# wei-zeng98/piano-a2s

Hardware: AMD Instinct MI355X
Metric: training clips/sec (12 s, 5-bar) (higher is better)
Workload: dtype f32

## Files before the change

### piano_a2s_amd/csrc/a2s_bwd.hip

```cpp
#include "a2s_internal.h"

__global__ __launch_bounds__(256) void log_softmax_bwd_rows(const float* __restrict__ g, const float* __restrict__ y,
                                                            long outer_stride, int inner, float* __restrict__ dx,
                                                            int R, int V, int n_outer, int time_major) {
    const int row = blockIdx.x * 4 + (threadIdx.x >> 6), lane = threadIdx.x & 63;
    if (row >= R) return;
    const int ob = row / inner, in = row % inner;
    const float* gr = g + (long)ob * outer_stride + (long)in * V;
    const float* yr = y + (long)ob * outer_stride + (long)in * V;
    float s = 0.f;
    for (int j = lane; j < V; j += 64) s += gr[j];
    s = wave_sum(s);
    const long orow = time_major ? ((long)in * n_outer + ob) : row;
    for (int j = lane; j < V; j += 64) dx[orow * V + j] = gr[j] - expf(yr[j]) * s;
}

int a2s_log_softmax_bwd_rows_impl(hipStream_t st, const float* g, const float* y, long outer_stride, int inner, float* dx,
                                  int R, int V, int n_outer, int time_major) {
    hipLaunchKernelGGL(log_softmax_bwd_rows, dim3(a2s_cdiv(R, 4)), dim3(256), 0, st, g, y, outer_stride, inner, dx, R, V, n_outer, time_major);
    A2S_CHECK_LAUNCH("log_softmax_bwd_rows");
    return A2S_OK;
}

__global__ void gru_gates_bwd(const float* __restrict__ dh_a, long lda, const float* __restrict__ dh_b, long ldb,
                              const float* __restrict__ save, const float* __restrict__ hprev, long ldhp,
                              float* __restrict__ dgi, long ldgi, float* __restrict__ dgh, long ldgh,
                              float* __restrict__ dgh2, long ldgh2, float* __restrict__ dhprev, long lddp, int R, int H) {
    const long idx = (long)blockIdx.x * blockDim.x + threadIdx.x;
    if (idx >= (long)R * H) return;
    const int r_ = (int)(idx / H), j = (int)(idx % H);
    const float* s = save + (long)r_ * 4 * H;
    const float rg = s[j], zg = s[H + j], ng = s[2 * H + j], ghn = s[3 * H + j];
    float dh = dh_a[(long)r_ * lda + j];
    if (dh_b) dh += dh_b[(long)r_ * ldb + j];
    const float hp = hprev ? hprev[(long)r_ * ldhp + j] : 0.f;
    const GruCellGrad cg = gru_cell_bwd(dh, rg, zg, ng, ghn, hp);
    const float dn = cg.dn, dz = cg.dz, dr = cg.dr;
    float* a = dgi + (long)r_ * ldgi;
    a[j] = dr; a[H + j] = dz; a[2 * H + j] = dn;
    float* b = dgh + (long)r_ * ldgh;
    b[j] = dr; b[H + j] = dz; b[2 * H + j] = cg.dnr;
    if (dgh2) { float* c = dgh2 + (long)r_ * ldgh2; c[j] = dr; c[H + j] = dz; c[2 * H + j] = cg.dnr; }
    dhprev[(long)r_ * lddp + j] = cg.dhz;
}

int a2s_gru_gates_bwd_impl(hipStream_t st, const float* dh_a, long lda, const float* dh_b, long ldb, const float* save,
                           const float* hprev, long ldhp, float* dgi, long ldgi, float* dgh, long ldgh, float* dgh2, long ldgh2,
                           float* dhprev, long lddp, int R, int H) {
    hipLaunchKernelGGL(gru_gates_bwd, dim3(a2s_cdiv((long)R * H, 256)), dim3(256), 0, st, dh_a, lda, dh_b, ldb, save, hprev, ldhp,
                       dgi, ldgi, dgh, ldgh, dgh2, ldgh2, dhprev, lddp, R, H);
    A2S_CHECK_LAUNCH("gru_gates_bwd");
    return A2S_OK;
}

__global__ __launch_bounds__(256) void attn_step_bwd(const float* __restrict__ Kmat, const float* __restrict__ enc,
                                                     const float* __restrict__ q, long ldq, const float* __restrict__ v,
                                                     const float* __restrict__ attw, const float* __restrict__ ctx, long ldctx,
                                                     const float* __restrict__ dctx_a, long ldda, const float* __restrict__ dctx_b, long lddb,
                                                     float* __restrict__ dctx_out, long lddo, float* __restrict__ dq, long lddq,
                                                     float* __restrict__ ds_out, int T, int n_clips, int H) {
    extern __shared__ __attribute__((aligned(16))) float sm[];
    float* dsv = sm;
    float* dc = sm + ((T + 3) & ~3);
    float* red = dc + 2 * H;
    const int b = blockIdx.x, tid = threadIdx.x, lane = tid & 63, wave = tid >> 6;
    const int clip = b % n_clips;
    const float* Kb = Kmat + (long)clip * T * H;
    const float* Eb = enc + (long)clip * T * 2 * H;
    float part = 0.f;
    for (int d = tid; d < 2 * H; d += 256) {
        float g = dctx_a[(long)b * ldda + d];
        if (dctx_b) g += dctx_b[(long)b * lddb + d];
        dc[d] = g;
        if (dctx_out) dctx_out[(long)b * lddo + d] = g;
        part += g * ctx[(long)b * ldctx + d];
    }
    const float dot_ctx = block_sum(part, red);
    for (int t = wave; t < T; t += 4) {
        float s = 0.f;
        for (int d = lane; d < 2 * H; d += 64) s = fmaf(dc[d], Eb[(long)t * 2 * H + d], s);
        s = wave_sum(s);
        if (lane == 0) {
            const float d_s = attw[(long)b * T + t] * (s - dot_ctx);
            dsv[t] = d_s;
            if (ds_out) ds_out[(long)b * T + t] = d_s;
        }
    }
    __syncthreads();
    for (int j = tid; j < H; j += 256) {
        const float eq = exp2x_clamped(q[(long)b * ldq + j]), vj = v[j];
        float acc = 0.f;
        for (int t = 0; t < T; ++t) acc = fmaf(dsv[t], sech2_ek(Kb[(long)t * H + j], eq), acc);
        dq[(long)b * lddq + j] = acc * vj;
    }
}

static int attn_step_bwd_split_impl(hipStream_t st, const float* Kmat, const float* enc, const float* q, long ldq, const float* v,
                                 const float* attw, const float* ctx, long ldctx, const float* dctx_a, long ldda, const float* dctx_b,
                                 long lddb, float* dctx_out, long lddo, float* dq, long lddq, float* ds_out, float* ws, int B, int T, int H,
                                 const a2s_attn_rows* rows);

int a2s_attn_step_bwd_impl(hipStream_t st, const float* Kmat, const float* enc, const float* q, long ldq, const float* v,
                           const float* attw, const float* ctx, long ldctx, const float* dctx_a, long ldda, const float* dctx_b,
                           long lddb, float* dctx_out, long lddo, float* dq, long lddq, float* ds_out, int B, int T, int H, float* ws,
                           const a2s_attn_rows* rows) {
    if (H == 256 && ws)
        return attn_step_bwd_split_impl(st, Kmat, enc, q, ldq, v, attw, ctx, ldctx, dctx_a, ldda, dctx_b, lddb, dctx_out, lddo, dq, lddq, ds_out, ws, B, T, H, rows);
    const int n_clips = rows ? rows->n_clips : B;
    const size_t shm = (((T + 3) & ~3) + 2 * H + 16) * sizeof(float);
    A2S_REQUIRE(H >= 1 && H <= 512, "attn_step_bwd: hidden_size must be in 1 .. 512 (got %d)", H);
    hipLaunchKernelGGL(attn_step_bwd, dim3(B), dim3(256), shm, st, Kmat, enc, q, ldq, v, attw, ctx, ldctx, dctx_a, ldda, dctx_b, lddb, dctx_out, lddo, dq, lddq, ds_out, T, n_clips, H);
    A2S_CHECK_LAUNCH("attn_step_bwd");
    return A2S_OK;
}

__global__ __launch_bounds__(256) void attn_dk_accum(const float* __restrict__ Kmat, const float* __restrict__ q_all,
                                                     const float* __restrict__ ds_all, const float* __restrict__ v,
                                                     float* __restrict__ dK, float* __restrict__ dv_partial, int B, int T, int S,
                                                     const int* __restrict__ row_until, int groups, int H) {
    constexpr int TT = 16;
    const int tiles = (T + TT - 1) / TT;
    const int b = blockIdx.x / tiles, t0 = (blockIdx.x % tiles) * TT;
    __shared__ float dss[TT];
    for (int j0 = 0; j0 < H; j0 += blockDim.x) {
        const int j = j0 + threadIdx.x;
        float kreg[TT], acc[TT];
        float dvj = 0.f;
        if (j < H) {
#pragma unroll
            for (int i = 0; i < TT; ++i) { kreg[i] = (t0 + i < T) ? Kmat[((long)b * T + t0 + i) * H + j] : 0.f; acc[i] = 0.f; }
        }
        for (int sg = 0; sg < S * groups; ++sg) {
            const int s = sg / groups, grp = sg % groups;
            if (row_until && s >= row_until[grp * B + b]) continue;
            const long row = (long)sg * B + b;
// ... 205 lines not shown
}

__global__ __launch_bounds__(256) void col_sum(const float* __restrict__ x, long ld, float* __restrict__ out, long rows, int C,
                                               float alpha, float beta) {
    const int c = blockIdx.x * 64 + (threadIdx.x & 63);
    const int part = threadIdx.x >> 6;
    __shared__ float red[4][64];
    float s = 0.f;
    if (c < C) for (long r = part; r < rows; r += 4) s += x[r * ld + c];
    red[part][threadIdx.x & 63] = s;
    __syncthreads();
    if (part == 0 && c < C) {
        const float t = red[0][threadIdx.x] + red[1][threadIdx.x] + red[2][threadIdx.x] + red[3][threadIdx.x];
        out[c] = alpha * t + (beta != 0.f ? beta * out[c] : 0.f);
    }
}

__global__ __launch_bounds__(256) void col_sum_partial(const float* __restrict__ x, long ld, float* __restrict__ partial, long rows, int C, long rpb) {
    const int c = blockIdx.x * 64 + (threadIdx.x & 63);
    const int part = threadIdx.x >> 6;
    const long r0 = (long)blockIdx.y * rpb, r1 = min(rows, r0 + rpb);
    __shared__ float red[4][64];
    float s = 0.f;
    if (c < C) for (long r = r0 + part; r < r1; r += 4) s += x[r * ld + c];
    red[part][threadIdx.x & 63] = s;
    __syncthreads();
    if (part == 0 && c < C)
        partial[(long)blockIdx.y * C + c] = red[0][threadIdx.x] + red[1][threadIdx.x] + red[2][threadIdx.x] + red[3][threadIdx.x];
}

int a2s_col_sum_impl(hipStream_t st, const float* x, long ld, float* out, long rows, int C, float alpha, float beta, float* ws, size_t ws_floats) {
    if (ws && rows >= 2048 && ws_floats >= (size_t)2 * C) {
        long nb = (rows + 511) / 512;
        if (nb > 1024) nb = 1024;
        if ((size_t)nb * C > ws_floats) nb = (long)(ws_floats / C);
        const long rpb = (rows + nb - 1) / nb;
        nb = (rows + rpb - 1) / rpb;
        hipLaunchKernelGGL(col_sum_partial, dim3(a2s_cdiv(C, 64), (unsigned)nb), dim3(256), 0, st, x, ld, ws, rows, C, rpb);
        A2S_CHECK_LAUNCH("col_sum_partial");
        hipLaunchKernelGGL(col_sum, dim3(a2s_cdiv(C, 64)), dim3(256), 0, st, ws, (long)C, out, nb, C, alpha, beta);
        A2S_CHECK_LAUNCH("col_sum");
        return A2S_OK;
    }
    hipLaunchKernelGGL(col_sum, dim3(a2s_cdiv(C, 64)), dim3(256), 0, st, x, ld, out, rows, C, alpha, beta);
    A2S_CHECK_LAUNCH("col_sum");
    return A2S_OK;
}

__global__ void embed_scatter_add(float* __restrict__ table_grad, const long long* __restrict__ ids64, const int* __restrict__ ids32,
                                  long id_stride, int const_id, const float* __restrict__ g, long ldg, int col0, int R, int E,
                                  const uint8_t* __restrict__ drop, float inv_keep) {
    const long idx = (long)blockIdx.x * blockDim.x + threadIdx.x;
    if (idx >= (long)R * E) return;
    const int r = (int)(idx / E), j = (int)(idx % E);
    const long id = ids64 ? ids64[(long)r * id_stride] : (ids32 ? ids32[(long)r * id_stride] : const_id);
    float v = g[(long)r * ldg + col0 + j];
    if (drop) v = drop[idx] ? v * inv_keep : 0.f;
    atomicAdd(table_grad + id * E + j, v);
}

int a2s_embed_scatter_add_impl(hipStream_t st, float* table_grad, const long long* ids64, const int* ids32, long id_stride,
                               int const_id, const float* g, long ldg, int col0, int R, int E, const uint8_t* drop, float inv_keep) {
    hipLaunchKernelGGL(embed_scatter_add, dim3(a2s_cdiv((long)R * E, 256)), dim3(256), 0, st, table_grad, ids64, ids32, id_stride,
                       const_id, g, ldg, col0, R, E, drop, inv_keep);
    A2S_CHECK_LAUNCH("embed_scatter_add");
    return A2S_OK;
}

__global__ void ew_act_bwd(const float* __restrict__ g, const float* __restrict__ y, float* __restrict__ dx, long n, int act) {
    const long stride = (long)gridDim.x * blockDim.x;
    for (long i = (long)blockIdx.x * blockDim.x + threadIdx.x; i < n; i += stride) {
        const float yy = y[i];
        dx[i] = act == 2 ? g[i] * (1.f - yy * yy) : (yy > 0.f ? g[i] : 0.f);
    }
}
int a2s_ew_act_bwd_impl(hipStream_t st, const float* g, const float* y, float* dx, long n, int act) {
    hipLaunchKernelGGL(ew_act_bwd, dim3(min((long)2048, (n + 255) / 256)), dim3(256), 0, st, g, y, dx, n, act);
    A2S_CHECK_LAUNCH("ew_act_bwd");
    return A2S_OK;
}


static int attn_pair_bwd_sweep(hipStream_t st, const a2s_note_dec_bwd_args& au, const a2s_note_dec_bwd_args& al, int s, AttnPairStep& p);
static int attn_pair_bwd_combine(hipStream_t st, const a2s_note_dec_bwd_args& a, int s, const AttnPairStep& p);

struct NoteBwdStaff { bool mid = false; int cur = 0; int fused_rows_limit = -1; };
static int note_bwd_step_rows(const a2s_note_dec_bwd_args& a, int s) { return (a.row_list && a.n_rows_active) ? a.n_rows_active[s] : a.R; }
static bool note_bwd_step_fused(const a2s_note_dec_bwd_args& a, int s, int rows_limit) {
    const void* ptrs[] = {a.dgi_all, a.dgh_all, a.dq_all, a.dx, a.dh, a.w_ih, a.w_hh, a.attn_w};
    const int n = note_bwd_step_rows(a, s);
    if (rows_limit >= 0 && n > rows_limit) return false;
    return n > 0 && a2s_dec_step_fusable(n, a.H, a.E, 173, ptrs, 8, a.step_ws, a.step_ws_floats);
}

static int note_bwd_step(hipStream_t st, const a2s_note_dec_bwd_args& a, int s, NoteBwdStaff& c, int part, const AttnPairStep* pair) {
    const int H2 = 2 * a.H, ldx = a.E + H2, R = a.R;
    const bool fused = note_bwd_step_fused(a, s, c.fused_rows_limit);
    a2s_attn_rows rows_v = {a.clip_order, a.clip_rank, a.row_until, a.n_clips > 0 ? a.n_clips : R, a.n_active ? a.n_active[s] : 0, s};
    const a2s_attn_rows* rows = a.n_active ? &rows_v : nullptr;
    float* dh_in = a.dh + (long)c.cur * R * H2;
    float* dh_out = a.dh + (long)(c.cur ^ 1) * R * H2;
    if (fused) {
        const int nrows = note_bwd_step_rows(a, s);
        int rc = a2s_note_step_fused_bwd(st, a, s, dh_in, dh_out, rows, nrows, nrows < R ? a.row_list : nullptr);
        if (rc) return rc;
        c.cur ^= 1;
        return A2S_OK;
    }
    int gM = R, gB = 1;
    long gS = 0;
    if (a.m_active && a.n_clips > 0 && a2s_prefix_rows_ok(a.m_active[s], a.n_clips)) { gM = a.m_active[s]; gB = R / a.n_clips; gS = a.n_clips; }
    const float* dos = a.do_all + (long)s * R * 2 * H2;
    float* dgi = a.dgi_all + (long)s * R * 3 * H2;
    float* dgh = a.dgh_all + (long)s * R * 3 * H2;
    float* dxs = a.dx + (long)s * R * ldx;
    int rc = A2S_OK;
    if (part != 2) {
        rc = a2s_gru_gates_bwd_impl(st, dh_in, H2, dos, 2 * H2, a.gates + (long)s * R * 4 * H2, a.h + (long)s * R * H2, H2,
                                    dgi, 3 * H2, dgh, 3 * H2, nullptr, 0, dh_out, H2, R, H2);
        if (rc) return rc;
        if (c.mid) {
            const int nrows = note_bwd_step_rows(a, s);
            rc = a2s_note_step_mid_bwd(st, a, s, dh_out, nrows, nrows < R ? a.row_list : nullptr);
        } else {
            rc = a2s_gemm_impl(st, gM, ldx, 3 * H2, 1.f, dgi, 3 * H2, 1, a.w_ih, ldx, 1, 0.f, dxs, ldx, nullptr, 0, gB, gS * 3 * H2, 0, gS * ldx, 0, a.gemm_ws, a.gemm_ws_bytes);
        }
        if (rc) return rc;
        if (part == 1) return A2S_OK;
    }
    rc = pair ? attn_pair_bwd_combine(st, a, s, *pair)
              : a2s_attn_step_bwd_impl(st, a.keys, a.enc, a.q + (long)s * R * a.H, a.H, a.attn_v, a.attw + (long)s * R * a.T,
                                       a.x + (long)s * R * ldx + a.E, ldx, dxs + a.E, ldx, dos + H2, 2 * H2,
                                       a.dctx_all + (long)s * R * H2, H2, a.dq_all + (long)s * R * a.H, a.H,
                                       a.ds_all + (long)s * R * a.T, R, a.T, a.H, a.attn_ws, rows);
    if (rc) return rc;
    if (!c.mid) {
        rc = a2s_gemm_impl(st, gM, H2, 3 * H2, 1.f, dgh, 3 * H2, 1, a.w_hh, H2, 1, 1.f, dh_out, H2, nullptr, 0, gB, gS * 3 * H2, 0, gS * H2, 0, a.gemm_ws, a.gemm_ws_bytes);
        if (rc) return rc;
    }
    if (c.mid) {
        const int nrows = note_bwd_step_rows(a, s);
        rc = a2s_note_step_mid_bwd_query(st, a, s, dh_out, nrows, nrows < R ? a.row_list : nullptr);
    } else
    rc = a2s_gemm_impl(st, gM, H2, a.H, 1.f, a.dq_all + (long)s * R * a.H, a.H, 1, a.attn_w, 2 * H2, 1, 1.f, dh_out, H2, nullptr, 0, gB, gS * a.H, 0, gS * H2, 0, a.gemm_ws, a.gemm_ws_bytes);
    if (rc) return rc;
    c.cur ^= 1;
    return A2S_OK;
}

static int note_bwd_prepare(hipStream_t st, const a2s_note_dec_bwd_args& a, NoteBwdStaff& c) {
    const int H2 = 2 * a.H, ldx = a.E + H2, R = a.R;
    hipError_t e = hipMemsetAsync(a.dh, 0, sizeof(float) * 2 * R * H2, st);
    if (e == hipSuccess && (a.m_active || a.row_list)) e = hipMemsetAsync(a.dx, 0, sizeof(float) * (size_t)a.steps * R * ldx, st);
    if (e != hipSuccess) A2S_FAIL(A2S_ERR_HIP, "note_decoder_bwd memset: %s", hipGetErrorString(e));
    bool any_fused = false;
    for (int s = a.steps - 1; s >= 0 && !any_fused; --s) any_fused = note_bwd_step_fused(a, s, c.fused_rows_limit);
    const bool mid = a2s_note_step_mid_bwd_ok(a);
    bool any_mid = false;
    if (mid) for (int s = a.steps - 1; s >= 0 && !any_mid; --s) any_mid = !note_bwd_step_fused(a, s, c.fused_rows_limit);
    if (any_fused || any_mid) { int rc = a2s_note_step_fused_bwd_prepare(st, a); if (rc) return rc; }
    c.mid = mid;
    return A2S_OK;
}
static int note_bwd_finish(hipStream_t st, const a2s_note_dec_bwd_args& a, int cur) {
    if (cur != 0) {
        const hipError_t e = hipMemcpyAsync(a.dh, a.dh + (long)a.R * 2 * a.H, sizeof(float) * a.R * 2 * a.H, hipMemcpyDeviceToDevice, st);
        if (e != hipSuccess) A2S_FAIL(A2S_ERR_HIP, "note_decoder_bwd copy: %s", hipGetErrorString(e));
    }
    return A2S_OK;
}

int a2s_note_decoder_bwd_impl(hipStream_t st, const a2s_note_dec_bwd_args& a) {
    if (a2s_note_decoder_bwd_persist_ok(a)) return a2s_note_decoder_bwd_persist(st, a);
    NoteBwdStaff c;
    int rc = note_bwd_prepare(st, a, c);
    if (rc) return rc;
    for (int s = a.steps - 1; s >= 0; --s) {
        rc = note_bwd_step(st, a, s, c, 0, nullptr);
        if (rc) return rc;
    }
    return note_bwd_finish(st, a, c.cur);
}

int a2s_note_decoder_bwd_pair_impl(hipStream_t su, hipStream_t sl, const a2s_note_dec_bwd_args& au, const a2s_note_dec_bwd_args& al, const int* pair_order,
                                   const int* pair_rank, const int* pair_n_active) {
    const a2s_note_dec_bwd_args* as[2] = {&au, &al};
    hipStream_t sts[2] = {su, sl};
    const bool can_pair = a2s_sw(A2S_SW_attn_pair) && su != sl && pair_order && pair_rank && pair_n_active && au.n_active && al.n_active && au.n_clips > 0 &&
                          au.n_clips == al.n_clips && au.R == al.R && au.T == al.T && au.H == 256 && al.H == 256 && au.enc == al.enc && au.attn_ws && al.attn_ws &&
                          !a2s_note_decoder_bwd_persist_ok(au) && !a2s_note_decoder_bwd_persist_ok(al) && a2s_note_step_mid_bwd_ok(au) && a2s_note_step_mid_bwd_ok(al);
    if (!can_pair) {
        const int rc = a2s_note_decoder_bwd_impl(su, au);
        return rc ? rc : a2s_note_decoder_bwd_impl(sl, al);
    }
    const char* who = "note_decoder_bwd_pair";
    hipEvent_t* ev = nullptr;
    { const int rc = a2s_pair_events(who, &ev); if (rc) return rc; }
    NoteBwdStaff cs[2] = {{.fused_rows_limit = a2s_attn_pair_fused_rows()}, {.fused_rows_limit = a2s_attn_pair_fused_rows()}};
    for (int k = 0; k < 2; ++k) { const int rc = note_bwd_prepare(sts[k], *as[k], cs[k]); if (rc) return rc; }
    const int nmax = au.steps > al.steps ? au.steps : al.steps;
    for (int s = nmax - 1; s >= 0; --s) {
        bool in[2], fused[2] = {false, false};
        for (int k = 0; k < 2; ++k) { in[k] = s < as[k]->steps; if (in[k]) fused[k] = note_bwd_step_fused(*as[k], s, cs[k].fused_rows_limit); }
        AttnPairStep p = {pair_order, pair_rank, au.n_clips, pair_n_active[s], s, 1, au.T};
        const bool joint = in[0] && in[1] && cs[0].mid && cs[1].mid && !fused[0] && !fused[1] && p.n_active > 0 && au.n_active[s] > 0 && al.n_active[s] > 0;
        if (!joint) {
            for (int k = 0; k < 2; ++k)
                if (in[k]) { const int rc = note_bwd_step(sts[k], *as[k], s, cs[k], 0, nullptr); if (rc) return rc; }
            continue;
        }
        for (int k = 0; k < 2; ++k) { const int rc = note_bwd_step(sts[k], *as[k], s, cs[k], 1, nullptr); if (rc) return rc; }
        int rc = a2s_record_wait(ev[1], sl, su, who);
        if (rc == A2S_OK) rc = attn_pair_bwd_sweep(su, au, al, s, p);
        if (rc == A2S_OK) rc = a2s_record_wait(ev[0], su, sl, who);
        if (rc) return rc;
        for (int k = 0; k < 2; ++k) { const int rc2 = note_bwd_step(sts[k], *as[k], s, cs[k], 2, &p); if (rc2) return rc2; }
    }
    for (int k = 0; k < 2; ++k) { const int rc = note_bwd_finish(sts[k], *as[k], cs[k].cur); if (rc) return rc; }
    return A2S_OK;
}


__global__ void transpose_f32(const float* __restrict__ in, float* __restrict__ out, int rows, int cols) {
    const int idx = blockIdx.x * blockDim.x + threadIdx.x;
    if (idx >= rows * cols) return;
    const int c = idx / rows, r = idx % rows;
    out[idx] = in[(long)r * cols + c];
}

int a2s_gru_seq_bwd_impl(hipStream_t st, const float* dout, long do_bstride, long do_tstride, const float* out, long out_bstride,
                         long out_tstride, const float* gates, const float* w_hh, const float* dhn, float* dgi_all, float* dgh_shift,
                         float* dgh_first, float* dhbuf, float* dgh_tmp, int B, int T, int H, int reverse, float* ws, size_t ws_bytes,
                         float* ranges_out, int* ranges_valid) {
    A2S_REQUIRE(dout && out && gates && w_hh && dgi_all && dgh_shift && dgh_first && dhbuf && dgh_tmp, "gru_seq_bwd: null tensor");
    if (ranges_valid) *ranges_valid = 0;
    hipError_t e;
    if (dhn) e = hipMemcpyAsync(dhbuf, dhn, sizeof(float) * B * H, hipMemcpyDeviceToDevice, st);
    else e = hipMemsetAsync(dhbuf, 0, sizeof(float) * B * H, st);
    if (e != hipSuccess) A2S_FAIL(A2S_ERR_HIP, "gru_seq_bwd init: %s", hipGetErrorString(e));
    e = hipMemsetAsync(dgh_shift, 0, sizeof(float) * (size_t)B * T * 3 * H, st);
    if (e != hipSuccess) A2S_FAIL(A2S_ERR_HIP, "gru_seq_bwd memset: %s", hipGetErrorString(e));
    const bool fused = a2s_sw(A2S_SW_gru_fused) && H % 32 == 0 && ws && ws_bytes >= sizeof(float) * 3 * H * H && ((uintptr_t)ws % 16 == 0);
    if (fused) {
        hipLaunchKernelGGL(transpose_f32, dim3(a2s_cdiv(3 * H * H, 256)), dim3(256), 0, st, w_hh, ws, 3 * H, H);
        A2S_CHECK_LAUNCH("transpose_f32");
    }
    if (fused && a2s_gru_seq_bwd_persist_ok(B, T, H, ws, ws_bytes, sizeof(float) * 3 * (size_t)H * H)) {
        const int rc = a2s_gru_seq_bwd_persist_impl(st, dout, do_bstride, do_tstride, out, out_bstride, out_tstride, gates, ws, dhn, dgi_all, dgh_shift, dgh_first,
                                                    B, T, H, reverse, ws, sizeof(float) * 3 * (size_t)H * H, ws_bytes, ranges_out);
        if (rc == A2S_OK && ranges_out && ranges_valid) *ranges_valid = 1;
        return rc;
    }
    if (fused && ws_bytes >= sizeof(float) * (3 * (size_t)H * H + 3 * (size_t)B * H) && (3 * H * H) % 4 == 0) {
        float* tmp[2] = {dgh_tmp, ws + 3 * (size_t)H * H};
        auto tix = [&](int s) { return reverse ? T - 1 - s : s; };
        int cur = 0, p = 0;
        {
            const int s = T - 1, t = tix(s), tp = reverse ? t + 1 : t - 1;
            float* dgh = (s == 0) ? dgh_first : tmp[p];
            int rc = a2s_gru_gates_bwd_impl(st, dhbuf, H, dout + (long)t * do_tstride, do_bstride, gates + (long)t * B * 4 * H,
                                            s == 0 ? nullptr : out + (long)tp * out_tstride, out_bstride,
                                            dgi_all + (long)t * 3 * H, (long)T * 3 * H, dgh, 3 * H,
                                            s == 0 ? nullptr : dgh_shift + (long)tp * 3 * H, (long)T * 3 * H, dhbuf + (long)B * H, H, B, H);
            if (rc) return rc;
            cur = 1;
        }
        for (int s = T - 1; s >= 1; --s) {
            const int sp = s - 1, t = tix(sp), tp = reverse ? t + 1 : t - 1;
            float* dgh_out = (sp == 0) ? dgh_first : tmp[p ^ 1];
            int rc = a2s_gru_bptt_step_impl(st, tmp[p], ws, dhbuf + (long)cur * B * H, dout + (long)t * do_tstride, do_bstride,
                                            gates + (long)t * B * 4 * H, sp == 0 ? nullptr : out + (long)tp * out_tstride, out_bstride,
                                            dgi_all + (long)t * 3 * H, (long)T * 3 * H, dgh_out,
                                            sp == 0 ? nullptr : dgh_shift + (long)tp * 3 * H, (long)T * 3 * H,
                                            dhbuf + (long)(cur ^ 1) * B * H, B, H);
            if (rc) return rc;
            cur ^= 1; p ^= 1;
        }
        return A2S_OK;
    }
    int cur = 0;
    for (int s = T - 1; s >= 0; --s) {
        const int t = reverse ? T - 1 - s : s;
        const int tp = reverse ? t + 1 : t - 1;
        float* dh_in = dhbuf + (long)cur * B * H;
        float* dh_out = dhbuf + (long)(cur ^ 1) * B * H;
        float* dgh = (s == 0) ? dgh_first : dgh_tmp;
        int rc = a2s_gru_gates_bwd_impl(st, dh_in, H, dout + (long)t * do_tstride, do_bstride, gates + (long)t * B * 4 * H,
                                        s == 0 ? nullptr : out + (long)tp * out_tstride, out_bstride,
                                        dgi_all + (long)t * 3 * H, (long)T * 3 * H, dgh, 3 * H,
                                        s == 0 ? nullptr : dgh_shift + (long)tp * 3 * H, (long)T * 3 * H, dh_out, H, B, H);
        if (rc) return rc;
        if (s > 0) {
            if (fused) rc = a2s_skinny_gemm_acc_impl(st, dgh, 3 * H, ws, 3 * H, dh_out, H, B, H, 3 * H);
            else rc = a2s_gemm_impl(st, B, H, 3 * H, 1.f, dgh, 3 * H, 1, w_hh, H, 1, 1.f, dh_out, H, nullptr, 0, 1, 0, 0, 0, 0, ws, ws_bytes);
            if (rc) return rc;
        }
        cur ^= 1;
    }
    return A2S_OK;
}
// ... 628 lines not shown
                        const float d_s = aw[r] * (acc[r] - dotn);
                        dsv[li * chunk + f2] = d_s;
                        if (ds_out) ds_out[arow + f2] = d_s;
                    }
                }
            }
        }
    }
    __syncthreads();
#pragma unroll
    for (int pass = 0; pass < 2; ++pass) {
        const int side = pass == 0 ? pre_side : 1 - pre_side;
        const int smask = (onmask >> (side * NQ)) & ((1 << NQ) - 1);
        if (!smask) continue;
        const AttnPairBwdSide& sd = side ? s1 : s0;
        const float* Kb = sd.Kmat + ((long)b * T + t0) * H;
        const float* dsj = dsv + side * NQ * chunk;
        f32x4 q4[NQ], acc[NQ];
#pragma unroll
        for (int j = 0; j < NQ; ++j) {
            acc[j] = (f32x4){0.f, 0.f, 0.f, 0.f};
            q4[j] = ((smask >> j) & 1) ? *reinterpret_cast<const f32x4*>(sd.q + ((long)j * n_clips + b) * ldq + c4 * 4) : (f32x4){0.f, 0.f, 0.f, 0.f};
#pragma unroll
            for (int c = 0; c < 4; ++c) q4[j][c] = exp2x_clamped(q4[j][c]);
        }
        int i = rg;
        auto tile = [&](const f32x4 (&k)[4]) {
#pragma unroll
            for (int j = 0; j < NQ; ++j) {
                if (!((smask >> j) & 1)) continue;
#pragma unroll
                for (int u = 0; u < 4; ++u) {
                    const float w = dsj[j * chunk + i + 4 * u];
#pragma unroll
                    for (int c = 0; c < 4; ++c) acc[j][c] = fmaf(w, sech2_ek(k[u][c], q4[j][c]), acc[j][c]);
                }
            }
        };
        if (pass == 0) {
#pragma unroll
            for (int p = 0; p < KPRE; ++p)
                if (i + 12 < n) { tile(kpre[p]); i += 16; }
        }
        for (; i + 12 < n; i += 16) {
            f32x4 k[4];
#pragma unroll
            for (int u = 0; u < 4; ++u) k[u] = ld_kv<NT>(Kb + (long)(i + 4 * u) * H + c4 * 4);
            tile(k);
        }
        for (; i < n; i += 4) {
            const f32x4 k0 = ld_kv<NT>(Kb + (long)i * H + c4 * 4);
#pragma unroll
            for (int j = 0; j < NQ; ++j) {
                if (!((smask >> j) & 1)) continue;
                const float w = dsj[j * chunk + i];
#pragma unroll
                for (int c = 0; c < 4; ++c) acc[j][c] = fmaf(w, sech2_ek(k0[c], q4[j][c]), acc[j][c]);
            }
        }
        if (pass == 1) __syncthreads();
        if (rg > 0) {
#pragma unroll
            for (int j = 0; j < NQ; ++j) red4[(j * 3 + rg - 1) * 64 + c4] = acc[j];
        }
        __syncthreads();
        if (rg == 0) {
            const f32x4 v4 = {sd.v[c4 * 4], sd.v[c4 * 4 + 1], sd.v[c4 * 4 + 2], sd.v[c4 * 4 + 3]};
#pragma unroll
            for (int j = 0; j < NQ; ++j) {
                if (!((smask >> j) & 1)) continue;
                f32x4 a = acc[j];
#pragma unroll
                for (int u = 0; u < 3; ++u) { const f32x4 o = red4[(j * 3 + u) * 64 + c4];
#pragma unroll
                    for (int c = 0; c < 4; ++c) a[c] += o[c]; }
#pragma unroll
                for (int c = 0; c < 4; ++c) a[c] *= v4[c];
                *reinterpret_cast<f32x4*>(sd.dq_partial + (((long)slot * NQ + j) * G + g) * H + c4 * 4) = a;
            }
        }
    }
}

__global__ __launch_bounds__(256) void attn_bwd_combine256(const float* __restrict__ dq_partial, float* __restrict__ dq, long lddq, int G,
                                                           const int* __restrict__ clip_rank, const int* __restrict__ row_until,
                                                           int n_clips, int groups, int n_active, int step, float* __restrict__ ds_out,
                                                           int T, float* __restrict__ dctx_out, long lddo) {
    const int b = blockIdx.x, j = threadIdx.x;
    const int clip = b % n_clips, grp = b / n_clips;
    const int slot = clip_rank ? clip_rank[clip] : clip;
    if (slot >= n_active || (row_until && step >= row_until[b])) {
        dq[(long)b * lddq + j] = 0.f;
        if (ds_out) for (int t = j; t < T; t += 256) ds_out[(long)b * T + t] = 0.f;
        if (dctx_out) for (int d = j; d < 512; d += 256) dctx_out[(long)b * lddo + d] = 0.f;
        return;
    }
    const float* pb = dq_partial + ((long)slot * groups + grp) * G * 256;
    float s = 0.f;
    for (int g0 = 0; g0 < G; g0 += 8) {
        float p[8];
#pragma unroll
        for (int u = 0; u < 8; ++u) p[u] = (g0 + u < G) ? pb[(long)(g0 + u) * 256 + j] : 0.f;
#pragma unroll
        for (int u = 0; u < 8; ++u) s += p[u];
    }
    dq[(long)b * lddq + j] = s;
}

template <int NQ>
static void launch_bwd_mq(hipStream_t st, int nwg, size_t shm, const float* Kmat, const float* enc, const float* q, long ldq, const float* v,
                          const float* attw, const float* ctx, long ldctx, const float* dctx_a, long ldda, const float* dctx_b, long lddb,
                          float* dctx_out, long lddo, float* ws, float* ds_out, int T, int G, int chunk, const a2s_attn_rows& r, bool nt) {
    if (nt) hipLaunchKernelGGL((attn_bwd_split256_mq<NQ, true>), dim3(nwg), dim3(256), shm, st, Kmat, enc, q, ldq, v, attw, ctx, ldctx, dctx_a, ldda, dctx_b, lddb,
                               dctx_out, lddo, ws, ds_out, T, G, chunk, r.clip_order, r.row_until, r.step, r.n_clips);
    else hipLaunchKernelGGL((attn_bwd_split256_mq<NQ, false>), dim3(nwg), dim3(256), shm, st, Kmat, enc, q, ldq, v, attw, ctx, ldctx, dctx_a, ldda, dctx_b, lddb,
                            dctx_out, lddo, ws, ds_out, T, G, chunk, r.clip_order, r.row_until, r.step, r.n_clips);
}

static int attn_step_bwd_split_impl(hipStream_t st, const float* Kmat, const float* enc, const float* q, long ldq, const float* v,
                                 const float* attw, const float* ctx, long ldctx, const float* dctx_a, long ldda, const float* dctx_b,
                                 long lddb, float* dctx_out, long lddo, float* dq, long lddq, float* ds_out, float* ws, int B, int T, int H,
                                 const a2s_attn_rows* rows) {
    A2S_REQUIRE(H == 256 && ws, "attn_step_bwd_split: needs hidden_size 256 and a workspace");
    A2S_REQUIRE(ldq % 4 == 0 && ldctx % 4 == 0 && ldda % 4 == 0 && (!dctx_b || lddb % 4 == 0) && (!dctx_out || lddo % 4 == 0),
                "attn_step_bwd_split: row strides must be multiples of 4 floats");
    A2S_REQUIRE(((uintptr_t)q | (uintptr_t)ctx | (uintptr_t)dctx_a | (uintptr_t)dctx_b | (uintptr_t)dctx_out | (uintptr_t)Kmat | (uintptr_t)enc) % 16 == 0,
                "attn_step_bwd_split: 16-byte alignment");
    a2s_attn_rows r = {nullptr, nullptr, nullptr, B, B, 0};
    if (rows) r = *rows;
    A2S_REQUIRE(r.n_clips > 0 && B % r.n_clips == 0, "attn_step_bwd_split: rows (%d) must be a multiple of the clips (%d)", B, r.n_clips);
    const int groups = B / r.n_clips;
    A2S_REQUIRE(groups <= A2S_ATTN_MAX_GROUPS, "attn_step_bwd_split: at most %d fused bars (got %d)", A2S_ATTN_MAX_GROUPS, groups);
    A2S_REQUIRE(r.n_active >= 0 && r.n_active <= r.n_clips && (!r.clip_order || r.clip_rank), "attn_step_bwd_split: bad row compaction");
    int G = 1, chunk = T;
    ws += A2S_ATTN_TICKETS;
    const bool nt = a2s_sw(A2S_SW_attn_nt) > 0 && r.n_active >= a2s_sw(A2S_SW_attn_nt) && groups == 1;
    if (r.n_active > 0) {
        a2s_attn_split_geometry(r.n_active, T, &G, &chunk);
        {
            const int fine = 4;
            if (fine > 0 && r.n_active <= fine && G == a2s_attn_max_split() && 2 * G <= 64) {
                int c = (T + 2 * G - 1) / (2 * G);
                c = (c + 3) & ~3;
                G = (T + c - 1) / c;
                chunk = c;
            }
        }
        const int nwg = r.n_active * G;
        if (groups == 1) {
            const size_t shm = a2s_attn_bulk_lds((chunk + 3 * 64 * 4) * sizeof(float), r.n_active, 1);
            if (nt) hipLaunchKernelGGL(attn_bwd_split256<true>, dim3(nwg), dim3(256), shm, st, Kmat, enc, q, ldq, v, attw, ctx, ldctx, dctx_a, ldda, dctx_b, lddb,
                                       dctx_out, lddo, ws, ds_out, T, G, chunk, r.clip_order);
            else hipLaunchKernelGGL(attn_bwd_split256<false>, dim3(nwg), dim3(256), shm, st, Kmat, enc, q, ldq, v, attw, ctx, ldctx, dctx_a, ldda, dctx_b, lddb,
                                    dctx_out, lddo, ws, ds_out, T, G, chunk, r.clip_order);
        } else {
            const size_t scratch = (size_t)groups * 3 * 64 * 4 > (size_t)groups * ATT_DCS + 16 ? (size_t)groups * 3 * 64 * 4 : (size_t)groups * ATT_DCS + 16;
            const size_t shm = a2s_attn_bulk_lds(((size_t)groups * chunk + scratch) * sizeof(float), r.n_active, 3);
#define A2S_BWD_MQ(N) launch_bwd_mq<N>(st, nwg, shm, Kmat, enc, q, ldq, v, attw, ctx, ldctx, dctx_a, ldda, dctx_b, lddb, dctx_out, lddo, ws, ds_out, T, G, chunk, r, nt)
            switch (groups) {
                case 2: A2S_BWD_MQ(2); break;
                case 3: A2S_BWD_MQ(3); break;
                case 4: A2S_BWD_MQ(4); break;
                default: A2S_BWD_MQ(5); break;
            }
#undef A2S_BWD_MQ
        }
        A2S_CHECK_LAUNCH("attn_bwd_split256");
    }
    hipLaunchKernelGGL(attn_bwd_combine256, dim3(B), dim3(256), 0, st, ws, dq, lddq, G, r.clip_rank, r.row_until, r.n_clips, groups, r.n_active, r.step,
                       ds_out, T, dctx_out, lddo);
    A2S_CHECK_LAUNCH("attn_bwd_combine256");
    return A2S_OK;
}

template <int NQ>
static void launch_bwd_pair(hipStream_t st, int nwg, size_t shm, const AttnPairBwdSide& s0, const AttnPairBwdSide& s1, const float* enc, long ldq, long ldctx,
                            long ldda, long lddb, long lddo, int T, const AttnPairStep& p) {
    hipLaunchKernelGGL((attn_bwd_split256_pair<NQ, false>), dim3(nwg), dim3(256), shm, st, s0, s1, enc, ldq, ldctx, ldda, lddb, lddo, T, p.G, p.chunk,
                       p.clip_order, p.step, p.n_clips);
}
static long g_attn_pair_bwd_launches = 0;
long a2s_attn_pair_bwd_launches(void) { return g_attn_pair_bwd_launches; }

static AttnPairBwdSide attn_pair_bwd_side(const a2s_note_dec_bwd_args& a, int s) {
    const int H2 = 2 * a.H, ldx = a.E + H2;
    const long R = a.R;
    return AttnPairBwdSide{a.keys, a.q + (long)s * R * a.H, a.attn_v, a.attw + (long)s * R * a.T, a.x + (long)s * R * ldx + a.E, a.dx + (long)s * R * ldx + a.E,
                           a.do_all + (long)s * R * 2 * H2 + H2, a.dctx_all + (long)s * R * H2, a.attn_ws + A2S_ATTN_TICKETS, a.ds_all + (long)s * R * a.T, a.row_until};
}

static int attn_pair_bwd_sweep(hipStream_t st, const a2s_note_dec_bwd_args& au, const a2s_note_dec_bwd_args& al, int s, AttnPairStep& p) {
    const int T = au.T, H2 = 2 * au.H, ldx = au.E + H2, groups = au.R / p.n_clips;
    A2S_REQUIRE(au.H == 256 && au.E == al.E && au.enc == al.enc && au.R == al.R && groups >= 1 && groups <= A2S_ATTN_MAX_GROUPS && ldx % 4 == 0,
                "attn_pair_bwd_sweep: the staves must decode the same rows over the same encoder outputs");
    a2s_attn_split_geometry(p.n_active, T, &p.G, &p.chunk);
    const AttnPairBwdSide s0 = attn_pair_bwd_side(au, s), s1 = attn_pair_bwd_side(al, s);
    const size_t red = (size_t)groups * 3 * 64 * 4, img = (size_t)2 * groups * ATT_DCS + 16;
    const size_t shm = a2s_attn_bulk_lds(((size_t)2 * groups * p.chunk + (red > img ? red : img)) * sizeof(float), p.n_active, 3);
    const int nwg = p.n_active * p.G;
#define A2S_BWD_PAIR(N) launch_bwd_pair<N>(st, nwg, shm, s0, s1, au.enc, au.H, ldx, ldx, 2 * H2, H2, T, p)
    switch (groups) {
        case 1: A2S_BWD_PAIR(1); break;
        case 2: A2S_BWD_PAIR(2); break;
        case 3: A2S_BWD_PAIR(3); break;
        case 4: A2S_BWD_PAIR(4); break;
        default: A2S_BWD_PAIR(5); break;
    }
#undef A2S_BWD_PAIR
    A2S_CHECK_LAUNCH("attn_bwd_split256_pair");
    __atomic_fetch_add(&g_attn_pair_bwd_launches, 1, __ATOMIC_RELAXED);
    return A2S_OK;
}

static int attn_pair_bwd_combine(hipStream_t st, const a2s_note_dec_bwd_args& a, int s, const AttnPairStep& p) {
    const int H2 = 2 * a.H;
    const long R = a.R;
    hipLaunchKernelGGL(attn_bwd_combine256, dim3(a.R), dim3(256), 0, st, a.attn_ws + A2S_ATTN_TICKETS, a.dq_all + (long)s * R * a.H, (long)a.H, p.G, p.clip_rank,
                       a.row_until, p.n_clips, a.R / p.n_clips, p.n_active, p.step, a.ds_all + (long)s * R * a.T, a.T, a.dctx_all + (long)s * R * H2, (long)H2);
    A2S_CHECK_LAUNCH("attn_bwd_combine256");
    return A2S_OK;
}
```

### piano_a2s_amd/csrc/a2s_internal.h

```cpp
#pragma once
#include "a2s_common.h"
#include "../../include/a2s.h"
#include "a2s_switches.h"

static inline int a2s_attn_pair_fused_rows(void) {
    const int cap = a2s_sw(A2S_SW_dec_fused_max_rows), v = a2s_sw(A2S_SW_attn_pair_fused_rows);
    return v < cap ? v : cap;
}
static inline unsigned a2s_persist_dbg(void) {
    return (a2s_sw(A2S_SW_persist_force_agent) ? PERSIST_DBG_FORCE_AGENT : 0u) | (a2s_sw(A2S_SW_persist_inject_abort) ? PERSIST_DBG_INJECT_ABORT : 0u);
}

int a2s_absmax_impl(hipStream_t st, const float* x, long n, float* out);
size_t a2s_gemm_workspace_bytes_impl(int M, int N, int batch, int splitk);
int a2s_gemm_pick_splitk_impl(int M, int N, int K, int batch);
int a2s_gemm_bnstats_slots(int period);
void a2s_gemm_debug_tile_impl(int cfg);
int a2s_gemm_affine_impl(hipStream_t st, int M, int N, int K, float alpha, const float* A, long sAm, long sAk,
    const float* B, long sBk, long sBn, float beta, float* C, long ldc, const float* bias, int act,
    int batch, long bsA, long bsB, long bsC, int splitk, float* ws, size_t ws_bytes,
    const float* a_scale, const float* a_shift, int a_period, const float* b_scale, const float* b_shift, int b_period,
    const float* ep_y, const float* ep_mean, const float* ep_invstd, const float* ep_scale, const float* ep_shift,
    float* ep_partial, int ep_period, int two_term, const float* a_absmax, const float* b_absmax);
int a2s_gemm_impl(hipStream_t st, int M, int N, int K, float alpha, const float* A, long sAm, long sAk,
// ... 37 lines not shown
    const uint8_t* mask, float inv_keep, long n, int C);
size_t a2s_conv3x3_wgrad_workspace_bytes_impl(int Cin, int Cout);
int a2s_conv3x3_wgrad_impl(hipStream_t st, const float* dy, const float* x, const float* in_scale, const float* in_shift, float* dW,
    float* ws, size_t ws_bytes, int B, int T, int F, int Cin, int Cout, const float* bn_y, const float* bn_mean,
    const float* bn_invstd, const float* bn_scale, const float* bn_shift, const float* bn_c12, float* dy_out,
    const float* dy_absmax, const float* act_absmax);
int a2s_bn_bwd_impl(hipStream_t st, const float* g, const float* x, const float* mean, const float* invstd, const float* scale,
    const float* shift, const uint8_t* mask, float inv_keep, float* dgamma, float* dbeta, float* dx, float* partial,
    float* c12, long rows, int C, int F, float* dx_absmax);
int a2s_bn_bwd_from_partial_impl(hipStream_t st, const float* g, const float* x, const float* mean, const float* invstd, const float* scale,
    const float* shift, float* dgamma, float* dbeta, float* dx, const float* partial, int nblocks, float* c12,
    long rows, int C, int F, float* dx_absmax);
int a2s_bn_bwd_stats_impl(hipStream_t st, const float* g, const float* x, const float* mean, const float* invstd, const float* scale,
    const float* shift, const uint8_t* mask, float inv_keep, float* partial, float* sums, long rows, int C, int F);
int a2s_bn_bwd_apply_impl(hipStream_t st, const float* g, const float* x, const float* mean, const float* invstd, const float* scale,
    const float* shift, const uint8_t* mask, float inv_keep, const float* sums_local, const float* sums_global,
    double count_global, float* dgamma, float* dbeta, float* dx, float* c12, long rows, int C, int F);
int a2s_bn_bwd_sums_from_partial_impl(hipStream_t st, const float* partial, int nblocks, int C, float* sums);
int a2s_bn_bwd_c12_from_sums_impl(hipStream_t st, const float* sums_local, const float* sums_global, double count_global, float* dgamma, float* dbeta,
    float* c12, int C);
size_t a2s_bn_bwd_partial_floats_impl(long rows, int C, int F);

int a2s_channel_absmax_impl(hipStream_t st, const float* x, long rows, int C, int F, float* out);
bool a2s_conv_rows_eligible(int F, int Cin);
int a2s_conv_rows_blocks(int B, int T, int F);
size_t a2s_conv_rows_workspace_floats(int Cin);
long a2s_conv_rows16_c20_launches(void);
int a2s_conv3x3_rows_impl(hipStream_t st, const float* x, const float* w, float* y, const float* in_scale, const float* in_shift,
    const float* in_absmax, float* stat_partial, float* out_absmax, int B, int T, int F, int Cin, int Cout, int flip,
    float* ws, const float* yl, const float* yl_mean, const float* yl_invstd, const float* yl_scale, const float* yl_shift,
    const float* x_absmax);

bool a2s_wgrad_rows_eligible(int F, int Cin, int Cout);
int a2s_conv3x3_wgrad_rows_bn_impl(hipStream_t st, const float* g, const float* y, const float* mean, const float* invstd, const float* scale,
    const float* shift, const float* c12, const float* g_absmax, int g_absmax_n, const float* y_absmax, float* dz_out,
    float* dz_absmax_out, const float* x, const float* in_scale, const float* in_shift, float* dW, float* ws, size_t ws_bytes,
    int B, int T, int F, int Cin, int Cout, const float* act_absmax);
int a2s_conv3x3_wgrad_rows_impl(hipStream_t st, const float* dy, const float* x, const float* in_scale, const float* in_shift, float* dW, float* ws,
    size_t ws_bytes, int B, int T, int F, int Cin, int Cout, const float* dy_absmax, const float* act_absmax);

struct StepFinArgs {
    const float* logits; long ldl;
    float* probs; long probs_bstride;
    const long long* gt; long gt_bstride;
    const float* emb;
    float* xnext; long ldx;
    const uint8_t* drop; float inv_keep;
    int* argmax_out; long am_bstride;
    int* eos_seen; long long* lengths; int* n_done; int* steps_exec;
    const int* t_base;
    const int* row_until;
    int n_clips;
    int R, V, E, t, teacher_force, eos_id, max_t;
};
struct a2s_grammar_ref { const signed char* next; int n_states; int* row_state; };
int a2s_gru_gates_fwd_impl(hipStream_t st, const float* gi, long ldgi, const float* gh, long ldgh, const float* hprev,
    long ldhp, float* hout, long ldho, float* hout2, long ldho2, float* save, int R, int H);
int a2s_gru_bptt_step_impl(hipStream_t st, const float* dgh, const float* w_hh_t, const float* dhz_in, const float* dout, long ld_dout,
    const float* save, const float* hprev, long ld_hprev, float* dgi, long ld_dgi, float* dgh_out, float* dgh2,
    long ld_dgh2, float* dhz_out, int R, int H);
int a2s_skinny_gemm_acc_impl(hipStream_t st, const float* A, long lda, const float* Bt, long ldb, float* Cm, long ldc, int R, int N, int K);
int a2s_gru_seq_fwd_impl(hipStream_t st, const float* gi_all, long gi_bstride, long gi_tstride, const float* w_hh,
    const float* b_hh, float* out, long out_bstride, long out_tstride, float* hbuf, float* gh,
    float* save, float* hn, int B, int T, int H, int reverse, float* ws, size_t ws_bytes);
int a2s_attn_step_fwd_impl(hipStream_t st, const float* Kmat, const float* enc, const float* q, long ldq, const float* v,
    float* ctx, long ldctx, float* ctx2, long ldctx2, float* attw, int B, int T, int H,
    const int* n_done, int n_rows_total, float* ws, const a2s_attn_rows* rows = nullptr, a2s_attn_deferred* defer = nullptr);
int a2s_log_softmax_rows_impl(hipStream_t st, const float* x, long ldx, float* y, long ldy, int* argmax_out, int R, int V);
int a2s_embed_rows_impl(hipStream_t st, const float* table, const long long* ids64, const int* ids32, long id_stride,
    int const_id, float* out, long ldo, int col0, int R, int E, const uint8_t* drop, float inv_keep);
int a2s_note_decoder_fwd_impl(hipStream_t st, const a2s_note_dec_args& a, int* steps_done);
int a2s_note_decoder_fwd_grammar_impl(hipStream_t st, const a2s_note_dec_args& a, const a2s_grammar_ref& g, int* steps_done);
int a2s_note_decoder_fwd_pair_impl(hipStream_t su, hipStream_t sl, const a2s_note_dec_args& au, const a2s_note_dec_args& al, const int* pair_order,
    const int* pair_rank, const int* pair_n_active, int* done_u, int* done_l);
int a2s_staff_emb_fwd_impl(hipStream_t st, const float* note_emb, const float* const* w ,
    const long long* ids64, const int* ids32, long id_bstride, const long long* lengths,
    long len_stride, float* out, long ldo, int col0, float* hsave, int R, int maxlen, int E, int S);
int a2s_note_decoder_zero_unwritten(hipStream_t st, const a2s_note_dec_args& a, const char* who );
size_t a2s_attn_workspace_floats_impl(int B, int T, int H, int groups);
size_t a2s_attn_bulk_lds(size_t shm, int n_active, int backward);
long a2s_attn_pair_launches(void);
struct AttnPairStep { const int* clip_order; const int* clip_rank; int n_clips; int n_active; int step; int G; int chunk; };
int a2s_pair_events(const char* who, hipEvent_t** ev_out);
static inline int a2s_record_wait(hipEvent_t ev, hipStream_t from, hipStream_t to, const char* who) {
    hipError_t e = hipEventRecord(ev, from);
    if (e == hipSuccess) e = hipStreamWaitEvent(to, ev, 0);
    if (e != hipSuccess) A2S_FAIL(A2S_ERR_HIP, "%s: event: %s", who, hipGetErrorString(e));
    return A2S_OK;
}

int a2s_log_softmax_bwd_rows_impl(hipStream_t st, const float* g, const float* y, long outer_stride, int inner, float* dx,
    int R, int V, int n_outer, int time_major);
int a2s_gru_gates_bwd_impl(hipStream_t st, const float* dh_a, long lda, const float* dh_b, long ldb, const float* save,
    const float* hprev, long ldhp, float* dgi, long ldgi, float* dgh, long ldgh, float* dgh2, long ldgh2,
    float* dhprev, long lddp, int R, int H);
int a2s_attn_step_bwd_impl(hipStream_t st, const float* Kmat, const float* enc, const float* q, long ldq, const float* v,
    const float* attw, const float* ctx, long ldctx, const float* dctx_a, long ldda, const float* dctx_b,
    long lddb, float* dctx_out, long lddo, float* dq, long lddq, float* ds_out, int B, int T, int H, float* ws,
    const a2s_attn_rows* rows = nullptr);
int a2s_attn_dk_accum_impl(hipStream_t st, const float* Kmat, const float* q_all, const float* ds_all, const float* v,
    float* dK, float* dv_partial, int B, int T, int S, int H, const int* row_until, int groups);
int a2s_attn_denc_accum_impl(hipStream_t st, const float* attw_all, const float* dctx_all, float* dEnc, int B, int T, int S, int H2,
    const int* row_until, int groups);
long a2s_attn_dk_ahead_launches(void);
long a2s_attn_denc_launches(void);
int a2s_col_sum_impl(hipStream_t st, const float* x, long ld, float* out, long rows, int C, float alpha, float beta, float* ws, size_t ws_floats);
int a2s_embed_scatter_add_impl(hipStream_t st, float* table_grad, const long long* ids64, const int* ids32, long id_stride,
    int const_id, const float* g, long ldg, int col0, int R, int E, const uint8_t* drop, float inv_keep);
int a2s_ew_act_bwd_impl(hipStream_t st, const float* g, const float* y, float* dx, long n, int act);
int a2s_note_decoder_bwd_impl(hipStream_t st, const a2s_note_dec_bwd_args& a);
int a2s_note_decoder_bwd_pair_impl(hipStream_t su, hipStream_t sl, const a2s_note_dec_bwd_args& au, const a2s_note_dec_bwd_args& al, const int* pair_order,
    const int* pair_rank, const int* pair_n_active);
int a2s_gru_seq_bwd_impl(hipStream_t st, const float* dout, long do_bstride, long do_tstride, const float* out, long out_bstride,
    long out_tstride, const float* gates, const float* w_hh, const float* dhn, float* dgi_all, float* dgh_shift,
    float* dgh_first, float* dhbuf, float* dgh_tmp, int B, int T, int H, int reverse, float* ws, size_t ws_bytes,
    float* ranges_out, int* ranges_valid);
int a2s_staff_emb_bwd_impl(hipStream_t st, const float* note_emb, const float* const* w, float* const* grads_dev, float* note_emb_grad,
    const long long* ids64, const int* ids32, long id_bstride, const long long* lengths, long len_stride,
    const float* dout, long lddo, int col0, const float* hsave, int R, int maxlen, int E, int S);
long a2s_attn_pair_bwd_launches(void);

size_t a2s_note_step_fused_head_floats(void);
size_t a2s_note_step_workspace_floats_impl(int H, int E);
int a2s_dec_mid_launches(void);
bool a2s_dec_step_fusable(int R, int H, int E, int V, const void* const* ptrs, int nptrs, const float* ws, size_t ws_floats, bool greedy = false);
int a2s_note_step_fused_fwd(hipStream_t st, const a2s_note_dec_args& a, int si, int so, int sv, int sv_next, int t, const int* t_base, int tf, bool last,
    int nrows, const int* rowmap, const a2s_attn_deferred* defer = nullptr);
int a2s_note_step_fused_bwd_prepare(hipStream_t st, const a2s_note_dec_bwd_args& a);
int a2s_note_step_fused_bwd(hipStream_t st, const a2s_note_dec_bwd_args& a, int s, const float* dh_in, float* dh_out, const a2s_attn_rows* rows,
    int nrows, const int* rowmap);
bool a2s_note_step_mid_ok(int H, int E, const void* const* ptrs, int nptrs);
int a2s_note_step_mid_gru(hipStream_t st, const a2s_note_dec_args& a, int si, int so, int sv, int sv_next, int nrows, const int* rowmap);
bool a2s_note_step_mid_bwd_ok(const a2s_note_dec_bwd_args& a);
int a2s_note_step_mid_bwd(hipStream_t st, const a2s_note_dec_bwd_args& a, int s, float* dh_out, int nrows, const int* rowmap);
int a2s_note_step_mid_bwd_query(hipStream_t st, const a2s_note_dec_bwd_args& a, int s, float* dh_out, int nrows, const int* rowmap);

bool a2s_grammar_ref_ok(const a2s_grammar_ref& g, int R, int V);
int a2s_grammar_argmax_rows_impl(hipStream_t st, const float* x, long ldx, float* y, long ldy, const signed char* next, int n_states, int* row_state,
    int* choice_out, int R, int V);
int a2s_grammar_step_finalize_impl(hipStream_t st, const StepFinArgs& a, const a2s_grammar_ref& g);
int a2s_grammar_launches_impl(void);

int a2s_attn_align_rows_impl(hipStream_t st, const float* attw, long ldw, int R, int T, int* peak_out, float* weight_out, float* centroid_out,
    long out_stride, const int* n_done = nullptr, int n_rows_total = 0);
int a2s_align_launches_impl(void);
int a2s_note_decoder_fwd_align_impl(hipStream_t st, const a2s_note_dec_args& a, const a2s_align_args& g, int* steps_done);

int a2s_render_notes_impl(hipStream_t st, const int* programs, int rows_per_clip, int n_samples, float* wave, long wave_bstride, int B);
int a2s_render_launches_impl(void);

int a2s_transpose_targets_impl(hipStream_t st, const int* new_key, const int* interval, const int* token_map, int n_rows, int V, const int* semitones,
    const float* detune, long long* key, long long* upper, long long* lower, int bars, int U, int L, int bins_per_semitone, float* eff_bins, int* counters,
    int B);
int a2s_shift_bins_impl(hipStream_t st, const float* x, float* y, const float* eff_bins, int B, int rows, int F);
int a2s_augment_launches_impl(void);

int a2s_tempo_plan_impl(hipStream_t st, const float* x, int B, int rows, int F, const float* u, float R, int min_frames, int* content, int* step,
    int* counters);
int a2s_stretch_frames_impl(hipStream_t st, const float* x, float* y, const int* step, int B, int rows, int F);
int a2s_tempo_launches_impl(void);

struct BeamStepArgs {
    const float* logits; long ldl;
    const float* emb;
    float* xnext; long ldx;
    float* h; int h_cols;
    float* q; int q_cols;
    const signed char* next; int n_states; int* row_state;
    float* score; int* finished; int* done_count;
    int* token_hist; int* parent_hist; float* score_hist;
    float* probs_scratch;
    int* n_done; int* steps_exec;
    int B, K, V, E, t, max_t, eos_id, pad_id;
};
struct BeamBackArgs {
    const float* score; const int* token_hist; const int* parent_hist; const float* probs_scratch;
    float* probs; long probs_bstride;
    int* ids_out; long ids_bstride; long long* lengths_out; float* score_out;
    const int* steps_exec;
    float alpha;
    int B, K, V, max_t, eos_id, pad_id;
};
bool a2s_beam_args_ok(const a2s_beam_args& g, int R, int n_clips, int V);
int a2s_beam_init_impl(hipStream_t st, const a2s_beam_args& g, int* n_done, int B, int steps);
int a2s_beam_step_finalize_impl(hipStream_t st, const BeamStepArgs& a);
int a2s_beam_backtrack_impl(hipStream_t st, const BeamBackArgs& a);
int a2s_beam_launches_impl(void);
int a2s_note_decoder_fwd_beam_impl(hipStream_t st, const a2s_note_dec_args& a, const a2s_beam_args& g, int* steps_done);

unsigned* a2s_persist_latch_ptr(void);
void a2s_persist_latch_set(void* p);
a2s_device_geom a2s_device_geometry(void);
bool a2s_gru_seq_fwd_persist_ok(const float* w_hh, const float* gi, int B, int T, int H, float* ws, size_t ws_bytes);
int a2s_gru_seq_fwd_persist_impl(hipStream_t st, const float* gi_all, long gi_bstride, long gi_tstride, const float* w_hh, const float* b_hh, float* out,
    long out_bstride, long out_tstride, float* save, float* hn, int B, int T, int H, int reverse, float* ws, size_t ws_bytes);
bool a2s_gru_seq_bwd_persist_ok(int B, int T, int H, float* ws, size_t ws_bytes, size_t ws_used);
int a2s_gru_seq_bwd_persist_impl(hipStream_t st, const float* dout, long do_bstride, long do_tstride, const float* out, long out_bstride, long out_tstride,
    const float* gates, const float* w_hh_t, const float* dhn, float* dgi_all, float* dgh_shift, float* dgh_first, int B, int T,
    int H, int reverse, float* ws, size_t ws_off, size_t ws_bytes, float* ranges_out);

int a2s_dec_persist_launches(void);
bool a2s_note_decoder_fwd_persist_ok(const a2s_note_dec_args& a);
int a2s_note_decoder_fwd_persist(hipStream_t st, const a2s_note_dec_args& a, int* steps_done);
bool a2s_note_decoder_bwd_persist_ok(const a2s_note_dec_bwd_args& a);
int a2s_note_decoder_bwd_persist(hipStream_t st, const a2s_note_dec_bwd_args& a);

int a2s_nll_loss_impl(hipStream_t st, const float* logp, const long long* target, long rows, int V, long long ignore_index,
    float* loss_out , float* dlogp , float gscale, double* partial, int nblocks);
int a2s_nll_grad_impl(hipStream_t st, float* dlogp, const long long* target, const float* loss_out, float gscale, long rows, int V, long long ignore_index);
int a2s_clip_adadelta_impl(hipStream_t st, float* params, float* grads, float* square_avg, float* acc_delta, long n, const float* loss,
    float max_norm, float lr, float rho, float eps, float* ctl , double* partial, int nblocks, int zero_grad);

int a2s_edit_distance_max_len_impl(void);
long a2s_edit_distance_launches(void);
int a2s_edit_distance_impl(hipStream_t st, const int* ref, const long long* ref_off, const int* hyp, const long long* hyp_off, const int* order,
    int n_pairs, int max_ref_len, int max_hyp_len, int* dist);
// ... 10 lines not shown
```

### piano_a2s_amd/csrc/a2s_seq.hip

```cpp
#include <vector>
#include "a2s_internal.h"

__global__ void gru_gates_fwd(const float* __restrict__ gi, long ldgi, const float* __restrict__ gh, long ldgh,
                              const float* __restrict__ hprev, long ldhp, float* __restrict__ hout, long ldho,
                              float* __restrict__ hout2, long ldho2, float* __restrict__ save, int R, int H) {
    const long idx = (long)blockIdx.x * blockDim.x + threadIdx.x;
    if (idx >= (long)R * H) return;
    const int r_ = (int)(idx / H), j = (int)(idx % H);
    const float* a = gi + (long)r_ * ldgi;
    const float* b = gh + (long)r_ * ldgh;
    const float rg = fast_sigmoid(a[j] + b[j]);
    const float zg = fast_sigmoid(a[H + j] + b[H + j]);
    const float ghn = b[2 * H + j];
    const float ng = fast_tanh(a[2 * H + j] + rg * ghn);
    const float hp = hprev[(long)r_ * ldhp + j];
    const float hn = (1.f - zg) * ng + zg * hp;
    hout[(long)r_ * ldho + j] = hn;
    if (hout2) hout2[(long)r_ * ldho2 + j] = hn;
    if (save) {
        float* s = save + (long)r_ * 4 * H;
        s[j] = rg; s[H + j] = zg; s[2 * H + j] = ng; s[3 * H + j] = ghn;
    }
}

// ... 225 lines not shown
    float* sc = sm;
    float* red = sm + ((T + 3) & ~3);
    const int b = blockIdx.x, tid = threadIdx.x, lane = tid & 63, wave = tid >> 6;
    const int clip = b % n_clips;
    const float* Kb = Kmat + (long)clip * T * H;
    const float* Eb = enc + (long)clip * T * 2 * H;
    float qv[PER], vv[PER];
#pragma unroll
    for (int i = 0; i < PER; ++i) {
        const int j = lane + i * 64;
        qv[i] = j < H ? exp2x_clamped(q[(long)b * ldq + j]) : 0.f;
        vv[i] = j < H ? v[j] : 0.f;
    }
    for (int t = wave; t < T; t += 4) {
        float s = 0.f;
#pragma unroll
        for (int i = 0; i < PER; ++i) {
            const int j = lane + i * 64;
            if (j < H) s = fmaf(vv[i], tanh_ek(Kb[(long)t * H + j], qv[i]), s);
        }
        s = wave_sum(s);
        if (lane == 0) sc[t] = s;
    }
    __syncthreads();
    float m = -INFINITY;
    for (int t = tid; t < T; t += 256) m = fmaxf(m, sc[t]);
    m = block_max(m, red);
    float l = 0.f;
    for (int t = tid; t < T; t += 256) { const float p = __expf(sc[t] - m); sc[t] = p; l += p; }
    l = block_sum(l, red);
    const float inv = 1.f / l;
    __syncthreads();
    for (int t = tid; t < T; t += 256) {
        const float w = sc[t] * inv;
        sc[t] = w;
        if (attw) attw[(long)b * T + t] = w;
    }
    __syncthreads();
    for (int d = tid; d < 2 * H; d += 256) {
        float acc = 0.f;
        int t = 0;
        for (; t + 4 <= T; t += 4) {
            const float e0 = Eb[(long)(t + 0) * 2 * H + d], e1 = Eb[(long)(t + 1) * 2 * H + d];
            const float e2 = Eb[(long)(t + 2) * 2 * H + d], e3 = Eb[(long)(t + 3) * 2 * H + d];
            acc = fmaf(sc[t], e0, acc); acc = fmaf(sc[t + 1], e1, acc);
            acc = fmaf(sc[t + 2], e2, acc); acc = fmaf(sc[t + 3], e3, acc);
        }
        for (; t < T; ++t) acc = fmaf(sc[t], Eb[(long)t * 2 * H + d], acc);
        ctx[(long)b * ldctx + d] = acc;
        if (ctx2) ctx2[(long)b * ldctx2 + d] = acc;
    }
}

static int attn_step_fwd_split_impl(hipStream_t st, const float* Kmat, const float* enc, const float* q, long ldq, const float* v,
                                 float* ctx, long ldctx, float* ctx2, long ldctx2, float* attw, float* ws, int B, int T, int H,
                                 const int* n_done, int n_rows_total, const a2s_attn_rows* rows, a2s_attn_deferred* defer = nullptr);

int a2s_attn_step_fwd_impl(hipStream_t st, const float* Kmat, const float* enc, const float* q, long ldq, const float* v,
                           float* ctx, long ldctx, float* ctx2, long ldctx2, float* attw, int B, int T, int H,
                           const int* n_done, int n_rows_total, float* ws, const a2s_attn_rows* rows, a2s_attn_deferred* defer) {
    if (defer) defer->G = 0;
    if (H == 256 && ws)
        return attn_step_fwd_split_impl(st, Kmat, enc, q, ldq, v, ctx, ldctx, ctx2, ldctx2, attw, ws, B, T, H, n_done, n_rows_total, rows, defer);
    const int n_clips = rows ? rows->n_clips : B;
    const size_t shm = (((T + 3) & ~3) + 16) * sizeof(float);
    A2S_REQUIRE(H >= 1 && H <= 512, "attn_step_fwd: hidden_size must be in 1 .. 512 (got %d)", H);
#define A2S_ATTN_FWD(P) hipLaunchKernelGGL(attn_step_fwd<P>, dim3(B), dim3(256), shm, st, Kmat, enc, q, ldq, v, ctx, ldctx, ctx2, ldctx2, attw, T, n_done, n_rows_total, n_clips, H)
    switch ((H + 63) / 64) {
        case 1: A2S_ATTN_FWD(1); break;
        case 2: A2S_ATTN_FWD(2); break;
        case 3: A2S_ATTN_FWD(3); break;
        case 4: A2S_ATTN_FWD(4); break;
        case 5: A2S_ATTN_FWD(5); break;
        case 6: A2S_ATTN_FWD(6); break;
        case 7: A2S_ATTN_FWD(7); break;
        default: A2S_ATTN_FWD(8); break;
    }
#undef A2S_ATTN_FWD
    A2S_CHECK_LAUNCH("attn_step_fwd");
    return A2S_OK;
}


__global__ __launch_bounds__(256) void note_step_finalize(StepFinArgs a) {
    const int row = blockIdx.x * 4 + (threadIdx.x >> 6), lane = threadIdx.x & 63;
    if (row >= a.R) return;
    if (*a.n_done >= a.R && a.gt == nullptr) return;
    const int t = a.t + (a.t_base ? *a.t_base : 0);
    if (t >= a.max_t) return;
    const float* lg = a.logits + (long)row * a.ldl;
    const bool finished = a.row_until && t >= a.row_until[row];
    float m = -INFINITY; int mi = 0x7fffffff;
    for (int j = lane; j < a.V; j += 64) { const float x = lg[j]; if (x > m) { m = x; mi = j; } }
#pragma unroll
    for (int o = 32; o > 0; o >>= 1) {
        const float om = __shfl_xor(m, o, 64); const int oi = __shfl_xor(mi, o, 64);
        if (om > m || (om == m && oi < mi)) { m = om; mi = oi; }
    }
    if (!finished) {
        float s = 0.f;
        for (int j = lane; j < a.V; j += 64) s += expf(lg[j] - m);
        s = wave_sum(s);
        const float lse = m + logf(s);
        float* pr = a.probs + (long)row * a.probs_bstride + (long)t * a.V;
        for (int j = lane; j < a.V; j += 64) pr[j] = lg[j] - lse;
    }
    const long long g = a.gt ? a.gt[(long)row * a.gt_bstride + t] : -1;
    const int tf = (a.teacher_force >> (a.n_clips > 0 ? row / a.n_clips : 0)) & 1;
    const int next_id = (a.gt && tf) ? (int)g : mi;
    for (int j = lane; j < a.E; j += 64) {
        float e = a.emb[(long)next_id * a.E + j];
        if (a.drop) e = a.drop[(long)row * a.E + j] ? e * a.inv_keep : 0.f;
        a.xnext[(long)row * a.ldx + j] = e;
    }
    if (lane == 0 && !finished) {
        if (row == 0 && a.steps_exec) *a.steps_exec = t + 1;
        if (a.argmax_out) a.argmax_out[(long)row * a.am_bstride + t] = mi;
        const bool hit = a.gt ? (g == a.eos_id) : (mi == a.eos_id);
        if (hit) {
            if (!a.eos_seen[row]) { a.eos_seen[row] = 1; atomicAdd(a.n_done, 1); }
            a.lengths[row] = t + 1;
        }
    }
}

static int a2s_note_step_finalize_impl(hipStream_t st, const StepFinArgs& a) {
    hipLaunchKernelGGL(note_step_finalize, dim3(a2s_cdiv(a.R, 4)), dim3(256), 0, st, a);
    A2S_CHECK_LAUNCH("note_step_finalize");
    return A2S_OK;
}

__global__ __launch_bounds__(256) void log_softmax_rows(const float* __restrict__ x, long ldx, float* __restrict__ y, long ldy,
                                                        int* __restrict__ argmax_out, int R, int V) {
    const int row = blockIdx.x * 4 + (threadIdx.x >> 6), lane = threadIdx.x & 63;
    if (row >= R) return;
    const float* lg = x + (long)row * ldx;
    float m = -INFINITY; int mi = 0x7fffffff;
    for (int j = lane; j < V; j += 64) { const float v = lg[j]; if (v > m) { m = v; mi = j; } }
#pragma unroll
    for (int o = 32; o > 0; o >>= 1) {
        const float om = __shfl_xor(m, o, 64); const int oi = __shfl_xor(mi, o, 64);
        if (om > m || (om == m && oi < mi)) { m = om; mi = oi; }
    }
    float s = 0.f;
    for (int j = lane; j < V; j += 64) s += expf(lg[j] - m);
    s = wave_sum(s);
    const float lse = m + logf(s);
    for (int j = lane; j < V; j += 64) y[(long)row * ldy + j] = lg[j] - lse;
    if (argmax_out && lane == 0) argmax_out[row] = mi;
}

int a2s_log_softmax_rows_impl(hipStream_t st, const float* x, long ldx, float* y, long ldy, int* argmax_out, int R, int V) {
    hipLaunchKernelGGL(log_softmax_rows, dim3(a2s_cdiv(R, 4)), dim3(256), 0, st, x, ldx, y, ldy, argmax_out, R, V);
    A2S_CHECK_LAUNCH("log_softmax_rows");
    return A2S_OK;
}

__global__ void embed_rows(const float* __restrict__ table, const long long* __restrict__ ids64, const int* __restrict__ ids32,
                           long id_stride, int const_id, float* __restrict__ out, long ldo, int col0, int R, int E,
                           const uint8_t* __restrict__ drop, float inv_keep) {
    const long idx = (long)blockIdx.x * blockDim.x + threadIdx.x;
    if (idx >= (long)R * E) return;
    const int r = (int)(idx / E), j = (int)(idx % E);
    const long id = ids64 ? ids64[(long)r * id_stride] : (ids32 ? ids32[(long)r * id_stride] : const_id);
    float e = table[id * E + j];
    if (drop) e = drop[idx] ? e * inv_keep : 0.f;
    out[(long)r * ldo + col0 + j] = e;
}

int a2s_embed_rows_impl(hipStream_t st, const float* table, const long long* ids64, const int* ids32, long id_stride,
                        int const_id, float* out, long ldo, int col0, int R, int E, const uint8_t* drop, float inv_keep) {
    hipLaunchKernelGGL(embed_rows, dim3(a2s_cdiv((long)R * E, 256)), dim3(256), 0, st, table, ids64, ids32, id_stride, const_id,
                       out, ldo, col0, R, E, drop, inv_keep);
    A2S_CHECK_LAUNCH("embed_rows");
    return A2S_OK;
}

typedef a2s_note_dec_args NoteDecArgs;

static int attn_pair_sweep(hipStream_t st, const NoteDecArgs& au, const NoteDecArgs& al, int sv, AttnPairStep& p);
static int attn_pair_combine(hipStream_t st, const NoteDecArgs& a, int si, int sv, const AttnPairStep& p);
static int note_step_rows(const NoteDecArgs& a, int t) { return (a.row_list && a.n_rows_active && t >= 0) ? a.n_rows_active[t] : a.R; }
static bool note_step_fusable(const NoteDecArgs& a, int t = -1, int rows_limit = -1) {
    const void* ptrs[] = {a.x, a.h, a.o, a.q, a.w_ih, a.w_hh, a.out_w, a.attn_w};
    const int n = note_step_rows(a, t);
    if (rows_limit >= 0 && n > rows_limit) return false;
    return n > 0 && a2s_dec_step_fusable(n, a.H, a.E, a.V, ptrs, 8, a.step_ws, a.step_ws_floats, a.gt == nullptr && !a.gates);
}
static bool note_step_mid(const NoteDecArgs& a, const int* t_base) {
    const void* ptrs[] = {a.x, a.h, a.o, a.q, a.w_ih, a.w_hh, a.out_w, a.attn_w};
    return !t_base && a2s_note_step_mid_ok(a.H, a.E, ptrs, 8);
}
static int enqueue_query(hipStream_t st, const NoteDecArgs& a, int si, int sv) {
    const int H2 = 2 * a.H;
    return a2s_gemm_impl(st, a.R, a.H, H2, 1.f, a.h + (long)si * a.R * H2, H2, 1, a.attn_w, 1, 2 * H2, 0.f, a.q + (long)sv * a.R * a.H, a.H, a.attn_b, 0, 1, 0,
                         0, 0, 0, a.gemm_ws, a.gemm_ws_bytes);
}

struct NoteStepMode {
    const a2s_grammar_ref* grammar = nullptr;
    const a2s_beam_args* beam = nullptr;
    const a2s_align_args* align = nullptr;
    const int* t_base = nullptr;
    bool parity_slots = false;
    bool few_row = false;
    int fused_rows_limit = -1;
    const char* label = "note_decoder";
};
struct NoteStep { int si, so, sv, sv_next, t, tf; bool fused, last; const AttnPairStep* pair; };
static NoteStep note_step_at(const NoteDecArgs& a, const NoteStepMode& m, int s, bool fused, const AttnPairStep* pair = nullptr) {
    const int i = m.parity_slots ? s & 1 : s, o = m.parity_slots ? (s + 1) & 1 : s + 1;
    return {.si = i, .so = o, .sv = i, .sv_next = o, .t = s, .tf = a.tf_flags ? a.tf_flags[s] : 0, .fused = fused, .last = s + 1 == a.steps, .pair = pair};
}

static int enqueue_note_step(hipStream_t st, const NoteDecArgs& a, const NoteStepMode& m, const NoteStep& k) {
    const int si = k.si, so = k.so, sv = k.sv, sv_next = k.sv_next, t = k.t, H2 = 2 * a.H, ldx = a.E + H2;
    float* xs = a.x + (long)si * a.R * ldx;
    float* qs = a.q + (long)sv * a.R * a.H;
    float* os = a.o + (long)sv * a.R * 2 * H2;
    a2s_attn_rows rows_v = {a.clip_order, a.clip_rank, a.row_until, a.n_clips > 0 ? a.n_clips : a.R, a.n_active ? a.n_active[t] : 0, t};
    const a2s_attn_rows* rows = a.n_active ? &rows_v : nullptr;
    int rc;
    if (k.fused) {
        a2s_attn_deferred defer;
        defer.G = 0;
        rc = a2s_attn_step_fwd_impl(st, a.keys, a.enc, qs, a.H, a.attn_v, xs + a.E, ldx, os + H2, 2 * H2, a.attw ? a.attw + (long)sv * a.R * a.T : nullptr, a.R, a.T, a.H,
                                    a.gt ? nullptr : a.n_done, a.R, a.attn_ws, rows, (a.gt && a.n_active && !m.t_base) ? &defer : nullptr);
        if (rc) return rc;
        const int nrows = note_step_rows(a, m.t_base ? -1 : t);
        return a2s_note_step_fused_fwd(st, a, si, so, sv, sv_next, t, m.t_base, k.tf, k.last, nrows, nrows < a.R ? a.row_list : nullptr, defer.G > 0 ? &defer : nullptr);
    }
    int gM = a.R, gB = 1;
    long gS = 0;
    if (a.m_active && a.n_clips > 0 && a2s_prefix_rows_ok(a.m_active[t], a.n_clips)) { gM = a.m_active[t]; gB = a.R / a.n_clips; gS = a.n_clips; }
    const float* hp = a.h + (long)si * a.R * H2;
    float* hq = a.h + (long)so * a.R * H2;
    const a2s_attn_rows rows_b = {nullptr, nullptr, nullptr, a.n_clips, a.n_clips, t};
    if (m.beam) rows = &rows_b;
    const int* attn_done = (a.gt || (m.beam && m.beam->K > 1)) ? nullptr : a.n_done;
    float* attw_s = m.align ? m.align->attw_step : (a.attw ? a.attw + (long)sv * a.R * a.T : nullptr);
    float* q_left = nullptr;
    const bool mid = note_step_mid(a, m.t_base);
    if (!mid) {
        rc = a2s_gemm_impl(st, gM, a.H, H2, 1.f, hp, H2, 1, a.attn_w, 1, 2 * H2, 0.f, qs, a.H, a.attn_b, 0, gB, gS * H2, 0, gS * a.H, 0, a.gemm_ws, a.gemm_ws_bytes);
        if (rc) return rc;
        rc = a2s_gemm_impl(st, gM, 3 * H2, H2, 1.f, hp, H2, 1, a.w_hh, 1, H2, 0.f, a.gh, 3 * H2, a.b_hh, 0, gB, gS * H2, 0, gS * 3 * H2, 0, a.gemm_ws, a.gemm_ws_bytes);
        if (rc) return rc;
    }
    rc = (mid && k.pair) ? attn_pair_combine(st, a, si, sv, *k.pair)
                         : a2s_attn_step_fwd_impl(st, a.keys, a.enc, qs, a.H, a.attn_v, xs + a.E, ldx, os + H2, 2 * H2, attw_s, a.R, a.T, a.H, attn_done, a.R, a.attn_ws, rows);
    if (rc) return rc;
    if (m.align) { rc = a2s_attn_align_rows_impl(st, attw_s, a.T, a.R, a.T, m.align->peak + t, m.align->weight + t, m.align->centroid + t, m.align->out_stride, attn_done, a.R); if (rc) return rc; }
    if (mid) {
        const int nrows = note_step_rows(a, t);
        rc = a2s_note_step_mid_gru(st, a, si, so, sv, k.last ? -1 : sv_next, nrows, nrows < a.R ? a.row_list : nullptr);
        if (rc) return rc;
        if (!k.last) q_left = a.q + (long)sv_next * a.R * a.H;
    } else {
        rc = a2s_gemm_impl(st, gM, 3 * H2, ldx, 1.f, xs, ldx, 1, a.w_ih, 1, ldx, 0.f, a.gi, 3 * H2, a.b_ih, 0, gB, gS * ldx, 0, gS * 3 * H2, 0, a.gemm_ws, a.gemm_ws_bytes);
        if (rc) return rc;
        rc = a2s_gru_gates_fwd_impl(st, a.gi, 3 * H2, a.gh, 3 * H2, hp, H2, hq, H2, os, 2 * H2, a.gates ? a.gates + (long)sv * a.R * 4 * H2 : nullptr, a.R, H2);
        if (rc) return rc;
        rc = a2s_gemm_impl(st, gM, a.V, 2 * H2, 1.f, os, 2 * H2, 1, a.out_w, 1, 2 * H2, 0.f, a.logits, a.V, a.out_b, 0, gB, gS * 2 * H2, 0, gS * a.V, 0, a.gemm_ws, a.gemm_ws_bytes);
        if (rc) return rc;
    }
    if (m.beam) {
        const a2s_beam_args& g = *m.beam;
        const BeamStepArgs bs = {a.logits, a.V, a.emb, a.x + (long)so * a.R * ldx, ldx, hq, H2, q_left, a.H, g.next_state, g.n_states, g.row_state, g.score, g.finished,
                                 g.done_count, g.token_hist, g.parent_hist, g.score_hist, g.probs_scratch, a.n_done, a.steps_exec, a.n_clips, g.K, a.V, a.E, t, a.steps,
                                 a.eos_id, g.pad_id};
        return a2s_beam_step_finalize_impl(st, bs);
    }
    StepFinArgs f;
    f.logits = a.logits; f.ldl = a.V; f.probs = a.probs; f.probs_bstride = a.probs_bstride;
    f.gt = a.gt; f.gt_bstride = a.gt_bstride; f.emb = a.emb;
    f.xnext = a.x + (long)so * a.R * ldx; f.ldx = ldx;
    f.drop = a.drop ? a.drop + (long)so * a.R * a.E : nullptr; f.inv_keep = a.inv_keep;
    f.argmax_out = a.argmax_out; f.am_bstride = a.am_bstride;
    f.eos_seen = a.eos_seen; f.lengths = a.lengths; f.n_done = a.n_done; f.steps_exec = a.steps_exec;
    f.t_base = m.t_base;
    f.row_until = a.n_active ? a.row_until : nullptr; f.n_clips = a.n_clips > 0 ? a.n_clips : a.R;
    f.R = a.R; f.V = a.V; f.E = a.E; f.t = t; f.teacher_force = k.tf; f.eos_id = a.eos_id; f.max_t = a.steps;
    if (m.grammar) return a2s_grammar_step_finalize_impl(st, f, *m.grammar);
    return a2s_note_step_finalize_impl(st, f);
}

__global__ void advance_counter(int* p, int inc) { if (threadIdx.x == 0 && blockIdx.x == 0) *p += inc; }

static int note_decoder_greedy_graph(hipStream_t st, const NoteDecArgs& a, const NoteStepMode& m, int* steps_done) {
    int chunk = a.poll > 0 ? a.poll : 16;
    if (chunk & 1) ++chunk;
    hipError_t e = hipMemsetAsync(a.t_base, 0, sizeof(int), st);
    if (e != hipSuccess) A2S_FAIL(A2S_ERR_HIP, "greedy graph memset: %s", hipGetErrorString(e));
    hipGraph_t graph = nullptr;
    hipGraphExec_t exec = nullptr;
    const bool fused = m.few_row && note_step_fusable(a);
    int rc = fused ? enqueue_query(st, a, 0, 0) : A2S_OK;
    if (rc) return rc;
    e = hipStreamBeginCapture(st, hipStreamCaptureModeRelaxed);
    if (e != hipSuccess) A2S_FAIL(A2S_ERR_HIP, "hipStreamBeginCapture: %s", hipGetErrorString(e));
    for (int j = 0; j < chunk && rc == A2S_OK; ++j)
        rc = enqueue_note_step(st, a, m, {.si = j & 1, .so = (j + 1) & 1, .sv = 0, .sv_next = 0, .t = j, .tf = 0, .fused = fused, .last = false, .pair = nullptr});
    if (rc == A2S_OK) hipLaunchKernelGGL(advance_counter, dim3(1), dim3(64), 0, st, a.t_base, chunk);
    e = hipStreamEndCapture(st, &graph);
    if (rc != A2S_OK) { if (graph) (void)hipGraphDestroy(graph); return rc; }
    if (e != hipSuccess) A2S_FAIL(A2S_ERR_HIP, "hipStreamEndCapture: %s", hipGetErrorString(e));
    e = hipGraphInstantiate(&exec, graph, nullptr, nullptr, 0);
    if (e != hipSuccess) { (void)hipGraphDestroy(graph); A2S_FAIL(A2S_ERR_HIP, "hipGraphInstantiate: %s", hipGetErrorString(e)); }
    int launched = 0;
    while (launched < a.steps) {
        e = hipGraphLaunch(exec, st);
        if (e != hipSuccess) break;
        launched += chunk;
        int done = 0;
        e = hipMemcpyAsync(&done, a.n_done, sizeof(int), hipMemcpyDeviceToHost, st);
        if (e == hipSuccess) e = hipStreamSynchronize(st);
        if (e != hipSuccess || done >= a.R) break;
    }
    (void)hipGraphExecDestroy(exec);
    (void)hipGraphDestroy(graph);
    if (e != hipSuccess) A2S_FAIL(A2S_ERR_HIP, "greedy graph replay: %s", hipGetErrorString(e));
    if (steps_done) *steps_done = launched < a.steps ? launched : a.steps;
    return A2S_OK;
}

int a2s_note_decoder_zero_unwritten(hipStream_t st, const NoteDecArgs& a, const char* who) {
    const long H2 = 2L * a.H, ldx = a.E + H2, n = a.steps, R = a.R;
    hipError_t e = hipMemsetAsync(a.h + R * H2, 0, sizeof(float) * n * R * H2, st);
    if (e == hipSuccess) e = hipMemsetAsync(a.x + R * ldx, 0, sizeof(float) * n * R * ldx, st);
    if (e == hipSuccess) e = hipMemsetAsync(a.q, 0, sizeof(float) * n * R * a.H, st);
    if (e == hipSuccess) e = hipMemsetAsync(a.o, 0, sizeof(float) * n * R * 2 * H2, st);
    if (e == hipSuccess && a.gates) e = hipMemsetAsync(a.gates, 0, sizeof(float) * n * R * 4 * H2, st);
    if (e != hipSuccess) A2S_FAIL(A2S_ERR_HIP, "%s memset: %s", who, hipGetErrorString(e));
    return A2S_OK;
}
static bool note_decoder_tail_rows(const NoteDecArgs& a) { return a.row_list && a.n_rows_active && a.steps > 0; }

static int note_decoder_run(hipStream_t st, const NoteDecArgs& a, const NoteStepMode& m, int* steps_done) {
    if (note_decoder_tail_rows(a)) { const int rc = a2s_note_decoder_zero_unwritten(st, a, "note_decoder"); if (rc) return rc; }
    const bool mid = note_step_mid(a, nullptr);
    bool prev_q = false;
    int s = 0;
    for (; s < a.steps; ++s) {
        const NoteStep k = note_step_at(a, m, s, m.few_row && note_step_fusable(a, s, m.fused_rows_limit));
        if ((k.fused || mid) && !prev_q) { const int rc = enqueue_query(st, a, k.si, k.sv); if (rc) return rc; }
        prev_q = k.fused || mid;
        const int rc = enqueue_note_step(st, a, m, k);
        if (rc) return rc;
        if (!a.gt && a.poll > 0 && ((s + 1) % a.poll == 0) && s + 1 < a.steps) {
            int done = 0;
            hipError_t e = hipMemcpyAsync(&done, a.n_done, sizeof(int), hipMemcpyDeviceToHost, st);
            if (e == hipSuccess) e = hipStreamSynchronize(st);
            if (e != hipSuccess) A2S_FAIL(A2S_ERR_HIP, "%s poll: %s", m.label, hipGetErrorString(e));
            if (done >= a.R) { ++s; break; }
        }
    }
    if (steps_done) *steps_done = s;
    return A2S_OK;
}

static int note_decoder_fwd(hipStream_t st, const NoteDecArgs& a, int* steps_done, const a2s_grammar_ref* grammar) {
    if (!grammar && a2s_note_decoder_fwd_persist_ok(a)) return a2s_note_decoder_fwd_persist(st, a, steps_done);
    if (!a.gt && a.use_graph && a.t_base && !a.gates && !a.attw && !a.drop && st != nullptr)
        return note_decoder_greedy_graph(st, a, {.grammar = grammar, .t_base = a.t_base, .few_row = !grammar}, steps_done);
    return note_decoder_run(st, a, {.grammar = grammar, .few_row = !grammar}, steps_done);
}

int a2s_note_decoder_fwd_impl(hipStream_t st, const NoteDecArgs& a, int* steps_done) { return note_decoder_fwd(st, a, steps_done, nullptr); }

int a2s_note_decoder_fwd_grammar_impl(hipStream_t st, const NoteDecArgs& a, const a2s_grammar_ref& g, int* steps_done) {
    A2S_REQUIRE(!a.gt && !a.tf_flags_dev, "note_decoder_fwd_grammar: greedy decoding only (ground truth given)");
    A2S_REQUIRE(!a.gates && !a.attw && !a.drop && !a.n_active && !a.row_list, "note_decoder_fwd_grammar: inference only (training buffers or row bookkeeping given)");
    A2S_REQUIRE(a2s_grammar_ref_ok(g, a.R, a.V), "note_decoder_fwd_grammar: needs a table of 1..127 states, row states and V <= 256 (got %d states, V = %d)", g.n_states, a.V);
    A2S_REQUIRE(a.R > 0 && a.steps >= 0 && a.n_done && a.eos_seen && a.lengths && a.logits && a.probs, "note_decoder_fwd_grammar: null bookkeeping or output buffers");
    return note_decoder_fwd(st, a, steps_done, &g);
}

int a2s_note_decoder_fwd_align_impl(hipStream_t st, const NoteDecArgs& a, const a2s_align_args& g, int* steps_done) {
    A2S_REQUIRE(!a.gates && !a.attw && !a.drop && !a.n_active && !a.row_list && !a.m_active && !a.clip_order && !a.row_until,
                "note_decoder_fwd_align: inference only (training buffers or row bookkeeping given)");
    A2S_REQUIRE(!(a.gt && (g.next_state || g.n_states || g.row_state)), "note_decoder_fwd_align: a grammar constrains greedy decoding only (ground truth given)");
    A2S_REQUIRE(a.gt ? (a.tf_flags && a.poll == 0) : !a.tf_flags_dev, "note_decoder_fwd_align: a teacher-forced call needs tf_flags and poll = 0, a greedy call no device flags");
    A2S_REQUIRE(a.R > 0 && a.T >= 1 && a.steps >= 0 && a.n_done && a.eos_seen && a.lengths && a.logits && a.probs && a.h && a.x && a.q && a.o,
                "note_decoder_fwd_align: null bookkeeping or output buffers");
    A2S_REQUIRE(g.attw_step && g.peak && g.weight && g.centroid && g.out_stride >= a.steps && g.out_stride >= 1,
                "note_decoder_fwd_align: needs the one-step weights scratch, the three outputs and a row stride >= steps (got %ld for %d steps)", g.out_stride, a.steps);
    const bool with_grammar = g.next_state || g.n_states || g.row_state;
    const a2s_grammar_ref gr = {g.next_state, g.n_states, g.row_state};
    A2S_REQUIRE(!with_grammar || a2s_grammar_ref_ok(gr, a.R, a.V), "note_decoder_fwd_align: needs a table of 1..127 states, row states and V <= 256 (got %d states, V = %d)", g.n_states, a.V);
    return note_decoder_run(st, a, {.grammar = with_grammar ? &gr : nullptr, .align = &g, .label = "note_decoder_fwd_align"}, steps_done);
}

int a2s_note_decoder_fwd_beam_impl(hipStream_t st, const NoteDecArgs& a, const a2s_beam_args& g, int* steps_done) {
    A2S_REQUIRE(!a.gt && !a.tf_flags_dev, "note_decoder_fwd_beam: greedy decoding only (ground truth given)");
    A2S_REQUIRE(!a.gates && !a.attw && !a.drop && !a.n_active && !a.row_list && !a.m_active && !a.clip_order && !a.row_until,
                "note_decoder_fwd_beam: inference only (training buffers or row bookkeeping given)");
    A2S_REQUIRE(a2s_beam_args_ok(g, a.R, a.n_clips, a.V), "note_decoder_fwd_beam: needs 1 <= K <= %d, R = K * n_clips, V <= 256, a table of 1..127 states or none, and "
                "every beam buffer (got K = %d, R = %d, n_clips = %d, V = %d, %d states)", A2S_BEAM_MAX, g.K, a.R, a.n_clips, a.V, g.n_states);
    A2S_REQUIRE(g.ids_out && g.lengths_out && g.score_out, "note_decoder_fwd_beam: null output buffers");
    A2S_REQUIRE(a.steps >= 0 && a.n_done && a.logits && a.probs && a.h && a.x && a.q && a.o, "note_decoder_fwd_beam: null bookkeeping or output buffers");
    int rc = a2s_beam_init_impl(st, g, a.n_done, a.n_clips, a.steps);
    if (rc) return rc;
    int s = 0;
    rc = note_decoder_run(st, a, {.beam = &g, .parity_slots = true, .label = "note_decoder_fwd_beam"}, &s);
    if (rc) return rc;
    const BeamBackArgs bk = {g.score, g.token_hist, g.parent_hist, g.probs_scratch, a.probs, a.probs_bstride, g.ids_out, (long)a.steps, g.lengths_out, g.score_out,
                             a.steps_exec, g.alpha, a.n_clips, g.K, a.V, a.steps, a.eos_id, g.pad_id};
    if (a.steps > 0) { rc = a2s_beam_backtrack_impl(st, bk); if (rc) return rc; }
    if (steps_done) *steps_done = s;
    return A2S_OK;
}

int a2s_pair_events(const char* who, hipEvent_t** ev_out) {
    struct Pair { hipEvent_t ev[2]; };
    static thread_local std::vector<Pair> pairs;
    int dev = 0;
    hipError_t e = hipGetDevice(&dev);
    if (e != hipSuccess) A2S_FAIL(A2S_ERR_HIP, "%s: hipGetDevice: %s", who, hipGetErrorString(e));
    if ((size_t)dev >= pairs.size()) pairs.resize(dev + 1, Pair{{nullptr, nullptr}});
    for (int k = 0; k < 2; ++k)
        if (!pairs[dev].ev[k]) { e = hipEventCreateWithFlags(&pairs[dev].ev[k], hipEventDisableTiming); if (e != hipSuccess) A2S_FAIL(A2S_ERR_HIP, "%s: hipEventCreate: %s", who, hipGetErrorString(e)); }
    *ev_out = pairs[dev].ev;
    return A2S_OK;
}

int a2s_note_decoder_fwd_pair_impl(hipStream_t su, hipStream_t sl, const NoteDecArgs& au, const NoteDecArgs& al, const int* pair_order,
                                   const int* pair_rank, const int* pair_n_active, int* done_u, int* done_l) {
    const NoteDecArgs* as[2] = {&au, &al};
    hipStream_t sts[2] = {su, sl};
    const bool can_pair = a2s_sw(A2S_SW_attn_pair) && su != sl && pair_order && pair_rank && pair_n_active && au.gt && al.gt && au.n_active && al.n_active &&
                          au.n_clips > 0 && au.n_clips == al.n_clips && au.R == al.R && au.T == al.T && au.H == 256 && al.H == 256 && au.enc == al.enc &&
                          au.attn_ws && al.attn_ws && !a2s_note_decoder_fwd_persist_ok(au) && !a2s_note_decoder_fwd_persist_ok(al) &&
                          note_step_mid(au, nullptr) && note_step_mid(al, nullptr);
    if (!can_pair) {
        int rc = a2s_note_decoder_fwd_impl(su, au, done_u);
        return rc ? rc : a2s_note_decoder_fwd_impl(sl, al, done_l);
    }
    const NoteStepMode m = {.few_row = true, .fused_rows_limit = a2s_attn_pair_fused_rows(), .label = "note_decoder_fwd_pair"};
    hipEvent_t* ev = nullptr;
    { const int rc = a2s_pair_events(m.label, &ev); if (rc) return rc; }
    for (int k = 0; k < 2; ++k)
        if (note_decoder_tail_rows(*as[k])) { const int rc = a2s_note_decoder_zero_unwritten(sts[k], *as[k], "note_decoder"); if (rc) return rc; }
    bool prev_q[2] = {false, false};
    const int nmax = au.steps > al.steps ? au.steps : al.steps;
    for (int s = 0; s < nmax; ++s) {
        bool fused[2] = {false, false}, in[2];
        for (int k = 0; k < 2; ++k) {
            in[k] = s < as[k]->steps;
            if (!in[k]) continue;
            fused[k] = note_step_fusable(*as[k], s, m.fused_rows_limit);
            if (!prev_q[k]) { const int rc = enqueue_query(sts[k], *as[k], s, s); if (rc) return rc; }
            prev_q[k] = true;
        }
        AttnPairStep p = {pair_order, pair_rank, au.n_clips, pair_n_active[s], s, 1, au.T};
        const bool joint = in[0] && in[1] && !fused[0] && !fused[1] && p.n_active > 0 && au.n_active[s] > 0 && al.n_active[s] > 0;
        if (joint) {
            int rc = a2s_record_wait(ev[1], sl, su, m.label);
            if (rc == A2S_OK) rc = attn_pair_sweep(su, au, al, s, p);
            if (rc == A2S_OK) rc = a2s_record_wait(ev[0], su, sl, m.label);
            if (rc) return rc;
        }
        for (int k = 0; k < 2; ++k) {
            if (!in[k]) continue;
            const int rc = enqueue_note_step(sts[k], *as[k], m, note_step_at(*as[k], m, s, fused[k], joint ? &p : nullptr));
            if (rc) return rc;
        }
    }
    if (done_u) *done_u = au.steps;
    if (done_l) *done_l = al.steps;
    return A2S_OK;
}

__global__ __launch_bounds__(128) void staff_emb_fwd(const float* __restrict__ note_emb, const float* __restrict__ w_ih_f,
                                                     const float* __restrict__ w_hh_f, const float* __restrict__ b_ih_f,
                                                     const float* __restrict__ b_hh_f, const float* __restrict__ w_ih_r,
                                                     const float* __restrict__ w_hh_r, const float* __restrict__ b_ih_r,
                                                     const float* __restrict__ b_hh_r, const long long* __restrict__ ids64,
                                                     const int* __restrict__ ids32, long id_bstride,
                                                     const long long* __restrict__ lengths, long len_stride,
                                                     float* __restrict__ out, long ldo, int col0, float* __restrict__ hsave,
                                                     int maxlen, int E, int S) {
    extern __shared__ float sm[];
    const int b = blockIdx.x, dir = blockIdx.y, tid = threadIdx.x;
    const float* w_ih = dir ? w_ih_r : w_ih_f; const float* w_hh = dir ? w_hh_r : w_hh_f;
    const float* b_ih = dir ? b_ih_r : b_ih_f; const float* b_hh = dir ? b_hh_r : b_hh_f;
    float* Wi = sm;
    float* Wh = Wi + 3 * S * E;
    float* bi = Wh + 3 * S * S;
    float* bh = bi + 3 * S;
    float* h = bh + 3 * S;
    float* xe = h + S;
    float* g = xe + E;
    for (int i = tid; i < 3 * S * E; i += blockDim.x) Wi[i] = w_ih[i];
    for (int i = tid; i < 3 * S * S; i += blockDim.x) Wh[i] = w_hh[i];
    for (int i = tid; i < 3 * S; i += blockDim.x) { bi[i] = b_ih[i]; bh[i] = b_hh[i]; }
    for (int i = tid; i < S; i += blockDim.x) h[i] = 0.f;
    int len = (int)lengths[(long)b * len_stride];
    len = max(0, min(len, maxlen));
    __syncthreads();
    for (int s = 0; s < len; ++s) {
        const int t = dir ? len - 1 - s : s;
        const long id = ids64 ? ids64[(long)b * id_bstride + t] : ids32[(long)b * id_bstride + t];
        for (int i = tid; i < E; i += blockDim.x) xe[i] = note_emb[id * E + i];
        __syncthreads();
        for (int r = tid; r < 6 * S; r += blockDim.x) {
            float acc;
            if (r < 3 * S) { acc = bi[r]; for (int k = 0; k < E; ++k) acc = fmaf(Wi[r * E + k], xe[k], acc); }
            else { const int rr = r - 3 * S; acc = bh[rr]; for (int k = 0; k < S; ++k) acc = fmaf(Wh[rr * S + k], h[k], acc); }
            g[r] = acc;
        }
        __syncthreads();
        if (tid < S) {
            const float rg = fast_sigmoid(g[tid] + g[3 * S + tid]);
            const float zg = fast_sigmoid(g[S + tid] + g[4 * S + tid]);
            const float ng = fast_tanh(g[2 * S + tid] + rg * g[5 * S + tid]);
            const float hn = (1.f - zg) * ng + zg * h[tid];
            h[tid] = hn;
            if (hsave) hsave[(((long)b * 2 + dir) * maxlen + s) * S + tid] = hn;
        }
        __syncthreads();
    }
    for (int i = tid; i < S; i += blockDim.x) out[(long)b * ldo + col0 + dir * S + i] = h[i];
}

__global__ __launch_bounds__(192) void staff_emb_fwd_e16s32(const float* __restrict__ note_emb, const float* __restrict__ w_ih_f,
                                                            const float* __restrict__ w_hh_f, const float* __restrict__ b_ih_f,
                                                            const float* __restrict__ b_hh_f, const float* __restrict__ w_ih_r,
                                                            const float* __restrict__ w_hh_r, const float* __restrict__ b_ih_r,
                                                            const float* __restrict__ b_hh_r, const long long* __restrict__ ids64,
                                                            const int* __restrict__ ids32, long id_bstride,
                                                            const long long* __restrict__ lengths, long len_stride,
                                                            float* __restrict__ out, long ldo, int col0, float* __restrict__ hsave, int maxlen) {
    constexpr int E = 16, S = 32;
    extern __shared__ __attribute__((aligned(16))) float sm[];
    float* xe = sm;
    float* hb = xe + E;
    float* g = hb + S;
    int* lid = reinterpret_cast<int*>(g + 6 * S);
    const int b = blockIdx.x, dir = blockIdx.y, tid = threadIdx.x;
    const bool gi_role = tid < 3 * S;
    const int r = gi_role ? tid : tid - 3 * S;
    const float* wsrc = gi_role ? (dir ? w_ih_r : w_ih_f) + r * E : (dir ? w_hh_r : w_hh_f) + r * S;
    float w[S];
#pragma unroll
    for (int k = 0; k < S; ++k) w[k] = (gi_role && k >= E) ? 0.f : wsrc[k];
    const float bias = gi_role ? (dir ? b_ih_r : b_ih_f)[r] : (dir ? b_hh_r : b_hh_f)[r];
    int len = (int)lengths[(long)b * len_stride];
    len = max(0, min(len, maxlen));
    for (int i = tid; i < len; i += 192) {
        const int t = dir ? len - 1 - i : i;
// ... 531 lines not shown
        q4[j] = on[j] ? *reinterpret_cast<const f32x4*>(q + ((long)j * n_clips + b) * ldq + lane * 4) : (f32x4){0.f, 0.f, 0.f, 0.f};
    const f32x4 v4 = {v[lane * 4], v[lane * 4 + 1], v[lane * 4 + 2], v[lane * 4 + 3]};
#pragma unroll
    for (int j = 0; j < NQ; ++j)
#pragma unroll
        for (int c = 0; c < 4; ++c) q4[j][c] = exp2x_clamped(q4[j][c]);
#pragma unroll
    for (int u = 0; u < KF; ++u) {
        const int f = wave + 8 * u;
#pragma unroll
        for (int j = 0; j < NQ; ++j) {
            if (!on[j]) continue;
            float sj = v4[0] * tanh_ek(k[u][0], q4[j][0]) + v4[1] * tanh_ek(k[u][1], q4[j][1])
                     + v4[2] * tanh_ek(k[u][2], q4[j][2]) + v4[3] * tanh_ek(k[u][3], q4[j][3]);
            sj = wave_sum_lane63(sj);
            if (lane == 63 && f < n) pw[j * chunk + f] = sj;
        }
    }
    __syncthreads();
    float mj[NQ], lj[NQ];
#pragma unroll
    for (int j = 0; j < NQ; ++j) {
        mj[j] = 0.f; lj[j] = 0.f;
        if (!on[j]) continue;
        const float sc = tid < n ? pw[j * chunk + tid] : -INFINITY;
        const float m = block_max(sc, red);
        const float p = tid < n ? __expf(sc - m) : 0.f;
        if (tid < n) {
            if (scores) scores[((long)j * n_clips + b) * T + t0 + tid] = sc;
            pw[j * chunk + tid] = p;
        }
        lj[j] = block_sum(p, red);
        mj[j] = m;
    }
    __syncthreads();
    f32x4 acc[NQ];
#pragma unroll
    for (int j = 0; j < NQ; ++j) acc[j] = (f32x4){0.f, 0.f, 0.f, 0.f};
#pragma unroll
    for (int m = 0; m < ER; ++m) {
        const int i = rp + 4 * m;
        if (i < n) {
#pragma unroll
            for (int j = 0; j < NQ; ++j) {
                if (!on[j]) continue;
                const float w = pw[j * chunk + i];
#pragma unroll
                for (int c = 0; c < 4; ++c) acc[j][c] = fmaf(w, e[m][c], acc[j][c]);
            }
        }
    }
    f32x4* red4 = reinterpret_cast<f32x4*>(red + 16);
    if (rp > 0) {
#pragma unroll
        for (int j = 0; j < NQ; ++j) red4[(j * 3 + rp - 1) * 128 + c4] = acc[j];
    }
    __syncthreads();
#pragma unroll
    for (int j = 0; j < NQ; ++j) {
        if (!on[j]) continue;
        float* pout = partial + (((long)slot * NQ + j) * G + g) * (2 * H + 4);
        if (rp == 0) {
            f32x4 a = acc[j];
#pragma unroll
            for (int w = 0; w < 3; ++w) {
                const f32x4 o = red4[(j * 3 + w) * 128 + c4];
#pragma unroll
                for (int c = 0; c < 4; ++c) a[c] += o[c];
            }
            *reinterpret_cast<f32x4*>(pout + 4 + c4 * 4) = a;
        }
        if (tid == 0) { pout[0] = mj[j]; pout[1] = lj[j]; }
    }
}
template <int NQ>
static void launch_fwd_deep(hipStream_t st, int nwg, const float* Kmat, const float* enc, const float* q, long ldq, const float* v, float* ws, float* attw,
                            int T, int G, int chunk, const a2s_attn_rows& r) {
    const size_t shm = ((size_t)NQ * chunk + 16 + (size_t)NQ * 3 * 128 * 4) * sizeof(float);
    hipLaunchKernelGGL((attn_fwd_split256_deep<NQ>), dim3(nwg), dim3(512), shm, st, Kmat, enc, q, ldq, v, ws, attw, T, G, chunk, r.clip_order, r.row_until, r.step,
                       r.n_clips);
}


__global__ __launch_bounds__(256) void attn_fwd_combine256(const float* __restrict__ partial, float* __restrict__ ctx, long ldctx,
                                                           float* __restrict__ ctx2, long ldctx2, float* __restrict__ attw, int T, int G,
                                                           const int* __restrict__ n_done, int n_rows_total,
                                                           const int* __restrict__ clip_rank, const int* __restrict__ row_until,
                                                           int n_clips, int groups, int n_active, int step) {
    if (n_done && *n_done >= n_rows_total) return;
    constexpr int H = 256;
    const int b = blockIdx.x;
    const int clip = b % n_clips, grp = b / n_clips;
    const int slot = clip_rank ? clip_rank[clip] : clip;
    if (slot >= n_active || (row_until && step >= row_until[b])) {
        attn_zero_row(AttnCombineOut{ctx + (long)b * ldctx, ctx2 ? ctx2 + (long)b * ldctx2 : nullptr, attw ? attw + (long)b * T : nullptr, T});
        return;
    }
    __shared__ float wgt[80];
    attn_combine_row(partial + ((long)slot * groups + grp) * G * (2 * H + 4), G,
                     AttnCombineOut{ctx + (long)b * ldctx, ctx2 ? ctx2 + (long)b * ldctx2 : nullptr, attw ? attw + (long)b * T : nullptr, T}, wgt);
}

size_t a2s_attn_workspace_floats_impl(int B, int T, int H, int groups) {
    size_t rows = 0;
    for (int n = 1; n <= B; ++n) {
        int G, chunk;
        a2s_attn_split_geometry(n, T, &G, &chunk);
        if ((size_t)n * G > rows) rows = (size_t)n * G;
    }
    return A2S_ATTN_TICKETS + rows * (groups > 0 ? groups : 1) * (2 * H + 4);
}

size_t a2s_attn_bulk_lds(size_t shm, int n_active, int backward) {
    if (!a2s_sw(A2S_SW_attn_bulk_cap)) return shm;
    const size_t c = (backward & 1) ? 28672 : 65536;
    return (n_active >= 64 && c > shm) ? c : shm;
}
template <int NQ>
static void launch_fwd_mq(hipStream_t st, int nwg, size_t shm, const float* Kmat, const float* enc, const float* q, long ldq, const float* v,
                          float* ws, float* attw, int T, int G, int chunk, const a2s_attn_rows& r, const AttnFusedTail& ft, bool nt) {
    if (nt && shm > 65536) {
        static bool raised = false;
        if (!raised) { (void)hipFuncSetAttribute(reinterpret_cast<const void*>(attn_fwd_split256_mq<NQ, true>), hipFuncAttributeMaxDynamicSharedMemorySize, 98304); raised = true; }
    }
    if (nt) hipLaunchKernelGGL((attn_fwd_split256_mq<NQ, true>), dim3(nwg), dim3(256), shm, st, Kmat, enc, q, ldq, v, ws, attw, T, G, chunk,
                               r.clip_order, r.row_until, r.step, r.n_clips, ft);
    else hipLaunchKernelGGL((attn_fwd_split256_mq<NQ, false>), dim3(nwg), dim3(256), shm, st, Kmat, enc, q, ldq, v, ws, attw, T, G, chunk,
                            r.clip_order, r.row_until, r.step, r.n_clips, ft);
}

static int attn_step_fwd_split_impl(hipStream_t st, const float* Kmat, const float* enc, const float* q, long ldq, const float* v,
                                 float* ctx, long ldctx, float* ctx2, long ldctx2, float* attw, float* ws, int B, int T, int H,
                                 const int* n_done, int n_rows_total, const a2s_attn_rows* rows, a2s_attn_deferred* defer) {
    A2S_REQUIRE(H == 256 && ws, "attn_step_fwd_split: needs hidden_size 256 and a workspace");
    A2S_REQUIRE(ldq % 4 == 0 && ((uintptr_t)q % 16 == 0) && ((uintptr_t)Kmat % 16 == 0) && ((uintptr_t)enc % 16 == 0), "attn_step_fwd_split: 16-byte alignment");
    a2s_attn_rows r = {nullptr, nullptr, nullptr, B, B, 0};
    if (rows) r = *rows;
    A2S_REQUIRE(r.n_clips > 0 && B % r.n_clips == 0, "attn_step_fwd_split: rows (%d) must be a multiple of the clips (%d)", B, r.n_clips);
    const int groups = B / r.n_clips;
    A2S_REQUIRE(groups <= A2S_ATTN_MAX_GROUPS, "attn_step_fwd_split: at most %d fused bars (got %d)", A2S_ATTN_MAX_GROUPS, groups);
    A2S_REQUIRE(r.n_active >= 0 && r.n_active <= r.n_clips && (!r.clip_order || r.clip_rank), "attn_step_fwd_split: bad row compaction");
    A2S_REQUIRE(groups == 1 || !n_done, "attn_step_fwd_split: fused bars are a training-only path");
    A2S_REQUIRE(a2s_attn_max_split() <= 64, "attn_step_fwd_split: the split must be <= 64");
    int G = 1, chunk = T;
    int* tickets = reinterpret_cast<int*>(ws);
    float* part = ws + A2S_ATTN_TICKETS;
    const int fmode = a2s_sw(A2S_SW_attn_fused_combine);
    const bool fused = fmode && (fmode == 1 || r.n_active <= fmode) && r.n_clips <= A2S_ATTN_TICKETS / 2;
    const int n_zero = fused ? r.n_clips - r.n_active : 0;
    const AttnFusedTail ft = {fused ? tickets : nullptr, ctx, ldctx, ctx2, ldctx2, r.n_active, B};
    const bool nt = a2s_sw(A2S_SW_attn_nt) > 0 && r.n_active >= a2s_sw(A2S_SW_attn_nt);
    if (r.n_active > 0 || n_zero > 0) {
        if (r.n_active > 0) a2s_attn_split_geometry(r.n_active, T, &G, &chunk);
        const int nwg = r.n_active * G + n_zero;
        if (!fused && !n_done && groups <= 4 && r.n_active <= a2s_sw(A2S_SW_attn_deep) && chunk <= 80) {
            switch (groups) {
                case 1: launch_fwd_deep<1>(st, nwg, Kmat, enc, q, ldq, v, part, attw, T, G, chunk, r); break;
                case 2: launch_fwd_deep<2>(st, nwg, Kmat, enc, q, ldq, v, part, attw, T, G, chunk, r); break;
                case 3: launch_fwd_deep<3>(st, nwg, Kmat, enc, q, ldq, v, part, attw, T, G, chunk, r); break;
                default: launch_fwd_deep<4>(st, nwg, Kmat, enc, q, ldq, v, part, attw, T, G, chunk, r); break;
            }
        } else if (groups == 1) {
            const size_t shm = a2s_attn_bulk_lds((chunk + 16 + 128 * 4) * sizeof(float), r.n_active, 0);
            if (nt && shm > 65536) {
                static bool raised = false;
                if (!raised) { (void)hipFuncSetAttribute(reinterpret_cast<const void*>(attn_fwd_split256<true>), hipFuncAttributeMaxDynamicSharedMemorySize, 98304); raised = true; }
            }
            if (nt) hipLaunchKernelGGL(attn_fwd_split256<true>, dim3(nwg), dim3(256), shm, st, Kmat, enc, q, ldq, v, part, attw, T, G, chunk, n_done, n_rows_total, r.clip_order, ft);
            else hipLaunchKernelGGL(attn_fwd_split256<false>, dim3(nwg), dim3(256), shm, st, Kmat, enc, q, ldq, v, part, attw, T, G, chunk, n_done, n_rows_total, r.clip_order, ft);
        } else {
            const size_t shm = a2s_attn_bulk_lds(((size_t)groups * chunk + 16 + (size_t)groups * 128 * 4) * sizeof(float), r.n_active, 2);
            switch (groups) {
                case 2: launch_fwd_mq<2>(st, nwg, shm, Kmat, enc, q, ldq, v, part, attw, T, G, chunk, r, ft, nt); break;
                case 3: launch_fwd_mq<3>(st, nwg, shm, Kmat, enc, q, ldq, v, part, attw, T, G, chunk, r, ft, nt); break;
                case 4: launch_fwd_mq<4>(st, nwg, shm, Kmat, enc, q, ldq, v, part, attw, T, G, chunk, r, ft, nt); break;
                default: launch_fwd_mq<5>(st, nwg, shm, Kmat, enc, q, ldq, v, part, attw, T, G, chunk, r, ft, nt); break;
            }
        }
        A2S_CHECK_LAUNCH("attn_fwd_split256");
    }
    if (fused) return A2S_OK;
    if (defer && !n_done && r.n_active > 0 && r.n_active <= a2s_sw(A2S_SW_attn_deep) && groups <= 4 && G <= 16 && a2s_sw(A2S_SW_attn_defer_combine)) {
        *defer = a2s_attn_deferred{part, attw, r.clip_rank, r.row_until, G, groups, r.n_clips, r.n_active, r.step, T};
        return A2S_OK;
    }
    hipLaunchKernelGGL(attn_fwd_combine256, dim3(B), dim3(256), 0, st, part, ctx, ldctx, ctx2, ldctx2, attw, T, G, n_done, n_rows_total,
                       r.clip_rank, r.row_until, r.n_clips, groups, r.n_active, r.step);
    A2S_CHECK_LAUNCH("attn_fwd_combine256");
    return A2S_OK;
}

static long g_attn_pair_launches = 0;
long a2s_attn_pair_launches(void) { return g_attn_pair_launches; }

template <int NQ>
static void launch_fwd_pair(hipStream_t st, int nwg, size_t shm, const AttnPairSide& s0, const AttnPairSide& s1, const float* enc, long ldq, int T,
                            const AttnPairStep& p, bool nt) {
    if (nt && shm > 65536) {
        static bool raised = false;
        if (!raised) { (void)hipFuncSetAttribute(reinterpret_cast<const void*>(attn_fwd_split256_pair<NQ, true>), hipFuncAttributeMaxDynamicSharedMemorySize, 98304); raised = true; }
    }
    if (nt) hipLaunchKernelGGL((attn_fwd_split256_pair<NQ, true>), dim3(nwg), dim3(256), shm, st, s0, s1, enc, ldq, T, p.G, p.chunk, p.clip_order, p.step, p.n_clips);
    else hipLaunchKernelGGL((attn_fwd_split256_pair<NQ, false>), dim3(nwg), dim3(256), shm, st, s0, s1, enc, ldq, T, p.G, p.chunk, p.clip_order, p.step, p.n_clips);
}

static int attn_pair_sweep(hipStream_t st, const NoteDecArgs& au, const NoteDecArgs& al, int sv, AttnPairStep& p) {
    const int T = au.T, H = au.H, groups = au.R / p.n_clips;
    A2S_REQUIRE(H == 256 && au.attn_ws && al.attn_ws && au.enc == al.enc && au.R == al.R && au.T == al.T && groups >= 1 && groups <= A2S_ATTN_MAX_GROUPS,
                "attn_pair_sweep: the staves must decode the same rows over the same encoder outputs");
    a2s_attn_split_geometry(p.n_active, T, &p.G, &p.chunk);
    const AttnPairSide s0 = {au.keys, au.q + (long)sv * au.R * H, au.attn_v, au.attn_ws + A2S_ATTN_TICKETS, au.attw ? au.attw + (long)sv * au.R * T : nullptr, au.row_until};
    const AttnPairSide s1 = {al.keys, al.q + (long)sv * al.R * H, al.attn_v, al.attn_ws + A2S_ATTN_TICKETS, al.attw ? al.attw + (long)sv * al.R * T : nullptr, al.row_until};
    const bool nt = a2s_sw(A2S_SW_attn_nt) > 0 && p.n_active >= a2s_sw(A2S_SW_attn_nt);
    const size_t shm = a2s_attn_bulk_lds(((size_t)2 * groups * p.chunk + 16 + (size_t)2 * groups * 128 * 4) * sizeof(float), p.n_active, 2);
    const int nwg = p.n_active * p.G;
    switch (groups) {
        case 1: launch_fwd_pair<1>(st, nwg, shm, s0, s1, au.enc, H, T, p, nt); break;
        case 2: launch_fwd_pair<2>(st, nwg, shm, s0, s1, au.enc, H, T, p, nt); break;
        case 3: launch_fwd_pair<3>(st, nwg, shm, s0, s1, au.enc, H, T, p, nt); break;
        case 4: launch_fwd_pair<4>(st, nwg, shm, s0, s1, au.enc, H, T, p, nt); break;
        default: launch_fwd_pair<5>(st, nwg, shm, s0, s1, au.enc, H, T, p, nt); break;
    }
    A2S_CHECK_LAUNCH("attn_fwd_split256_pair");
    __atomic_fetch_add(&g_attn_pair_launches, 1, __ATOMIC_RELAXED);
    return A2S_OK;
}

static int attn_pair_combine(hipStream_t st, const NoteDecArgs& a, int si, int sv, const AttnPairStep& p) {
    const int H2 = 2 * a.H, ldx = a.E + H2;
    float* xs = a.x + (long)si * a.R * ldx;
    float* os = a.o + (long)sv * a.R * 2 * H2;
    hipLaunchKernelGGL(attn_fwd_combine256, dim3(a.R), dim3(256), 0, st, a.attn_ws + A2S_ATTN_TICKETS, xs + a.E, (long)ldx, os + H2, (long)(2 * H2),
                       a.attw ? a.attw + (long)sv * a.R * a.T : nullptr, a.T, p.G, (const int*)nullptr, a.R, p.clip_rank, a.row_until, p.n_clips,
                       a.R / p.n_clips, p.n_active, p.step);
    A2S_CHECK_LAUNCH("attn_fwd_combine256");
    return A2S_OK;
}
```

### piano_a2s_amd/csrc/a2s_step.hip

```cpp
#include "a2s_internal.h"
#include <type_traits>

#define NW 8
#ifndef DEC_CH_GRU
#define DEC_CH_GRU 1
#define DEC_CH_OUT 1
#define DEC_CH_PROD 1
#define DEC_CH_QUERY 1
#endif
#ifndef DEC_NW_PROD
#define DEC_NW_PROD 8
#define DEC_NW_OUT 8
#endif

template <int NT, int CH, int NWV = NW>
__device__ __forceinline__ void mfma_rows8(const float* __restrict__ arow, const float* const (&brow)[NT], int ksteps, int wave, int lk,
                                           f32x4 (&acc)[NT]) {
    for (int u0 = wave; u0 < ksteps; u0 += NWV * CH) {
        f32x4 a[CH], b[NT][CH];
#pragma unroll
        for (int c = 0; c < CH; ++c) {
            const int u = u0 + NWV * c;
            const bool ok = u < ksteps;
            a[c] = ok ? *reinterpret_cast<const f32x4*>(arow + 16 * u + 4 * lk) : (f32x4){0.f, 0.f, 0.f, 0.f};
// ... 189 lines not shown
            const float mg = have ? pb[(long)lane * CMB_PS] : -INFINITY, lg = have ? pb[(long)lane * CMB_PS + 1] : 0.f;
            float m, inv_l;
            const float wg = attn_merge_weight(mg, lg, have, m, inv_l);
            if (lane < 16) cw[i * 20 + lane] = wg;
            if (lane == 0) { cw[i * 20 + 16] = m; cw[i * 20 + 17] = inv_l; cw[i * 20 + 18] = 1.f; cbase[i] = base; }
        } else if (lane == 0) { cw[i * 20 + 18] = 0.f; cbase[i] = 0; }
    }
    __syncthreads();
    for (int i0 = 0; i0 < nb; i0 += 2) {
        float p[2][16];
#pragma unroll
        for (int rr = 0; rr < 2; ++rr) {
            const int i = min(i0 + rr, nb - 1);
            const bool on = cw[i * 20 + 18] != 0.f;
            const float* pb = c.part + (long)cbase[i] * c.G * CMB_PS + 4 + tid;
#pragma unroll
            for (int u = 0; u < 16; ++u) p[rr][u] = (on && u < c.G) ? pb[(long)u * CMB_PS] : 0.f;
        }
#pragma unroll
        for (int rr = 0; rr < 2; ++rr) {
            const int i = i0 + rr;
            if (i >= nb) break;
            float acc = 0.f;
#pragma unroll
            for (int u = 0; u < 16; ++u) acc = fmaf(p[rr][u], cw[i * 20 + u], acc);
            ctxs[i * CMB_LD + tid] = acc;
        }
    }
    __syncthreads();
    if ((int)blockIdx.x < nb) {
        const int i = blockIdx.x;
        const long row = dec_row(a.rowmap, row0 + i);
        const float v = ctxs[i * CMB_LD + tid];
        c.xw[row * a.ldx + c.E + tid] = v;
        a.o[row * a.ldo + H2 + tid] = v;
    } else if ((int)blockIdx.x >= 16 && (int)blockIdx.x - 16 < nb && c.attw) {
        const int i = blockIdx.x - 16;
        float* aw = c.attw + (long)dec_row(a.rowmap, row0 + i) * c.T;
        const bool on = cw[i * 20 + 18] != 0.f;
        const float m = cw[i * 20 + 16], inv = cw[i * 20 + 17];
        float sv[4];
#pragma unroll
        for (int u = 0; u < 4; ++u) sv[u] = (on && tid + 64 * NW * u < c.T) ? aw[tid + 64 * NW * u] : 0.f;
#pragma unroll
        for (int u = 0; u < 4; ++u) if (tid + 64 * NW * u < c.T) aw[tid + 64 * NW * u] = on ? __expf(sv[u] - m) * inv : 0.f;
        for (int t = tid + 4 * 64 * NW; t < c.T; t += 64 * NW) aw[t] = on ? __expf(aw[t] - m) * inv : 0.f;
    }
    const int arow_i = dec_row(a.rowmap, min(row0 + li, R - 1));
    const float* lrow = ctxs + min(li, nb - 1) * CMB_LD;
    const float* bi[3];
    const float* bh[3];
#pragma unroll
    for (int g = 0; g < 3; ++g) { bi[g] = a.w_ih + ((long)g * H2 + j0 + li) * a.kx; bh[g] = a.w_hh + ((long)g * H2 + j0 + li) * H2; }
    f32x4 t[3], u[3];
#pragma unroll
    for (int g = 0; g < 3; ++g) t[g] = (f32x4){0.f, 0.f, 0.f, 0.f};
    mfma_rows8_split<3, DEC_CH_GRU>(a.x + (long)arow_i * a.ldx, c.E / 16, lrow, bi, a.kx / 16, wave, lk, t);
    u[0] = t[0]; u[1] = t[1]; u[2] = (f32x4){0.f, 0.f, 0.f, 0.f};
    mfma_rows8<3, DEC_CH_GRU>(a.h + (long)arow_i * H2, bh, H2 / 16, wave, lk, u);
    f32x4 acc[4] = {u[0], u[1], t[2], u[2]};
    reduce_waves<4>(acc, part, wave, lane);
    if (wave > 0) return;
#pragma unroll
    for (int r = 0; r < 4; ++r) {
        if (row0 + lk * 4 + r >= R) continue;
        const int row = dec_row(a.rowmap, row0 + lk * 4 + r);
        const GruCellOut cell = gru_cell(acc[0][r], acc[1][r], acc[2][r], acc[3][r], br, bz, bin, bhn, hp[r]);
        const float rg = cell.rg, zg = cell.zg, ng = cell.ng, ghn = cell.ghn, hn = cell.hn;
        a.hout[(long)row * H2 + j] = hn;
        a.o[(long)row * a.ldo + j] = hn;
        if (a.save) {
            float* sv = a.save + (long)row * 4 * H2;
            sv[j] = rg; sv[H2 + j] = zg; sv[2 * H2 + j] = ng; sv[3 * H2 + j] = ghn;
        }
    }
}

#define MID_KC 64
#define MID_LDB 72
#ifndef MID_WAVES
#define MID_WAVES 4
#define MID_AHEAD 1
#endif
__global__ __launch_bounds__(256, MID_WAVES) void dec_gru_mid(DecGruArgs a) {
    __shared__ __attribute__((aligned(16))) float bs[2][48 * MID_LDB];
    const int tid = threadIdx.x, lane = tid & 63, wave = tid >> 6;
    if (a.n_done) {
        const bool done = *a.n_done >= a.R;
        if (blockIdx.x == 0 && blockIdx.y == 0 && tid == 0) *a.skip = done ? 1 : 0;
        if (done) return;
    }
    const int H2 = a.H2, R = a.R, kx = a.kx;
    const int j0 = blockIdx.x * 16, row0 = blockIdx.y * 64 + wave * 16;
    const int li = lane & 15, lk = lane >> 4;
    const int j = j0 + li;
    const int ncx = (kx + MID_KC - 1) / MID_KC, nc = ncx + (H2 + MID_KC - 1) / MID_KC;
    const float br = a.b_ih[j] + a.b_hh[j], bz = a.b_ih[H2 + j] + a.b_hh[H2 + j], bin = a.b_ih[2 * H2 + j], bhn = a.b_hh[2 * H2 + j];
    float hp[4];
#pragma unroll
    for (int r = 0; r < 4; ++r) hp[r] = a.h[(long)dec_row(a.rowmap, min(row0 + lk * 4 + r, R - 1)) * H2 + j];
    const int arow = dec_row(a.rowmap, min(row0 + li, R - 1));
    const float* const xa = a.x + (long)arow * a.ldx + 4 * lk;
    const float* const ha = a.h + (long)arow * H2 + 4 * lk;
    const f32x4 zero4 = {0.f, 0.f, 0.f, 0.f};
    auto bload = [&](int c, f32x4 (&v)[3]) {
        const bool px = c < ncx;
        const int k0 = (px ? c : c - ncx) * MID_KC, K = px ? kx : H2;
        const float* const W = px ? a.w_ih : a.w_hh;
#pragma unroll
        for (int i = 0; i < 3; ++i) {
            const int e = tid + 256 * i, r = e >> 4, k = k0 + 4 * (e & 15);
            v[i] = k < K ? *reinterpret_cast<const f32x4*>(W + ((long)(r >> 4) * H2 + j0 + (r & 15)) * K + k) : zero4;
        }
    };
    auto bstore = [&](int buf, const f32x4 (&v)[3]) {
#pragma unroll
        for (int i = 0; i < 3; ++i) {
            const int e = tid + 256 * i;
            *reinterpret_cast<f32x4*>(&bs[buf][(e >> 4) * MID_LDB + 4 * (e & 15)]) = v[i];
        }
    };
    auto aload = [&](int c, f32x4 (&v)[4]) {
        const bool px = c < ncx;
        const int k0 = (px ? c : c - ncx) * MID_KC, K = px ? kx : H2;
        const float* const p = px ? xa : ha;
#pragma unroll
        for (int u = 0; u < 4; ++u) v[u] = (k0 + 16 * u < K) ? *reinterpret_cast<const f32x4*>(p + k0 + 16 * u) : zero4;
    };
    f32x4 acc[4] = {zero4, zero4, zero4, zero4};
    auto compute = [&](auto PX, int c, int buf, const f32x4 (&av)[4]) {
        constexpr bool px = decltype(PX)::value;
        const int k0 = (px ? c : c - ncx) * MID_KC, K = px ? kx : H2;
#pragma unroll
        for (int u = 0; u < 4; ++u) {
            if (k0 + 16 * u >= K) break;
            f32x4 b[3];
#pragma unroll
            for (int g = 0; g < 3; ++g) b[g] = *reinterpret_cast<const f32x4*>(&bs[buf][(g * 16 + li) * MID_LDB + 16 * u + 4 * lk]);
#pragma unroll
            for (int jj = 0; jj < 4; ++jj) {
                acc[0] = __builtin_amdgcn_mfma_f32_16x16x4f32(av[u][jj], b[0][jj], acc[0], 0, 0, 0);
                acc[1] = __builtin_amdgcn_mfma_f32_16x16x4f32(av[u][jj], b[1][jj], acc[1], 0, 0, 0);
                acc[px ? 2 : 3] = __builtin_amdgcn_mfma_f32_16x16x4f32(av[u][jj], b[2][jj], acc[px ? 2 : 3], 0, 0, 0);
            }
        }
    };
    f32x4 bv[3], a_cur[4], a_n1[4], a_n2[4];
    bload(0, bv);
    aload(0, a_cur);
    if (MID_AHEAD > 1 && nc > 1) aload(1, a_n1);
    bstore(0, bv);
    if (nc > 1) bload(1, bv);
    __syncthreads();
    for (int c = 0; c < nc; ++c) {
#if MID_AHEAD > 1
        if (c + 2 < nc) aload(c + 2, a_n2);
#else
        if (c + 1 < nc) aload(c + 1, a_n1);
#endif
        if (c + 1 < nc) {
            bstore((c + 1) & 1, bv);
            if (c + 2 < nc) bload(c + 2, bv);
        }
        if (c < ncx) compute(std::true_type{}, c, c & 1, a_cur);
        else compute(std::false_type{}, c, c & 1, a_cur);
        __syncthreads();
#pragma unroll
        for (int u = 0; u < 4; ++u) { a_cur[u] = a_n1[u]; if (MID_AHEAD > 1) a_n1[u] = a_n2[u]; }
    }
#pragma unroll
    for (int r = 0; r < 4; ++r) {
        if (row0 + lk * 4 + r >= R) continue;
        const int row = dec_row(a.rowmap, row0 + lk * 4 + r);
        const GruCellOut cell = gru_cell(acc[0][r], acc[1][r], acc[2][r], acc[3][r], br, bz, bin, bhn, hp[r]);
        a.hout[(long)row * H2 + j] = cell.hn;
        a.o[(long)row * a.ldo + j] = cell.hn;
        if (a.save) {
            float* sv = a.save + (long)row * 4 * H2;
            sv[j] = cell.rg; sv[H2 + j] = cell.zg; sv[2 * H2 + j] = cell.ng; sv[3 * H2 + j] = cell.ghn;
        }
    }
}

#define NTV 11
#define NVW 6
struct DecOutArgs {
    const float* o; long ldo; int ko;
    const float* out_w; const float* out_b;
    float* logits; long ldl;
    int* tickets;
    float* probs; long probs_bstride;
    const long long* gt; long gt_bstride;
    const float* emb; float* xnext; long ldx;
    const uint8_t* drop; float inv_keep;
    int* argmax_out; long am_bstride;
    int* eos_seen; long long* lengths; int* n_done; int* steps_exec;
    const int* t_base; const int* row_until; const int* skip;
    const float* hnew; const float* attn_w; long ld_aw; const float* attn_b; float* q_next; int H;
    const int* rowmap;
    int n_clips, R, V, E, t, teacher_force, eos_id, max_t, H2;
};

__device__ __forceinline__ void dec_row_epilogue(const DecOutArgs& a, int vrow, int t, int lane) {
    const volatile float* lg = a.logits + (long)vrow * a.ldl;
    const int row = dec_row(a.rowmap, vrow);
    const bool finished = a.row_until && t >= a.row_until[row];
    float v[3];
    float m = -INFINITY; int mi = 0x7fffffff;
#pragma unroll
    for (int k = 0; k < 3; ++k) {
        const int j = lane + 64 * k;
        v[k] = j < a.V ? lg[j] : -INFINITY;
        if (v[k] > m) { m = v[k]; mi = j; }
    }
#pragma unroll
    for (int o = 32; o > 0; o >>= 1) {
        const float om = __shfl_xor(m, o, 64); const int oi = __shfl_xor(mi, o, 64);
        if (om > m || (om == m && oi < mi)) { m = om; mi = oi; }
    }
    if (!finished) {
        float s = 0.f;
#pragma unroll
        for (int k = 0; k < 3; ++k) if (lane + 64 * k < a.V) s += expf(v[k] - m);
        s = wave_sum(s);
        const float lse = m + logf(s);
        float* pr = a.probs + (long)row * a.probs_bstride + (long)t * a.V;
#pragma unroll
        for (int k = 0; k < 3; ++k) if (lane + 64 * k < a.V) pr[lane + 64 * k] = v[k] - lse;
    }
    const long long gtok = a.gt ? a.gt[(long)row * a.gt_bstride + t] : -1;
    const int tf = (a.teacher_force >> (a.n_clips > 0 ? row / a.n_clips : 0)) & 1;
    const int next_id = (a.gt && tf) ? (int)gtok : mi;
    for (int j = lane; j < a.E; j += 64) {
        float e = a.emb[(long)next_id * a.E + j];
        if (a.drop) e = a.drop[(long)row * a.E + j] ? e * a.inv_keep : 0.f;
        a.xnext[(long)row * a.ldx + j] = e;
    }
    if (lane == 0 && !finished) {
        if (row == 0 && a.steps_exec) *a.steps_exec = t + 1;
        if (a.argmax_out) a.argmax_out[(long)row * a.am_bstride + t] = mi;
        const bool hit = a.gt ? (gtok == a.eos_id) : (mi == a.eos_id);
        if (hit) {
            if (!a.eos_seen[row]) { a.eos_seen[row] = 1; atomicAdd(a.n_done, 1); }
            a.lengths[row] = t + 1;
        }
    }
}

__global__ __launch_bounds__(64 * DEC_NW_OUT) void dec_out_step(DecOutArgs a) {
    __shared__ f32x4 part[(DEC_NW_OUT / 2) * 2 * 64];
    __shared__ int last_flag;
    const int tid = threadIdx.x, lane = tid & 63, wave = tid >> 6;
    if (a.skip && *a.skip) return;
    const int t = a.t + (a.t_base ? *a.t_base : 0);
    if (t >= a.max_t) return;
    const int R = a.R, row0 = blockIdx.x * 16;
    const int li = lane & 15, lk = lane >> 4;
    const bool vocab = (int)blockIdx.y < NVW;
    if (!vocab && !a.q_next) return;
    const int n0 = (vocab ? blockIdx.y : blockIdx.y - NVW) * 32;
    const int ncols = vocab ? a.V : a.H;
    const float* Bm = vocab ? a.out_w : a.attn_w;
    const long ldb = vocab ? (long)a.ko : a.ld_aw;
    const int K = vocab ? a.ko : a.H2;
    const float* brow[2];
// ... 66 lines not shown
    if (wave == 0 && !role_a) {
#pragma unroll
        for (int g = 0; g < 2; ++g)
#pragma unroll
            for (int r = 0; r < 4; ++r) c0[g][r] = a.dh[(long)dec_row(a.rowmap, min(row0 + lk * 4 + r, R - 1)) * a.H2 + min(n0 + g * 16 + li, ncols - 1)];
    }
    f32x4 acc[2] = {(f32x4){0.f, 0.f, 0.f, 0.f}, (f32x4){0.f, 0.f, 0.f, 0.f}};
    mfma_rows8<2, DEC_CH_PROD, DEC_NW_PROD>(A + (long)dec_row(a.rowmap, min(row0 + li, R - 1)) * K, brow, K / 16, wave, lk, acc);
    reduce_waves<2, DEC_NW_PROD>(acc, part, wave, lane);
    if (wave > 0) return;
#pragma unroll
    for (int g = 0; g < 2; ++g) {
        const int col = n0 + g * 16 + li;
        if (col >= ncols) continue;
#pragma unroll
        for (int r = 0; r < 4; ++r) {
            if (row0 + lk * 4 + r >= R) continue;
            const int row = dec_row(a.rowmap, row0 + lk * 4 + r);
            if (role_a) a.dx[(long)row * a.ldx + col] = acc[g][r];
            else a.dh[(long)row * a.H2 + col] = c0[g][r] + acc[g][r];
        }
    }
}


__device__ __forceinline__ void mid_product_64x32(const float* __restrict__ ar, const float* __restrict__ Bt, long ldb, int n0, int ncols, int K,
                                                  float (*bs)[32 * MID_LDB], f32x4 (&acc)[2]) {
    const int tid = threadIdx.x, lane = tid & 63, li = lane & 15, lk = lane >> 4;
    const int nc = K / MID_KC;
    const f32x4 zero4 = {0.f, 0.f, 0.f, 0.f};
    auto bload = [&](int c, f32x4 (&v)[2]) {
#pragma unroll
        for (int i = 0; i < 2; ++i) {
            const int e = tid + 256 * i, n = n0 + (e >> 4);
            v[i] = n < ncols ? *reinterpret_cast<const f32x4*>(Bt + (long)n * ldb + c * MID_KC + 4 * (e & 15)) : zero4;
        }
    };
    auto bstore = [&](int buf, const f32x4 (&v)[2]) {
#pragma unroll
        for (int i = 0; i < 2; ++i) {
            const int e = tid + 256 * i;
            *reinterpret_cast<f32x4*>(&bs[buf][(e >> 4) * MID_LDB + 4 * (e & 15)]) = v[i];
        }
    };
    auto aload = [&](int c, f32x4 (&v)[4]) {
#pragma unroll
        for (int u = 0; u < 4; ++u) v[u] = *reinterpret_cast<const f32x4*>(ar + c * MID_KC + 16 * u);
    };
    f32x4 bv[2], a_cur[4], a_n1[4], a_n2[4];
    bload(0, bv);
    aload(0, a_cur);
    if (MID_AHEAD > 1 && nc > 1) aload(1, a_n1);
    bstore(0, bv);
    if (nc > 1) bload(1, bv);
    __syncthreads();
    for (int c = 0; c < nc; ++c) {
#if MID_AHEAD > 1
        if (c + 2 < nc) aload(c + 2, a_n2);
#else
        if (c + 1 < nc) aload(c + 1, a_n1);
#endif
        if (c + 1 < nc) {
            bstore((c + 1) & 1, bv);
            if (c + 2 < nc) bload(c + 2, bv);
        }
        const float* const bb = bs[c & 1];
#pragma unroll
        for (int u = 0; u < 4; ++u) {
            f32x4 b[2];
#pragma unroll
            for (int g = 0; g < 2; ++g) b[g] = *reinterpret_cast<const f32x4*>(&bb[(g * 16 + li) * MID_LDB + 16 * u + 4 * lk]);
#pragma unroll
            for (int jj = 0; jj < 4; ++jj) {
                acc[0] = __builtin_amdgcn_mfma_f32_16x16x4f32(a_cur[u][jj], b[0][jj], acc[0], 0, 0, 0);
                acc[1] = __builtin_amdgcn_mfma_f32_16x16x4f32(a_cur[u][jj], b[1][jj], acc[1], 0, 0, 0);
            }
        }
        __syncthreads();
#pragma unroll
        for (int u = 0; u < 4; ++u) { a_cur[u] = a_n1[u]; if (MID_AHEAD > 1) a_n1[u] = a_n2[u]; }
    }
}

__global__ __launch_bounds__(256, MID_WAVES) void dec_bwd_mid(DecBwdProdArgs a) {
    __shared__ __attribute__((aligned(16))) float bs[2][32 * MID_LDB];
    const int lane = threadIdx.x & 63, wave = threadIdx.x >> 6;
    const int li = lane & 15, lk = lane >> 4;
    const int R = a.R, K = 3 * a.H2, row0 = blockIdx.y * 64 + wave * 16;
    const bool role_a = (int)blockIdx.x < a.nxa;
    const int n0 = (role_a ? blockIdx.x : blockIdx.x - a.nxa) * 32;
    const int ncols = role_a ? a.kx : a.H2;
    float c0[2][4];
    if (!role_a) {
#pragma unroll
        for (int g = 0; g < 2; ++g)
#pragma unroll
            for (int r = 0; r < 4; ++r) c0[g][r] = a.dh[(long)dec_row(a.rowmap, min(row0 + lk * 4 + r, R - 1)) * a.H2 + min(n0 + g * 16 + li, ncols - 1)];
    }
    f32x4 acc[2] = {(f32x4){0.f, 0.f, 0.f, 0.f}, (f32x4){0.f, 0.f, 0.f, 0.f}};
    mid_product_64x32((role_a ? a.dgi : a.dgh) + (long)dec_row(a.rowmap, min(row0 + li, R - 1)) * K + 4 * lk, role_a ? a.wih_t : a.whh_t, K, n0, ncols, K, bs, acc);
#pragma unroll
    for (int g = 0; g < 2; ++g) {
        const int col = n0 + g * 16 + li;
        if (col >= ncols) continue;
#pragma unroll
        for (int r = 0; r < 4; ++r) {
            if (row0 + lk * 4 + r >= R) continue;
            const int row = dec_row(a.rowmap, row0 + lk * 4 + r);
            if (role_a) a.dx[(long)row * a.ldx + col] = acc[g][r];
            else a.dh[(long)row * a.H2 + col] = c0[g][r] + acc[g][r];
        }
    }
}

__global__ __launch_bounds__(256, MID_WAVES) void dec_bwd_query_mid(const float* __restrict__ dq, const float* __restrict__ wh_t, float* __restrict__ dh, int R, int H, int H2,
                                                         const int* __restrict__ rowmap) {
    __shared__ __attribute__((aligned(16))) float bs[2][32 * MID_LDB];
    const int lane = threadIdx.x & 63, wave = threadIdx.x >> 6;
    const int li = lane & 15, lk = lane >> 4;
    const int row0 = blockIdx.y * 64 + wave * 16, n0 = blockIdx.x * 32;
    float c0[2][4];
#pragma unroll
    for (int g = 0; g < 2; ++g)
#pragma unroll
        for (int r = 0; r < 4; ++r) c0[g][r] = dh[(long)dec_row(rowmap, min(row0 + lk * 4 + r, R - 1)) * H2 + min(n0 + g * 16 + li, H2 - 1)];
    f32x4 acc[2] = {(f32x4){0.f, 0.f, 0.f, 0.f}, (f32x4){0.f, 0.f, 0.f, 0.f}};
    mid_product_64x32(dq + (long)dec_row(rowmap, min(row0 + li, R - 1)) * H + 4 * lk, wh_t, H, n0, H2, H, bs, acc);
#pragma unroll
    for (int g = 0; g < 2; ++g) {
        const int col = n0 + g * 16 + li;
        if (col >= H2) continue;
#pragma unroll
        for (int r = 0; r < 4; ++r) {
            if (row0 + lk * 4 + r >= R) continue;
            const int row = dec_row(rowmap, row0 + lk * 4 + r);
            dh[(long)row * H2 + col] = c0[g][r] + acc[g][r];
        }
    }
}

struct DecOutqMidArgs {
    const float* o; long ldo;
    const float* out_w; const float* out_b; float* logits; long ldl; int V;
    const float* attn_w; long ld_aw; const float* attn_b; float* q_next; int H;
    const int* rowmap;
    int nva, R, H2;
};
__global__ __launch_bounds__(256, MID_WAVES) void dec_outq_mid(DecOutqMidArgs a) {
    __shared__ __attribute__((aligned(16))) float bs[2][32 * MID_LDB];
    const int lane = threadIdx.x & 63, wave = threadIdx.x >> 6;
    const int li = lane & 15, lk = lane >> 4;
    const int R = a.R, row0 = blockIdx.y * 64 + wave * 16;
    const bool role_a = (int)blockIdx.x < a.nva;
    const int n0 = (role_a ? blockIdx.x : blockIdx.x - a.nva) * 32;
    const int ncols = role_a ? a.V : a.H;
    float bias[2];
#pragma unroll
    for (int g = 0; g < 2; ++g) bias[g] = (role_a ? a.out_b : a.attn_b)[min(n0 + g * 16 + li, ncols - 1)];
    f32x4 acc[2] = {(f32x4){0.f, 0.f, 0.f, 0.f}, (f32x4){0.f, 0.f, 0.f, 0.f}};
    mid_product_64x32(a.o + (long)dec_row(a.rowmap, min(row0 + li, R - 1)) * a.ldo + 4 * lk, role_a ? a.out_w : a.attn_w, role_a ? 2L * a.H2 : a.ld_aw, n0, ncols,
                      role_a ? 2 * a.H2 : a.H2, bs, acc);
#pragma unroll
    for (int g = 0; g < 2; ++g) {
        const int col = n0 + g * 16 + li;
        if (col >= ncols) continue;
#pragma unroll
        for (int r = 0; r < 4; ++r) {
            if (row0 + lk * 4 + r >= R) continue;
            const int row = dec_row(a.rowmap, row0 + lk * 4 + r);
            if (role_a) a.logits[(long)row * a.ldl + col] = acc[g][r] + bias[g];
            else a.q_next[(long)row * a.H + col] = acc[g][r] + bias[g];
        }
    }
}

__global__ __launch_bounds__(64 * NW) void dec_bwd_query(const float* __restrict__ dq, const float* __restrict__ wh_t, float* __restrict__ dh,
                                                         int R, int H, int H2, const int* __restrict__ rowmap) {
    __shared__ f32x4 part[4 * 2 * 64];
    const int tid = threadIdx.x, lane = tid & 63, wave = tid >> 6;
    const int li = lane & 15, lk = lane >> 4;
    const int row0 = blockIdx.y * 16, n0 = blockIdx.x * 32;
    const float* brow[2];
#pragma unroll
    for (int g = 0; g < 2; ++g) brow[g] = wh_t + (long)min(n0 + g * 16 + li, H2 - 1) * H;
    float c0[2][4];
    if (wave == 0) {
#pragma unroll
        for (int g = 0; g < 2; ++g)
#pragma unroll
            for (int r = 0; r < 4; ++r) c0[g][r] = dh[(long)dec_row(rowmap, min(row0 + lk * 4 + r, R - 1)) * H2 + min(n0 + g * 16 + li, H2 - 1)];
    }
    f32x4 acc[2] = {(f32x4){0.f, 0.f, 0.f, 0.f}, (f32x4){0.f, 0.f, 0.f, 0.f}};
    mfma_rows8<2, DEC_CH_QUERY>(dq + (long)dec_row(rowmap, min(row0 + li, R - 1)) * H, brow, H / 16, wave, lk, acc);
    reduce_waves<2>(acc, part, wave, lane);
    if (wave > 0) return;
#pragma unroll
    for (int g = 0; g < 2; ++g) {
        const int col = n0 + g * 16 + li;
        if (col >= H2) continue;
#pragma unroll
        for (int r = 0; r < 4; ++r) {
            if (row0 + lk * 4 + r < R) dh[(long)dec_row(rowmap, row0 + lk * 4 + r) * H2 + col] = c0[g][r] + acc[g][r];
        }
    }
}

__global__ void transpose_ld(const float* __restrict__ in, long ld, float* __restrict__ out, int rows, int cols) {
    const long i = (long)blockIdx.x * blockDim.x + threadIdx.x;
    if (i >= (long)rows * cols) return;
    const int c = (int)(i / rows), r = (int)(i % rows);
    out[i] = in[(long)r * ld + c];
}

#define FUSED_MAX_ROWS_CAP 2048
#define FUSED_HEAD (16 + FUSED_MAX_ROWS_CAP / 16 + (long)FUSED_MAX_ROWS_CAP * 16 * NTV)
size_t a2s_note_step_fused_head_floats(void) { return (size_t)FUSED_HEAD; }
size_t a2s_note_step_workspace_floats_impl(int H, int E) {
    const long H2 = 2L * H, kx = E + H2;
    return (size_t)(FUSED_HEAD + kx * 3 * H2 + H2 * 3 * H2 + H2 * H);
}
static bool aligned16(const void* p) { return ((uintptr_t)p & 15) == 0; }
static int g_dec_mid_launches = 0;
int a2s_dec_mid_launches(void) { return g_dec_mid_launches; }
static bool dec_use_mid(int nrows, int H2) { return a2s_sw(A2S_SW_dec_mid) && nrows > 160 && H2 % MID_KC == 0; }
bool a2s_dec_step_fusable(int R, int H, int E, int V, const void* const* ptrs, int nptrs, const float* ws, size_t ws_floats, bool greedy) {
    const int max_rows = greedy ? FUSED_MAX_ROWS_CAP : a2s_sw(A2S_SW_dec_fused_max_rows);
    if (!a2s_sw(A2S_SW_dec_fused) || R > max_rows || R > FUSED_MAX_ROWS_CAP || !ws || ws_floats < a2s_note_step_workspace_floats_impl(H, E)) return false;
    if (H % 16 || E % 16 || (V + 15) / 16 != NTV || !aligned16(ws)) return false;
    for (int i = 0; i < nptrs; ++i) if (!aligned16(ptrs[i])) return false;
    return true;
}

int a2s_note_step_fused_fwd(hipStream_t st, const a2s_note_dec_args& a, int si, int so, int sv, int sv_next, int t, const int* t_base, int tf, bool last,
                            int nrows, const int* rowmap, const a2s_attn_deferred* defer) {
    const int H2 = 2 * a.H, ldx = a.E + H2, R = a.R;
    int* flags = reinterpret_cast<int*>(a.step_ws);
    const bool greedy = a.gt == nullptr;
    DecGruArgs g;
    g.x = a.x + (long)si * R * ldx; g.ldx = ldx; g.kx = ldx;
    g.h = a.h + (long)si * R * H2;
    g.w_ih = a.w_ih; g.w_hh = a.w_hh; g.b_ih = a.b_ih; g.b_hh = a.b_hh;
    g.hout = a.h + (long)so * R * H2; g.o = a.o + (long)sv * R * 2 * H2; g.ldo = 2 * H2;
    g.save = a.gates ? a.gates + (long)sv * R * 4 * H2 : nullptr;
    g.n_done = greedy ? a.n_done : nullptr; g.skip = flags;
    g.rowmap = rowmap;
    g.R = nrows; g.H2 = H2;
    if (defer && defer->G > 0) {
        A2S_REQUIRE(H2 == 64 * NW && defer->G <= 16 && a.E % 16 == 0, "note_step_fused_fwd: deferred combine needs 2 * hidden_size == %d and G <= 16", 64 * NW);
        DecCmbArgs c;
        c.part = defer->part; c.attw = defer->attw; c.xw = a.x + (long)si * R * ldx;
        c.clip_rank = defer->clip_rank; c.row_until = defer->row_until;
        c.G = defer->G; c.groups = defer->groups; c.n_clips = defer->n_clips; c.n_active = defer->n_active; c.step = defer->step; c.T = defer->T;
        c.Rall = R; c.E = a.E;
        hipLaunchKernelGGL(dec_gru_step_cmb, dim3(H2 / 16, a2s_cdiv(nrows, 16)), dim3(64 * NW), dec_cmb_lds_bytes(nrows < 16 ? nrows : 16), st, g, c);
    } else
    if (dec_use_mid(nrows, H2)) { hipLaunchKernelGGL(dec_gru_mid, dim3(H2 / 16, a2s_cdiv(nrows, 64)), dim3(256), 0, st, g); __atomic_fetch_add(&g_dec_mid_launches, 1, __ATOMIC_RELAXED); }
    else hipLaunchKernelGGL(dec_gru_step, dim3(H2 / 16, a2s_cdiv(nrows, 16)), dim3(64 * NW), 0, st, g);
    A2S_CHECK_LAUNCH("dec_gru_step");
    DecOutArgs f;
    f.o = g.o; f.ldo = 2 * H2; f.ko = 2 * H2; f.out_w = a.out_w; f.out_b = a.out_b;
    f.tickets = flags + 16; f.logits = a.step_ws + 16 + FUSED_MAX_ROWS_CAP / 16; f.ldl = 16 * NTV;
    f.probs = a.probs; f.probs_bstride = a.probs_bstride; f.gt = a.gt; f.gt_bstride = a.gt_bstride;
    f.emb = a.emb; f.xnext = a.x + (long)so * R * ldx; f.ldx = ldx;
    f.drop = a.drop ? a.drop + (long)so * R * a.E : nullptr; f.inv_keep = a.inv_keep;
    f.argmax_out = a.argmax_out; f.am_bstride = a.am_bstride;
    f.eos_seen = a.eos_seen; f.lengths = a.lengths; f.n_done = a.n_done; f.steps_exec = a.steps_exec;
    f.t_base = t_base; f.row_until = a.n_active ? a.row_until : nullptr; f.skip = greedy ? flags : nullptr;
    f.hnew = g.hout; f.attn_w = a.attn_w; f.ld_aw = 2 * H2; f.attn_b = a.attn_b;
    f.q_next = last ? nullptr : a.q + (long)sv_next * R * a.H; f.H = a.H;
    f.rowmap = rowmap;
    f.n_clips = a.n_clips > 0 ? a.n_clips : R; f.R = nrows; f.V = a.V; f.E = a.E; f.t = t; f.teacher_force = tf; f.eos_id = a.eos_id;
    f.max_t = a.steps; f.H2 = H2;
    hipLaunchKernelGGL(dec_out_step, dim3(a2s_cdiv(nrows, 16), NVW + a2s_cdiv(a.H, 32)), dim3(64 * DEC_NW_OUT), 0, st, f);
    A2S_CHECK_LAUNCH("dec_out_step");
    return A2S_OK;
}

int a2s_note_step_fused_bwd_prepare(hipStream_t st, const a2s_note_dec_bwd_args& a) {
    const int H2 = 2 * a.H, kx = a.E + H2;
    float* wih_t = a.step_ws + FUSED_HEAD;
    float* whh_t = wih_t + (long)kx * 3 * H2;
    float* wh_t = whh_t + (long)H2 * 3 * H2;
    hipLaunchKernelGGL(transpose_ld, dim3(a2s_cdiv((long)3 * H2 * kx, 256)), dim3(256), 0, st, a.w_ih, (long)kx, wih_t, 3 * H2, kx);
    hipLaunchKernelGGL(transpose_ld, dim3(a2s_cdiv((long)3 * H2 * H2, 256)), dim3(256), 0, st, a.w_hh, (long)H2, whh_t, 3 * H2, H2);
    hipLaunchKernelGGL(transpose_ld, dim3(a2s_cdiv((long)a.H * H2, 256)), dim3(256), 0, st, a.attn_w, (long)2 * H2, wh_t, a.H, H2);
    A2S_CHECK_LAUNCH("transpose_ld");
    return A2S_OK;
}

int a2s_note_step_fused_bwd(hipStream_t st, const a2s_note_dec_bwd_args& a, int s, const float* dh_in, float* dh_out, const a2s_attn_rows* rows,
                            int nrows, const int* rowmap) {
    const int H2 = 2 * a.H, ldx = a.E + H2, R = a.R;
    const float* dos = a.do_all + (long)s * R * 2 * H2;
    float* dgi = a.dgi_all + (long)s * R * 3 * H2;
    float* dgh = a.dgh_all + (long)s * R * 3 * H2;
    float* dxs = a.dx + (long)s * R * ldx;
    float* wih_t = a.step_ws + FUSED_HEAD;
    float* whh_t = wih_t + (long)ldx * 3 * H2;
    float* wh_t = whh_t + (long)H2 * 3 * H2;
    DecBwdProdArgs p;
    p.dgi = dgi; p.dgh = dgh; p.wih_t = wih_t; p.whh_t = whh_t; p.dx = dxs; p.ldx = ldx; p.dh = dh_out;
    p.rowmap = rowmap;
    p.nxa = a2s_cdiv(ldx, 32); p.kx = ldx; p.R = nrows; p.H2 = H2;
    const bool mid = dec_use_mid(nrows, H2);
    int rc = a2s_gru_gates_bwd_impl(st, dh_in, H2, dos, 2 * H2, a.gates + (long)s * R * 4 * H2, a.h + (long)s * R * H2, H2,
                                    dgi, 3 * H2, dgh, 3 * H2, nullptr, 0, dh_out, H2, R, H2);
    if (rc) return rc;
    if (mid) { hipLaunchKernelGGL(dec_bwd_mid, dim3(p.nxa + a2s_cdiv(H2, 32), a2s_cdiv(nrows, 64)), dim3(256), 0, st, p); __atomic_fetch_add(&g_dec_mid_launches, 1, __ATOMIC_RELAXED); }
    else hipLaunchKernelGGL(dec_bwd_products, dim3(p.nxa + a2s_cdiv(H2, 32), a2s_cdiv(nrows, 16)), dim3(64 * DEC_NW_PROD), 0, st, p);
    A2S_CHECK_LAUNCH("dec_bwd_products");
    rc = a2s_attn_step_bwd_impl(st, a.keys, a.enc, a.q + (long)s * R * a.H, a.H, a.attn_v, a.attw + (long)s * R * a.T,
                                a.x + (long)s * R * ldx + a.E, ldx, dxs + a.E, ldx, dos + H2, 2 * H2,
                                a.dctx_all + (long)s * R * H2, H2, a.dq_all + (long)s * R * a.H, a.H,
                                a.ds_all + (long)s * R * a.T, R, a.T, a.H, a.attn_ws, rows);
    if (rc) return rc;
    if (mid) hipLaunchKernelGGL(dec_bwd_query_mid, dim3(a2s_cdiv(H2, 32), a2s_cdiv(nrows, 64)), dim3(256), 0, st, a.dq_all + (long)s * R * a.H, wh_t, dh_out, nrows, a.H, H2, rowmap);
    else hipLaunchKernelGGL(dec_bwd_query, dim3(a2s_cdiv(H2, 32), a2s_cdiv(nrows, 16)), dim3(64 * NW), 0, st, a.dq_all + (long)s * R * a.H, wh_t, dh_out, nrows, a.H, H2,
                            rowmap);
    A2S_CHECK_LAUNCH("dec_bwd_query");
    return A2S_OK;
}


bool a2s_note_step_mid_ok(int H, int E, const void* const* ptrs, int nptrs) {
    if (!a2s_sw(A2S_SW_dec_mid) || H % MID_KC || E % 16) return false;
    for (int i = 0; i < nptrs; ++i) if (!aligned16(ptrs[i])) return false;
    return true;
}
int a2s_note_step_mid_gru(hipStream_t st, const a2s_note_dec_args& a, int si, int so, int sv, int sv_next, int nrows, const int* rowmap) {
    const int H2 = 2 * a.H, ldx = a.E + H2, R = a.R;
    if (nrows <= 0) return A2S_OK;
    DecGruArgs g;
    g.x = a.x + (long)si * R * ldx; g.ldx = ldx; g.kx = ldx;
    g.h = a.h + (long)si * R * H2;
    g.w_ih = a.w_ih; g.w_hh = a.w_hh; g.b_ih = a.b_ih; g.b_hh = a.b_hh;
    g.hout = a.h + (long)so * R * H2; g.o = a.o + (long)sv * R * 2 * H2; g.ldo = 2 * H2;
    g.save = a.gates ? a.gates + (long)sv * R * 4 * H2 : nullptr;
    g.n_done = nullptr; g.skip = nullptr;
    g.rowmap = rowmap;
    g.R = nrows; g.H2 = H2;
    hipLaunchKernelGGL(dec_gru_mid, dim3(H2 / 16, a2s_cdiv(nrows, 64)), dim3(256), 0, st, g);
    __atomic_fetch_add(&g_dec_mid_launches, 1, __ATOMIC_RELAXED);
    A2S_CHECK_LAUNCH("dec_gru_mid");
    DecOutqMidArgs f;
    f.o = g.o; f.ldo = 2 * H2; f.out_w = a.out_w; f.out_b = a.out_b; f.logits = a.logits; f.ldl = a.V; f.V = a.V;
    f.attn_w = a.attn_w; f.ld_aw = 2 * H2; f.attn_b = a.attn_b; f.q_next = sv_next >= 0 ? a.q + (long)sv_next * R * a.H : nullptr; f.H = a.H;
    f.rowmap = rowmap;
    f.nva = a2s_cdiv(a.V, 32); f.R = nrows; f.H2 = H2;
    hipLaunchKernelGGL(dec_outq_mid, dim3(f.nva + (f.q_next ? a2s_cdiv(a.H, 32) : 0), a2s_cdiv(nrows, 64)), dim3(256), 0, st, f);
    A2S_CHECK_LAUNCH("dec_outq_mid");
    return A2S_OK;
}
bool a2s_note_step_mid_bwd_ok(const a2s_note_dec_bwd_args& a) {
    const void* ptrs[] = {a.dgi_all, a.dgh_all, a.dx, a.dh, a.step_ws};
    return a.step_ws && a.step_ws_floats >= a2s_note_step_workspace_floats_impl(a.H, a.E) && a2s_note_step_mid_ok(a.H, a.E, ptrs, 5);
}
int a2s_note_step_mid_bwd(hipStream_t st, const a2s_note_dec_bwd_args& a, int s, float* dh_out, int nrows, const int* rowmap) {
    const int H2 = 2 * a.H, ldx = a.E + H2, R = a.R;
    if (nrows <= 0) return A2S_OK;
    DecBwdProdArgs p;
    p.dgi = a.dgi_all + (long)s * R * 3 * H2; p.dgh = a.dgh_all + (long)s * R * 3 * H2;
    p.wih_t = a.step_ws + FUSED_HEAD; p.whh_t = p.wih_t + (long)ldx * 3 * H2;
    p.dx = a.dx + (long)s * R * ldx; p.ldx = ldx; p.dh = dh_out;
    p.rowmap = rowmap;
    p.nxa = a2s_cdiv(ldx, 32); p.kx = ldx; p.R = nrows; p.H2 = H2;
    hipLaunchKernelGGL(dec_bwd_mid, dim3(p.nxa + a2s_cdiv(H2, 32), a2s_cdiv(nrows, 64)), dim3(256), 0, st, p);
    __atomic_fetch_add(&g_dec_mid_launches, 1, __ATOMIC_RELAXED);
    A2S_CHECK_LAUNCH("dec_bwd_mid");
    return A2S_OK;
}
int a2s_note_step_mid_bwd_query(hipStream_t st, const a2s_note_dec_bwd_args& a, int s, float* dh_out, int nrows, const int* rowmap) {
    const int H2 = 2 * a.H, ldx = a.E + H2, R = a.R;
    if (nrows <= 0) return A2S_OK;
    const float* wh_t = a.step_ws + FUSED_HEAD + (long)ldx * 3 * H2 + (long)H2 * 3 * H2;
    hipLaunchKernelGGL(dec_bwd_query_mid, dim3(a2s_cdiv(H2, 32), a2s_cdiv(nrows, 64)), dim3(256), 0, st, a.dq_all + (long)s * R * a.H, wh_t, dh_out, nrows, a.H, H2, rowmap);
    A2S_CHECK_LAUNCH("dec_bwd_query_mid");
    return A2S_OK;
}
```

Before: 629.5.

## Batch both staff decoders into paired kernel launches on one stream

```diff
diff --git a/piano_a2s_amd/csrc/a2s_bwd.hip b/piano_a2s_amd/csrc/a2s_bwd.hip
--- a/piano_a2s_amd/csrc/a2s_bwd.hip
+++ b/piano_a2s_amd/csrc/a2s_bwd.hip
@@ -22,11 +22,16 @@
     return A2S_OK;
 }
 
-__global__ void gru_gates_bwd(const float* __restrict__ dh_a, long lda, const float* __restrict__ dh_b, long ldb,
-                              const float* __restrict__ save, const float* __restrict__ hprev, long ldhp,
-                              float* __restrict__ dgi, long ldgi, float* __restrict__ dgh, long ldgh,
-                              float* __restrict__ dgh2, long ldgh2, float* __restrict__ dhprev, long lddp, int R, int H) {
-    const long idx = (long)blockIdx.x * blockDim.x + threadIdx.x;
+struct GruGatesBwdArgs {
+    const float* dh_a; long lda; const float* dh_b; long ldb; const float* save; const float* hprev; long ldhp;
+    float* dgi; long ldgi; float* dgh; long ldgh; float* dgh2; long ldgh2; float* dhprev; long lddp; int R, H;
+};
+__device__ __forceinline__ void gru_gates_bwd_body(const GruGatesBwdArgs& g, int bx, int ) {
+    const float* __restrict__ dh_a = g.dh_a; const float* __restrict__ dh_b = g.dh_b; const float* __restrict__ save = g.save; const float* __restrict__ hprev = g.hprev;
+    float* __restrict__ dgi = g.dgi; float* __restrict__ dgh = g.dgh; float* __restrict__ dgh2 = g.dgh2; float* __restrict__ dhprev = g.dhprev;
+    const long lda = g.lda, ldb = g.ldb, ldhp = g.ldhp, ldgi = g.ldgi, ldgh = g.ldgh, ldgh2 = g.ldgh2, lddp = g.lddp;
+    const int R = g.R, H = g.H;
+    const long idx = (long)bx * blockDim.x + threadIdx.x;
     if (idx >= (long)R * H) return;
     const int r_ = (int)(idx / H), j = (int)(idx % H);
     const float* s = save + (long)r_ * 4 * H;
@@ -43,14 +48,18 @@
     if (dgh2) { float* c = dgh2 + (long)r_ * ldgh2; c[j] = dr; c[H + j] = dz; c[2 * H + j] = cg.dnr; }
     dhprev[(long)r_ * lddp + j] = cg.dhz;
 }
-
+__global__ void gru_gates_bwd(GruGatesBwdArgs g) { gru_gates_bwd_body(g, blockIdx.x, 0); }
+A2S_PAIR_KERNEL(gru_gates_bwd_pair, gru_gates_bwd_body, GruGatesBwdArgs, )
+
+static int gru_gates_bwd_launch(hipStream_t st, const GruGatesBwdArgs& g) {
+    hipLaunchKernelGGL(gru_gates_bwd, dim3(a2s_cdiv((long)g.R * g.H, 256)), dim3(256), 0, st, g);
+    A2S_CHECK_LAUNCH("gru_gates_bwd");
+    return A2S_OK;
+}
 int a2s_gru_gates_bwd_impl(hipStream_t st, const float* dh_a, long lda, const float* dh_b, long ldb, const float* save,
                            const float* hprev, long ldhp, float* dgi, long ldgi, float* dgh, long ldgh, float* dgh2, long ldgh2,
                            float* dhprev, long lddp, int R, int H) {
-    hipLaunchKernelGGL(gru_gates_bwd, dim3(a2s_cdiv((long)R * H, 256)), dim3(256), 0, st, dh_a, lda, dh_b, ldb, save, hprev, ldhp,
-                       dgi, ldgi, dgh, ldgh, dgh2, ldgh2, dhprev, lddp, R, H);
-    A2S_CHECK_LAUNCH("gru_gates_bwd");
-    return A2S_OK;
+    return gru_gates_bwd_launch(st, GruGatesBwdArgs{dh_a, lda, dh_b, ldb, save, hprev, ldhp, dgi, ldgi, dgh, ldgh, dgh2, ldgh2, dhprev, lddp, R, H});
 }
 
 __global__ __launch_bounds__(256) void attn_step_bwd(const float* __restrict__ Kmat, const float* __restrict__ enc,
@@ -422,7 +431,7 @@
 
 
 static int attn_pair_bwd_sweep(hipStream_t st, const a2s_note_dec_bwd_args& au, const a2s_note_dec_bwd_args& al, int s, AttnPairStep& p);
-static int attn_pair_bwd_combine(hipStream_t st, const a2s_note_dec_bwd_args& a, int s, const AttnPairStep& p);
+static int attn_pair_bwd_combine(hipStream_t st, const a2s_note_dec_bwd_args& au, const a2s_note_dec_bwd_args& al, int s, const AttnPairStep& p);
 
 struct NoteBwdStaff { bool mid = false; int cur = 0; int fused_rows_limit = -1; };
 static int note_bwd_step_rows(const a2s_note_dec_bwd_args& a, int s) { return (a.row_list && a.n_rows_active) ? a.n_rows_active[s] : a.R; }
@@ -433,7 +442,13 @@
     return n > 0 && a2s_dec_step_fusable(n, a.H, a.E, 173, ptrs, 8, a.step_ws, a.step_ws_floats);
 }
 
-static int note_bwd_step(hipStream_t st, const a2s_note_dec_bwd_args& a, int s, NoteBwdStaff& c, int part, const AttnPairStep* pair) {
+static GruGatesBwdArgs note_bwd_gates_args(const a2s_note_dec_bwd_args& a, int s, const float* dh_in, float* dh_out) {
+    const int H2 = 2 * a.H;
+    const long R = a.R;
+    return GruGatesBwdArgs{dh_in, H2, a.do_all + s * R * 2 * H2, 2 * H2, a.gates + s * R * 4 * H2, a.h + s * R * H2, H2, a.dgi_all + s * R * 3 * H2, 3 * H2,
+                           a.dgh_all + s * R * 3 * H2, 3 * H2, nullptr, 0, dh_out, H2, a.R, H2};
+}
+static int note_bwd_step(hipStream_t st, const a2s_note_dec_bwd_args& a, int s, NoteBwdStaff& c) {
     const int H2 = 2 * a.H, ldx = a.E + H2, R = a.R;
     const bool fused = note_bwd_step_fused(a, s, c.fused_rows_limit);
     a2s_attn_rows rows_v = {a.clip_order, a.clip_rank, a.row_until, a.n_clips > 0 ? a.n_clips : R, a.n_active ? a.n_active[s] : 0, s};
@@ -454,25 +469,19 @@
     float* dgi = a.dgi_all + (long)s * R * 3 * H2;
     float* dgh = a.dgh_all + (long)s * R * 3 * H2;
     float* dxs = a.dx + (long)s * R * ldx;
-    int rc = A2S_OK;
-    if (part != 2) {
-        rc = a2s_gru_gates_bwd_impl(st, dh_in, H2, dos, 2 * H2, a.gates + (long)s * R * 4 * H2, a.h + (long)s * R * H2, H2,
-                                    dgi, 3 * H2, dgh, 3 * H2, nullptr, 0, dh_out, H2, R, H2);
-        if (rc) return rc;
-        if (c.mid) {
-            const int nrows = note_bwd_step_rows(a, s);
-            rc = a2s_note_step_mid_bwd(st, a, s, dh_out, nrows, nrows < R ? a.row_list : nullptr);
-        } else {
-            rc = a2s_gemm_impl(st, gM, ldx, 3 * H2, 1.f, dgi, 3 * H2, 1, a.w_ih, ldx, 1, 0.f, dxs, ldx, nullptr, 0, gB, gS * 3 * H2, 0, gS * ldx, 0, a.gemm_ws, a.gemm_ws_bytes);
-        }
-        if (rc) return rc;
-        if (part == 1) return A2S_OK;
-    }
-    rc = pair ? attn_pair_bwd_combine(st, a, s, *pair)
-              : a2s_attn_step_bwd_impl(st, a.keys, a.enc, a.q + (long)s * R * a.H, a.H, a.attn_v, a.attw + (long)s * R * a.T,
-                                       a.x + (long)s * R * ldx + a.E, ldx, dxs + a.E, ldx, dos + H2, 2 * H2,
-                                       a.dctx_all + (long)s * R * H2, H2, a.dq_all + (long)s * R * a.H, a.H,
-                                       a.ds_all + (long)s * R * a.T, R, a.T, a.H, a.attn_ws, rows);
+    int rc = gru_gates_bwd_launch(st, note_bwd_gates_args(a, s, dh_in, dh_out));
+    if (rc) return rc;
+    if (c.mid) {
+        const int nrows = note_bwd_step_rows(a, s);
+        rc = a2s_note_step_mid_bwd(st, a, s, dh_out, nrows, nrows < R ? a.row_list : nullptr);
+    } else {
+        rc = a2s_gemm_impl(st, gM, ldx, 3 * H2, 1.f, dgi, 3 * H2, 1, a.w_ih, ldx, 1, 0.f, dxs, ldx, nullptr, 0, gB, gS * 3 * H2, 0, gS * ldx, 0, a.gemm_ws, a.gemm_ws_bytes);
+    }
+    if (rc) return rc;
+    rc = a2s_attn_step_bwd_impl(st, a.keys, a.enc, a.q + (long)s * R * a.H, a.H, a.attn_v, a.attw + (long)s * R * a.T,
+                                a.x + (long)s * R * ldx + a.E, ldx, dxs + a.E, ldx, dos + H2, 2 * H2,
+                                a.dctx_all + (long)s * R * H2, H2, a.dq_all + (long)s * R * a.H, a.H,
+                                a.ds_all + (long)s * R * a.T, R, a.T, a.H, a.attn_ws, rows);
     if (rc) return rc;
     if (!c.mid) {
         rc = a2s_gemm_impl(st, gM, H2, 3 * H2, 1.f, dgh, 3 * H2, 1, a.w_hh, H2, 1, 1.f, dh_out, H2, nullptr, 0, gB, gS * 3 * H2, 0, gS * H2, 0, a.gemm_ws, a.gemm_ws_bytes);
@@ -516,10 +525,36 @@
     int rc = note_bwd_prepare(st, a, c);
     if (rc) return rc;
     for (int s = a.steps - 1; s >= 0; --s) {
-        rc = note_bwd_step(st, a, s, c, 0, nullptr);
+        rc = note_bwd_step(st, a, s, c);
         if (rc) return rc;
     }
     return note_bwd_finish(st, a, c.cur);
+}
+
+static int note_bwd_step_pair(hipStream_t st, const a2s_note_dec_bwd_args* const as[2], int s, NoteBwdStaff (&cs)[2], AttnPairStep& p) {
+    GruGatesBwdArgs gg[2];
+    float* dh_out[2];
+    int nrows[2];
+    const int* rowmap[2];
+    for (int k = 0; k < 2; ++k) {
+        const a2s_note_dec_bwd_args& a = *as[k];
+        const long half = (long)a.R * 2 * a.H;
+        dh_out[k] = a.dh + (cs[k].cur ^ 1) * half;
+        gg[k] = note_bwd_gates_args(a, s, a.dh + cs[k].cur * half, dh_out[k]);
+        nrows[k] = note_bwd_step_rows(a, s);
+        rowmap[k] = nrows[k] < a.R ? a.row_list : nullptr;
+    }
+    const PairGrid g = {a2s_cdiv((long)gg[0].R * gg[0].H, 256), 1, a2s_cdiv((long)gg[1].R * gg[1].H, 256), 1};
+    hipLaunchKernelGGL(gru_gates_bwd_pair, a2s_pair_grid_dim(g), dim3(256), 0, st, gg[0], gg[1], g);
+    A2S_CHECK_LAUNCH("gru_gates_bwd_pair");
+    int rc = a2s_note_step_mid_bwd_pair(st, as, s, dh_out, nrows, rowmap);
+    if (rc == A2S_OK) rc = attn_pair_bwd_sweep(st, *as[0], *as[1], s, p);
+    if (rc == A2S_OK) rc = attn_pair_bwd_combine(st, *as[0], *as[1], s, p);
+    if (rc == A2S_OK) rc = a2s_note_step_mid_bwd_query_pair(st, as, s, dh_out, nrows, rowmap);
+    if (rc) return rc;
+    cs[0].cur ^= 1;
+    cs[1].cur ^= 1;
+    return A2S_OK;
 }
 
 int a2s_note_decoder_bwd_pair_impl(hipStream_t su, hipStream_t sl, const a2s_note_dec_bwd_args& au, const a2s_note_dec_bwd_args& al, const int* pair_order,
@@ -538,24 +573,23 @@
     { const int rc = a2s_pair_events(who, &ev); if (rc) return rc; }
     NoteBwdStaff cs[2] = {{.fused_rows_limit = a2s_attn_pair_fused_rows()}, {.fused_rows_limit = a2s_attn_pair_fused_rows()}};
     for (int k = 0; k < 2; ++k) { const int rc = note_bwd_prepare(sts[k], *as[k], cs[k]); if (rc) return rc; }
+    bool lower_on_su = false;
     const int nmax = au.steps > al.steps ? au.steps : al.steps;
     for (int s = nmax - 1; s >= 0; --s) {
         bool in[2], fused[2] = {false, false};
         for (int k = 0; k < 2; ++k) { in[k] = s < as[k]->steps; if (in[k]) fused[k] = note_bwd_step_fused(*as[k], s, cs[k].fused_rows_limit); }
         AttnPairStep p = {pair_order, pair_rank, au.n_clips, pair_n_active[s], s, 1, au.T};
         const bool joint = in[0] && in[1] && cs[0].mid && cs[1].mid && !fused[0] && !fused[1] && p.n_active > 0 && au.n_active[s] > 0 && al.n_active[s] > 0;
-        if (!joint) {
-            for (int k = 0; k < 2; ++k)
-                if (in[k]) { const int rc = note_bwd_step(sts[k], *as[k], s, cs[k], 0, nullptr); if (rc) return rc; }
+        if (in[1]) { const int rc = a2s_pair_handoff(ev, su, sl, lower_on_su, joint, who); if (rc) return rc; }
+        if (joint) {
+            const int rc = note_bwd_step_pair(su, as, s, cs, p);
+            if (rc) return rc;
             continue;
         }
-        for (int k = 0; k < 2; ++k) { const int rc = note_bwd_step(sts[k], *as[k], s, cs[k], 1, nullptr); if (rc) return rc; }
-        int rc = a2s_record_wait(ev[1], sl, su, who);
-        if (rc == A2S_OK) rc = attn_pair_bwd_sweep(su, au, al, s, p);
-        if (rc == A2S_OK) rc = a2s_record_wait(ev[0], su, sl, who);
-        if (rc) return rc;
-        for (int k = 0; k < 2; ++k) { const int rc2 = note_bwd_step(sts[k], *as[k], s, cs[k], 2, &p); if (rc2) return rc2; }
-    }
+        for (int k = 0; k < 2; ++k)
+            if (in[k]) { const int rc = note_bwd_step(sts[k], *as[k], s, cs[k]); if (rc) return rc; }
+    }
+    { const int rc = a2s_pair_handoff(ev, su, sl, lower_on_su, false, who); if (rc) return rc; }
     for (int k = 0; k < 2; ++k) { const int rc = note_bwd_finish(sts[k], *as[k], cs[k].cur); if (rc) return rc; }
     return A2S_OK;
 }
@@ -1350,11 +1384,16 @@
     }
 }
 
-__global__ __launch_bounds__(256) void attn_bwd_combine256(const float* __restrict__ dq_partial, float* __restrict__ dq, long lddq, int G,
-                                                           const int* __restrict__ clip_rank, const int* __restrict__ row_until,
-                                                           int n_clips, int groups, int n_active, int step, float* __restrict__ ds_out,
-                                                           int T, float* __restrict__ dctx_out, long lddo) {
-    const int b = blockIdx.x, j = threadIdx.x;
+struct AttnBwdCombineArgs {
+    const float* dq_partial; float* dq; long lddq; int G; const int* clip_rank; const int* row_until;
+    int n_clips, groups, n_active, step; float* ds_out; int T; float* dctx_out; long lddo;
+};
+__device__ __forceinline__ void attn_bwd_combine256_body(const AttnBwdCombineArgs& a, int bx, int ) {
+    const float* __restrict__ dq_partial = a.dq_partial; float* __restrict__ dq = a.dq; float* __restrict__ ds_out = a.ds_out; float* __restrict__ dctx_out = a.dctx_out;
+    const int* __restrict__ clip_rank = a.clip_rank; const int* __restrict__ row_until = a.row_until;
+    const long lddq = a.lddq, lddo = a.lddo;
+    const int G = a.G, n_clips = a.n_clips, groups = a.groups, n_active = a.n_active, step = a.step, T = a.T;
+    const int b = bx, j = threadIdx.x;
     const int clip = b % n_clips, grp = b / n_clips;
     const int slot = clip_rank ? clip_rank[clip] : clip;
     if (slot >= n_active || (row_until && step >= row_until[b])) {
@@ -1374,6 +1413,8 @@
     }
     dq[(long)b * lddq + j] = s;
 }
+__global__ __launch_bounds__(256) void attn_bwd_combine256(AttnBwdCombineArgs a) { attn_bwd_combine256_body(a, blockIdx.x, 0); }
+A2S_PAIR_KERNEL(attn_bwd_combine256_pair, attn_bwd_combine256_body, AttnBwdCombineArgs, __launch_bounds__(256))
 
 template <int NQ>
 static void launch_bwd_mq(hipStream_t st, int nwg, size_t shm, const float* Kmat, const float* enc, const float* q, long ldq, const float* v,
@@ -1435,8 +1476,8 @@
         }
         A2S_CHECK_LAUNCH("attn_bwd_split256");
     }
-    hipLaunchKernelGGL(attn_bwd_combine256, dim3(B), dim3(256), 0, st, ws, dq, lddq, G, r.clip_rank, r.row_until, r.n_clips, groups, r.n_active, r.step,
-                       ds_out, T, dctx_out, lddo);
+    hipLaunchKernelGGL(attn_bwd_combine256, dim3(B), dim3(256), 0, st,
+                       AttnBwdCombineArgs{ws, dq, lddq, G, r.clip_rank, r.row_until, r.n_clips, groups, r.n_active, r.step, ds_out, T, dctx_out, lddo});
     A2S_CHECK_LAUNCH("attn_bwd_combine256");
     return A2S_OK;
 }
@@ -1480,11 +1521,15 @@
     return A2S_OK;
 }
 
-static int attn_pair_bwd_combine(hipStream_t st, const a2s_note_dec_bwd_args& a, int s, const AttnPairStep& p) {
+static AttnBwdCombineArgs attn_pair_bwd_combine_args(const a2s_note_dec_bwd_args& a, int s, const AttnPairStep& p) {
     const int H2 = 2 * a.H;
     const long R = a.R;
-    hipLaunchKernelGGL(attn_bwd_combine256, dim3(a.R), dim3(256), 0, st, a.attn_ws + A2S_ATTN_TICKETS, a.dq_all + (long)s * R * a.H, (long)a.H, p.G, p.clip_rank,
-                       a.row_until, p.n_clips, a.R / p.n_clips, p.n_active, p.step, a.ds_all + (long)s * R * a.T, a.T, a.dctx_all + (long)s * R * H2, (long)H2);
-    A2S_CHECK_LAUNCH("attn_bwd_combine256");
-    return A2S_OK;
-}
+    return AttnBwdCombineArgs{a.attn_ws + A2S_ATTN_TICKETS, a.dq_all + (long)s * R * a.H, (long)a.H, p.G, p.clip_rank, a.row_until, p.n_clips, a.R / p.n_clips,
+                              p.n_active, p.step, a.ds_all + (long)s * R * a.T, a.T, a.dctx_all + (long)s * R * H2, (long)H2};
+}
+static int attn_pair_bwd_combine(hipStream_t st, const a2s_note_dec_bwd_args& au, const a2s_note_dec_bwd_args& al, int s, const AttnPairStep& p) {
+    const PairGrid g = {au.R, 1, al.R, 1};
+    hipLaunchKernelGGL(attn_bwd_combine256_pair, a2s_pair_grid_dim(g), dim3(256), 0, st, attn_pair_bwd_combine_args(au, s, p), attn_pair_bwd_combine_args(al, s, p), g);
+    A2S_CHECK_LAUNCH("attn_bwd_combine256_pair");
+    return A2S_OK;
+}
diff --git a/piano_a2s_amd/csrc/a2s_internal.h b/piano_a2s_amd/csrc/a2s_internal.h
--- a/piano_a2s_amd/csrc/a2s_internal.h
+++ b/piano_a2s_amd/csrc/a2s_internal.h
@@ -143,6 +143,17 @@
 long a2s_attn_pair_launches(void);
 struct AttnPairStep { const int* clip_order; const int* clip_rank; int n_clips; int n_active; int step; int G; int chunk; };
 int a2s_pair_events(const char* who, hipEvent_t** ev_out);
+int a2s_pair_handoff(hipEvent_t* ev, hipStream_t su, hipStream_t sl, bool& on_su, bool to_su, const char* who);
+struct PairGrid { int gx0, gy0, gx1, gy1; };
+static inline void a2s_pair_grid_set(PairGrid& g, int staff, int gx, int gy) { if (staff) { g.gx1 = gx; g.gy1 = gy; } else { g.gx0 = gx; g.gy0 = gy; } }
+static inline dim3 a2s_pair_grid_dim(const PairGrid& g) { return dim3(g.gx0 > g.gx1 ? g.gx0 : g.gx1, g.gy0 > g.gy1 ? g.gy0 : g.gy1, 2); }
+#define A2S_PAIR_KERNEL(name, body, Args, ...)                                                                          \
+    __global__ __VA_ARGS__ void name(Args a0, Args a1, PairGrid g) {                                                    \
+        const bool lower = blockIdx.z != 0;                                                                             \
+        if ((int)blockIdx.x >= (lower ? g.gx1 : g.gx0) || (int)blockIdx.y >= (lower ? g.gy1 : g.gy0)) return;           \
+        const Args a = lower ? a1 : a0;       \
+        body(a, (int)blockIdx.x, (int)blockIdx.y);                                                                      \
+    }
 static inline int a2s_record_wait(hipEvent_t ev, hipStream_t from, hipStream_t to, const char* who) {
     hipError_t e = hipEventRecord(ev, from);
     if (e == hipSuccess) e = hipStreamWaitEvent(to, ev, 0);
@@ -192,7 +203,13 @@
     int nrows, const int* rowmap);
 bool a2s_note_step_mid_ok(int H, int E, const void* const* ptrs, int nptrs);
 int a2s_note_step_mid_gru(hipStream_t st, const a2s_note_dec_args& a, int si, int so, int sv, int sv_next, int nrows, const int* rowmap);
+int a2s_note_step_mid_gru_pair(hipStream_t st, const a2s_note_dec_args* const as[2], int si, int so, int sv, const int sv_next[2], const int nrows[2],
+    const int* const rowmap[2]);
 bool a2s_note_step_mid_bwd_ok(const a2s_note_dec_bwd_args& a);
+int a2s_note_step_mid_bwd_pair(hipStream_t st, const a2s_note_dec_bwd_args* const as[2], int s, float* const dh_out[2], const int nrows[2],
+    const int* const rowmap[2]);
+int a2s_note_step_mid_bwd_query_pair(hipStream_t st, const a2s_note_dec_bwd_args* const as[2], int s, float* const dh_out[2], const int nrows[2],
+    const int* const rowmap[2]);
 int a2s_note_step_mid_bwd(hipStream_t st, const a2s_note_dec_bwd_args& a, int s, float* dh_out, int nrows, const int* rowmap);
 int a2s_note_step_mid_bwd_query(hipStream_t st, const a2s_note_dec_bwd_args& a, int s, float* dh_out, int nrows, const int* rowmap);
 
diff --git a/piano_a2s_amd/csrc/a2s_seq.hip b/piano_a2s_amd/csrc/a2s_seq.hip
--- a/piano_a2s_amd/csrc/a2s_seq.hip
+++ b/piano_a2s_amd/csrc/a2s_seq.hip
@@ -331,8 +331,8 @@
 }
 
 
-__global__ __launch_bounds__(256) void note_step_finalize(StepFinArgs a) {
-    const int row = blockIdx.x * 4 + (threadIdx.x >> 6), lane = threadIdx.x & 63;
+__device__ __forceinline__ void note_step_finalize_body(const StepFinArgs& a, int bx, int ) {
+    const int row = bx * 4 + (threadIdx.x >> 6), lane = threadIdx.x & 63;
     if (row >= a.R) return;
     if (*a.n_done >= a.R && a.gt == nullptr) return;
     const int t = a.t + (a.t_base ? *a.t_base : 0);
@@ -372,10 +372,18 @@
         }
     }
 }
+__global__ __launch_bounds__(256) void note_step_finalize(StepFinArgs a) { note_step_finalize_body(a, blockIdx.x, 0); }
+A2S_PAIR_KERNEL(note_step_finalize_pair, note_step_finalize_body, StepFinArgs, __launch_bounds__(256))
 
 static int a2s_note_step_finalize_impl(hipStream_t st, const StepFinArgs& a) {
     hipLaunchKernelGGL(note_step_finalize, dim3(a2s_cdiv(a.R, 4)), dim3(256), 0, st, a);
     A2S_CHECK_LAUNCH("note_step_finalize");
+    return A2S_OK;
+}
+static int a2s_note_step_finalize_pair_impl(hipStream_t st, const StepFinArgs& au, const StepFinArgs& al) {
+    const PairGrid g = {a2s_cdiv(au.R, 4), 1, a2s_cdiv(al.R, 4), 1};
+    hipLaunchKernelGGL(note_step_finalize_pair, a2s_pair_grid_dim(g), dim3(256), 0, st, au, al, g);
+    A2S_CHECK_LAUNCH("note_step_finalize_pair");
     return A2S_OK;
 }
 
@@ -428,7 +436,7 @@
 typedef a2s_note_dec_args NoteDecArgs;
 
 static int attn_pair_sweep(hipStream_t st, const NoteDecArgs& au, const NoteDecArgs& al, int sv, AttnPairStep& p);
-static int attn_pair_combine(hipStream_t st, const NoteDecArgs& a, int si, int sv, const AttnPairStep& p);
+static int attn_pair_combine(hipStream_t st, const NoteDecArgs& au, const NoteDecArgs& al, int si, int sv, const AttnPairStep& p);
 static int note_step_rows(const NoteDecArgs& a, int t) { return (a.row_list && a.n_rows_active && t >= 0) ? a.n_rows_active[t] : a.R; }
 static bool note_step_fusable(const NoteDecArgs& a, int t = -1, int rows_limit = -1) {
     const void* ptrs[] = {a.x, a.h, a.o, a.q, a.w_ih, a.w_hh, a.out_w, a.attn_w};
@@ -456,10 +464,25 @@
     int fused_rows_limit = -1;
     const char* label = "note_decoder";
 };
-struct NoteStep { int si, so, sv, sv_next, t, tf; bool fused, last; const AttnPairStep* pair; };
-static NoteStep note_step_at(const NoteDecArgs& a, const NoteStepMode& m, int s, bool fused, const AttnPairStep* pair = nullptr) {
+struct NoteStep { int si, so, sv, sv_next, t, tf; bool fused, last; };
+static NoteStep note_step_at(const NoteDecArgs& a, const NoteStepMode& m, int s, bool fused) {
     const int i = m.parity_slots ? s & 1 : s, o = m.parity_slots ? (s + 1) & 1 : s + 1;
-    return {.si = i, .so = o, .sv = i, .sv_next = o, .t = s, .tf = a.tf_flags ? a.tf_flags[s] : 0, .fused = fused, .last = s + 1 == a.steps, .pair = pair};
+    return {.si = i, .so = o, .sv = i, .sv_next = o, .t = s, .tf = a.tf_flags ? a.tf_flags[s] : 0, .fused = fused, .last = s + 1 == a.steps};
+}
+
+static StepFinArgs step_fin_args(const NoteDecArgs& a, const NoteStepMode& m, const NoteStep& k) {
+    const int ldx = a.E + 2 * a.H;
+    StepFinArgs f;
+    f.logits = a.logits; f.ldl = a.V; f.probs = a.probs; f.probs_bstride = a.probs_bstride;
+    f.gt = a.gt; f.gt_bstride = a.gt_bstride; f.emb = a.emb;
+    f.xnext = a.x + (long)k.so * a.R * ldx; f.ldx = ldx;
+    f.drop = a.drop ? a.drop + (long)k.so * a.R * a.E : nullptr; f.inv_keep = a.inv_keep;
+    f.argmax_out = a.argmax_out; f.am_bstride = a.am_bstride;
+    f.eos_seen = a.eos_seen; f.lengths = a.lengths; f.n_done = a.n_done; f.steps_exec = a.steps_exec;
+    f.t_base = m.t_base;
+    f.row_until = a.n_active ? a.row_until : nullptr; f.n_clips = a.n_clips > 0 ? a.n_clips : a.R;
+    f.R = a.R; f.V = a.V; f.E = a.E; f.t = k.t; f.teacher_force = k.tf; f.eos_id = a.eos_id; f.max_t = a.steps;
+    return f;
 }
 
 static int enqueue_note_step(hipStream_t st, const NoteDecArgs& a, const NoteStepMode& m, const NoteStep& k) {
@@ -496,8 +519,7 @@
         rc = a2s_gemm_impl(st, gM, 3 * H2, H2, 1.f, hp, H2, 1, a.w_hh, 1, H2, 0.f, a.gh, 3 * H2, a.b_hh, 0, gB, gS * H2, 0, gS * 3 * H2, 0, a.gemm_ws, a.gemm_ws_bytes);
         if (rc) return rc;
     }
-    rc = (mid && k.pair) ? attn_pair_combine(st, a, si, sv, *k.pair)
-                         : a2s_attn_step_fwd_impl(st, a.keys, a.enc, qs, a.H, a.attn_v, xs + a.E, ldx, os + H2, 2 * H2, attw_s, a.R, a.T, a.H, attn_done, a.R, a.attn_ws, rows);
+    rc = a2s_attn_step_fwd_impl(st, a.keys, a.enc, qs, a.H, a.attn_v, xs + a.E, ldx, os + H2, 2 * H2, attw_s, a.R, a.T, a.H, attn_done, a.R, a.attn_ws, rows);
     if (rc) return rc;
     if (m.align) { rc = a2s_attn_align_rows_impl(st, attw_s, a.T, a.R, a.T, m.align->peak + t, m.align->weight + t, m.align->centroid + t, m.align->out_stride, attn_done, a.R); if (rc) return rc; }
     if (mid) {
@@ -520,16 +542,7 @@
                                  a.eos_id, g.pad_id};
         return a2s_beam_step_finalize_impl(st, bs);
     }
-    StepFinArgs f;
-    f.logits = a.logits; f.ldl = a.V; f.probs = a.probs; f.probs_bstride = a.probs_bstride;
-    f.gt = a.gt; f.gt_bstride = a.gt_bstride; f.emb = a.emb;
-    f.xnext = a.x + (long)so * a.R * ldx; f.ldx = ldx;
-    f.drop = a.drop ? a.drop + (long)so * a.R * a.E : nullptr; f.inv_keep = a.inv_keep;
-    f.argmax_out = a.argmax_out; f.am_bstride = a.am_bstride;
-    f.eos_seen = a.eos_seen; f.lengths = a.lengths; f.n_done = a.n_done; f.steps_exec = a.steps_exec;
-    f.t_base = m.t_base;
-    f.row_until = a.n_active ? a.row_until : nullptr; f.n_clips = a.n_clips > 0 ? a.n_clips : a.R;
-    f.R = a.R; f.V = a.V; f.E = a.E; f.t = t; f.teacher_force = k.tf; f.eos_id = a.eos_id; f.max_t = a.steps;
+    const StepFinArgs f = step_fin_args(a, m, k);
     if (m.grammar) return a2s_grammar_step_finalize_impl(st, f, *m.grammar);
     return a2s_note_step_finalize_impl(st, f);
 }
@@ -549,7 +562,7 @@
     e = hipStreamBeginCapture(st, hipStreamCaptureModeRelaxed);
     if (e != hipSuccess) A2S_FAIL(A2S_ERR_HIP, "hipStreamBeginCapture: %s", hipGetErrorString(e));
     for (int j = 0; j < chunk && rc == A2S_OK; ++j)
-        rc = enqueue_note_step(st, a, m, {.si = j & 1, .so = (j + 1) & 1, .sv = 0, .sv_next = 0, .t = j, .tf = 0, .fused = fused, .last = false, .pair = nullptr});
+        rc = enqueue_note_step(st, a, m, {.si = j & 1, .so = (j + 1) & 1, .sv = 0, .sv_next = 0, .t = j, .tf = 0, .fused = fused, .last = false});
     if (rc == A2S_OK) hipLaunchKernelGGL(advance_counter, dim3(1), dim3(64), 0, st, a.t_base, chunk);
     e = hipStreamEndCapture(st, &graph);
     if (rc != A2S_OK) { if (graph) (void)hipGraphDestroy(graph); return rc; }
@@ -673,6 +686,29 @@
     return A2S_OK;
 }
 
+int a2s_pair_handoff(hipEvent_t* ev, hipStream_t su, hipStream_t sl, bool& on_su, bool to_su, const char* who) {
+    if (on_su == to_su) return A2S_OK;
+    on_su = to_su;
+    return to_su ? a2s_record_wait(ev[1], sl, su, who) : a2s_record_wait(ev[0], su, sl, who);
+}
+
+static int enqueue_note_step_pair(hipStream_t st, const NoteDecArgs* const as[2], const NoteStepMode& m, int s, AttnPairStep& p) {
+    const NoteStep ks[2] = {note_step_at(*as[0], m, s, false), note_step_at(*as[1], m, s, false)};
+    int rc = attn_pair_sweep(st, *as[0], *as[1], s, p);
+    if (rc == A2S_OK) rc = attn_pair_combine(st, *as[0], *as[1], ks[0].si, ks[0].sv, p);
+    if (rc) return rc;
+    int nrows[2], sv_next[2];
+    const int* rowmap[2];
+    for (int k = 0; k < 2; ++k) {
+        nrows[k] = note_step_rows(*as[k], s);
+        rowmap[k] = nrows[k] < as[k]->R ? as[k]->row_list : nullptr;
+        sv_next[k] = ks[k].last ? -1 : ks[k].sv_next;
+    }
+    rc = a2s_note_step_mid_gru_pair(st, as, ks[0].si, ks[0].so, ks[0].sv, sv_next, nrows, rowmap);
+    if (rc) return rc;
+    return a2s_note_step_finalize_pair_impl(st, step_fin_args(*as[0], m, ks[0]), step_fin_args(*as[1], m, ks[1]));
+}
+
 int a2s_note_decoder_fwd_pair_impl(hipStream_t su, hipStream_t sl, const NoteDecArgs& au, const NoteDecArgs& al, const int* pair_order,
                                    const int* pair_rank, const int* pair_n_active, int* done_u, int* done_l) {
     const NoteDecArgs* as[2] = {&au, &al};
@@ -691,6 +727,7 @@
     for (int k = 0; k < 2; ++k)
         if (note_decoder_tail_rows(*as[k])) { const int rc = a2s_note_decoder_zero_unwritten(sts[k], *as[k], "note_decoder"); if (rc) return rc; }
     bool prev_q[2] = {false, false};
+    bool lower_on_su = false;
     const int nmax = au.steps > al.steps ? au.steps : al.steps;
     for (int s = 0; s < nmax; ++s) {
         bool fused[2] = {false, false}, in[2];
@@ -703,18 +740,19 @@
         }
         AttnPairStep p = {pair_order, pair_rank, au.n_clips, pair_n_active[s], s, 1, au.T};
         const bool joint = in[0] && in[1] && !fused[0] && !fused[1] && p.n_active > 0 && au.n_active[s] > 0 && al.n_active[s] > 0;
+        if (in[1]) { const int rc = a2s_pair_handoff(ev, su, sl, lower_on_su, joint, m.label); if (rc) return rc; }
         if (joint) {
-            int rc = a2s_record_wait(ev[1], sl, su, m.label);
-            if (rc == A2S_OK) rc = attn_pair_sweep(su, au, al, s, p);
-            if (rc == A2S_OK) rc = a2s_record_wait(ev[0], su, sl, m.label);
+            const int rc = enqueue_note_step_pair(su, as, m, s, p);
             if (rc) return rc;
+            continue;
         }
         for (int k = 0; k < 2; ++k) {
             if (!in[k]) continue;
-            const int rc = enqueue_note_step(sts[k], *as[k], m, note_step_at(*as[k], m, s, fused[k], joint ? &p : nullptr));
+            const int rc = enqueue_note_step(sts[k], *as[k], m, note_step_at(*as[k], m, s, fused[k]));
             if (rc) return rc;
         }
     }
+    { const int rc = a2s_pair_handoff(ev, su, sl, lower_on_su, false, m.label); if (rc) return rc; }
     if (done_u) *done_u = au.steps;
     if (done_l) *done_l = al.steps;
     return A2S_OK;
@@ -1412,14 +1450,20 @@
 }
 
 
-__global__ __launch_bounds__(256) void attn_fwd_combine256(const float* __restrict__ partial, float* __restrict__ ctx, long ldctx,
-                                                           float* __restrict__ ctx2, long ldctx2, float* __restrict__ attw, int T, int G,
-                                                           const int* __restrict__ n_done, int n_rows_total,
-                                                           const int* __restrict__ clip_rank, const int* __restrict__ row_until,
-                                                           int n_clips, int groups, int n_active, int step) {
-    if (n_done && *n_done >= n_rows_total) return;
+struct AttnCombineArgs {
+    const float* partial; float* ctx; long ldctx; float* ctx2; long ldctx2; float* attw; int T, G;
+    const int* n_done; int n_rows_total;
+    const int* clip_rank; const int* row_until;
+    int n_clips, groups, n_active, step;
+};
+__device__ __forceinline__ void attn_fwd_combine256_body(const AttnCombineArgs& a, int bx, int ) {
+    const float* __restrict__ partial = a.partial; float* __restrict__ ctx = a.ctx; float* __restrict__ ctx2 = a.ctx2; float* __restrict__ attw = a.attw;
+    const int* __restrict__ clip_rank = a.clip_rank; const int* __restrict__ row_until = a.row_until;
+    const long ldctx = a.ldctx, ldctx2 = a.ldctx2;
+    const int T = a.T, G = a.G, n_clips = a.n_clips, groups = a.groups, n_active = a.n_active, step = a.step;
+    if (a.n_done && *a.n_done >= a.n_rows_total) return;
     constexpr int H = 256;
-    const int b = blockIdx.x;
+    const int b = bx;
     const int clip = b % n_clips, grp = b / n_clips;
     const int slot = clip_rank ? clip_rank[clip] : clip;
     if (slot >= n_active || (row_until && step >= row_until[b])) {
@@ -1430,6 +1474,8 @@
     attn_combine_row(partial + ((long)slot * groups + grp) * G * (2 * H + 4), G,
                      AttnCombineOut{ctx + (long)b * ldctx, ctx2 ? ctx2 + (long)b * ldctx2 : nullptr, attw ? attw + (long)b * T : nullptr, T}, wgt);
 }
+__global__ __launch_bounds__(256) void attn_fwd_combine256(AttnCombineArgs a) { attn_fwd_combine256_body(a, blockIdx.x, 0); }
+A2S_PAIR_KERNEL(attn_fwd_combine256_pair, attn_fwd_combine256_body, AttnCombineArgs, __launch_bounds__(256))
 
 size_t a2s_attn_workspace_floats_impl(int B, int T, int H, int groups) {
     size_t rows = 0;
@@ -1514,8 +1560,8 @@
         *defer = a2s_attn_deferred{part, attw, r.clip_rank, r.row_until, G, groups, r.n_clips, r.n_active, r.step, T};
         return A2S_OK;
     }
-    hipLaunchKernelGGL(attn_fwd_combine256, dim3(B), dim3(256), 0, st, part, ctx, ldctx, ctx2, ldctx2, attw, T, G, n_done, n_rows_total,
-                       r.clip_rank, r.row_until, r.n_clips, groups, r.n_active, r.step);
+    hipLaunchKernelGGL(attn_fwd_combine256, dim3(B), dim3(256), 0, st,
+                       AttnCombineArgs{part, ctx, ldctx, ctx2, ldctx2, attw, T, G, n_done, n_rows_total, r.clip_rank, r.row_until, r.n_clips, groups, r.n_active, r.step});
     A2S_CHECK_LAUNCH("attn_fwd_combine256");
     return A2S_OK;
 }
@@ -1556,13 +1602,16 @@
     return A2S_OK;
 }
 
-static int attn_pair_combine(hipStream_t st, const NoteDecArgs& a, int si, int sv, const AttnPairStep& p) {
+static AttnCombineArgs attn_pair_combine_args(const NoteDecArgs& a, int si, int sv, const AttnPairStep& p) {
     const int H2 = 2 * a.H, ldx = a.E + H2;
     float* xs = a.x + (long)si * a.R * ldx;
     float* os = a.o + (long)sv * a.R * 2 * H2;
-    hipLaunchKernelGGL(attn_fwd_combine256, dim3(a.R), dim3(256), 0, st, a.attn_ws + A2S_ATTN_TICKETS, xs + a.E, (long)ldx, os + H2, (long)(2 * H2),
-                       a.attw ? a.attw + (long)sv * a.R * a.T : nullptr, a.T, p.G, (const int*)nullptr, a.R, p.clip_rank, a.row_until, p.n_clips,
-                       a.R / p.n_clips, p.n_active, p.step);
-    A2S_CHECK_LAUNCH("attn_fwd_combine256");
-    return A2S_OK;
-}
+    return AttnCombineArgs{a.attn_ws + A2S_ATTN_TICKETS, xs + a.E, (long)ldx, os + H2, (long)(2 * H2), a.attw ? a.attw + (long)sv * a.R * a.T : nullptr, a.T, p.G,
+                           nullptr, a.R, p.clip_rank, a.row_until, p.n_clips, a.R / p.n_clips, p.n_active, p.step};
+}
+static int attn_pair_combine(hipStream_t st, const NoteDecArgs& au, const NoteDecArgs& al, int si, int sv, const AttnPairStep& p) {
+    const PairGrid g = {au.R, 1, al.R, 1};
+    hipLaunchKernelGGL(attn_fwd_combine256_pair, a2s_pair_grid_dim(g), dim3(256), 0, st, attn_pair_combine_args(au, si, sv, p), attn_pair_combine_args(al, si, sv, p), g);
+    A2S_CHECK_LAUNCH("attn_fwd_combine256_pair");
+    return A2S_OK;
+}
diff --git a/piano_a2s_amd/csrc/a2s_step.hip b/piano_a2s_amd/csrc/a2s_step.hip
--- a/piano_a2s_amd/csrc/a2s_step.hip
+++ b/piano_a2s_amd/csrc/a2s_step.hip
@@ -295,16 +295,16 @@
 #define MID_WAVES 4
 #define MID_AHEAD 1
 #endif
-__global__ __launch_bounds__(256, MID_WAVES) void dec_gru_mid(DecGruArgs a) {
+__device__ __forceinline__ void dec_gru_mid_body(const DecGruArgs& a, int bx, int by) {
     __shared__ __attribute__((aligned(16))) float bs[2][48 * MID_LDB];
     const int tid = threadIdx.x, lane = tid & 63, wave = tid >> 6;
     if (a.n_done) {
         const bool done = *a.n_done >= a.R;
-        if (blockIdx.x == 0 && blockIdx.y == 0 && tid == 0) *a.skip = done ? 1 : 0;
+        if (bx == 0 && by == 0 && tid == 0) *a.skip = done ? 1 : 0;
         if (done) return;
     }
     const int H2 = a.H2, R = a.R, kx = a.kx;
-    const int j0 = blockIdx.x * 16, row0 = blockIdx.y * 64 + wave * 16;
+    const int j0 = bx * 16, row0 = by * 64 + wave * 16;
     const int li = lane & 15, lk = lane >> 4;
     const int j = j0 + li;
     const int ncx = (kx + MID_KC - 1) / MID_KC, nc = ncx + (H2 + MID_KC - 1) / MID_KC;
@@ -394,6 +394,8 @@
         }
     }
 }
+__global__ __launch_bounds__(256, MID_WAVES) void dec_gru_mid(DecGruArgs a) { dec_gru_mid_body(a, blockIdx.x, blockIdx.y); }
+A2S_PAIR_KERNEL(dec_gru_mid_pair, dec_gru_mid_body, DecGruArgs, __launch_bounds__(256, MID_WAVES))
 
 #define NTV 11
 #define NVW 6
@@ -626,13 +628,13 @@
     }
 }
 
-__global__ __launch_bounds__(256, MID_WAVES) void dec_bwd_mid(DecBwdProdArgs a) {
+__device__ __forceinline__ void dec_bwd_mid_body(const DecBwdProdArgs& a, int bx, int by) {
     __shared__ __attribute__((aligned(16))) float bs[2][32 * MID_LDB];
     const int lane = threadIdx.x & 63, wave = threadIdx.x >> 6;
     const int li = lane & 15, lk = lane >> 4;
-    const int R = a.R, K = 3 * a.H2, row0 = blockIdx.y * 64 + wave * 16;
-    const bool role_a = (int)blockIdx.x < a.nxa;
-    const int n0 = (role_a ? blockIdx.x : blockIdx.x - a.nxa) * 32;
+    const int R = a.R, K = 3 * a.H2, row0 = by * 64 + wave * 16;
+    const bool role_a = bx < a.nxa;
+    const int n0 = (role_a ? bx : bx - a.nxa) * 32;
     const int ncols = role_a ? a.kx : a.H2;
     float c0[2][4];
     if (!role_a) {
@@ -656,13 +658,17 @@
         }
     }
 }
-
-__global__ __launch_bounds__(256, MID_WAVES) void dec_bwd_query_mid(const float* __restrict__ dq, const float* __restrict__ wh_t, float* __restrict__ dh, int R, int H, int H2,
-                                                         const int* __restrict__ rowmap) {
+__global__ __launch_bounds__(256, MID_WAVES) void dec_bwd_mid(DecBwdProdArgs a) { dec_bwd_mid_body(a, blockIdx.x, blockIdx.y); }
+A2S_PAIR_KERNEL(dec_bwd_mid_pair, dec_bwd_mid_body, DecBwdProdArgs, __launch_bounds__(256, MID_WAVES))
+
+struct DecBwdQueryMidArgs { const float* dq; const float* wh_t; float* dh; int R, H, H2; const int* rowmap; };
+__device__ __forceinline__ void dec_bwd_query_mid_body(const DecBwdQueryMidArgs& a, int bx, int by) {
     __shared__ __attribute__((aligned(16))) float bs[2][32 * MID_LDB];
+    const float* __restrict__ dq = a.dq; const float* __restrict__ wh_t = a.wh_t; float* __restrict__ dh = a.dh; const int* __restrict__ rowmap = a.rowmap;
+    const int R = a.R, H = a.H, H2 = a.H2;
     const int lane = threadIdx.x & 63, wave = threadIdx.x >> 6;
     const int li = lane & 15, lk = lane >> 4;
-    const int row0 = blockIdx.y * 64 + wave * 16, n0 = blockIdx.x * 32;
+    const int row0 = by * 64 + wave * 16, n0 = bx * 32;
     float c0[2][4];
 #pragma unroll
     for (int g = 0; g < 2; ++g)
@@ -682,6 +688,8 @@
         }
     }
 }
+__global__ __launch_bounds__(256, MID_WAVES) void dec_bwd_query_mid(DecBwdQueryMidArgs a) { dec_bwd_query_mid_body(a, blockIdx.x, blockIdx.y); }
+A2S_PAIR_KERNEL(dec_bwd_query_mid_pair, dec_bwd_query_mid_body, DecBwdQueryMidArgs, __launch_bounds__(256, MID_WAVES))
 
 struct DecOutqMidArgs {
     const float* o; long ldo;
@@ -690,13 +698,13 @@
     const int* rowmap;
     int nva, R, H2;
 };
-__global__ __launch_bounds__(256, MID_WAVES) void dec_outq_mid(DecOutqMidArgs a) {
+__device__ __forceinline__ void dec_outq_mid_body(const DecOutqMidArgs& a, int bx, int by) {
     __shared__ __attribute__((aligned(16))) float bs[2][32 * MID_LDB];
     const int lane = threadIdx.x & 63, wave = threadIdx.x >> 6;
     const int li = lane & 15, lk = lane >> 4;
-    const int R = a.R, row0 = blockIdx.y * 64 + wave * 16;
-    const bool role_a = (int)blockIdx.x < a.nva;
-    const int n0 = (role_a ? blockIdx.x : blockIdx.x - a.nva) * 32;
+    const int R = a.R, row0 = by * 64 + wave * 16;
+    const bool role_a = bx < a.nva;
+    const int n0 = (role_a ? bx : bx - a.nva) * 32;
     const int ncols = role_a ? a.V : a.H;
     float bias[2];
 #pragma unroll
@@ -717,6 +725,8 @@
         }
     }
 }
+__global__ __launch_bounds__(256, MID_WAVES) void dec_outq_mid(DecOutqMidArgs a) { dec_outq_mid_body(a, blockIdx.x, blockIdx.y); }
+A2S_PAIR_KERNEL(dec_outq_mid_pair, dec_outq_mid_body, DecOutqMidArgs, __launch_bounds__(256, MID_WAVES))
 
 __global__ __launch_bounds__(64 * NW) void dec_bwd_query(const float* __restrict__ dq, const float* __restrict__ wh_t, float* __restrict__ dh,
                                                          int R, int H, int H2, const int* __restrict__ rowmap) {
@@ -858,7 +868,8 @@
                                 a.dctx_all + (long)s * R * H2, H2, a.dq_all + (long)s * R * a.H, a.H,
                                 a.ds_all + (long)s * R * a.T, R, a.T, a.H, a.attn_ws, rows);
     if (rc) return rc;
-    if (mid) hipLaunchKernelGGL(dec_bwd_query_mid, dim3(a2s_cdiv(H2, 32), a2s_cdiv(nrows, 64)), dim3(256), 0, st, a.dq_all + (long)s * R * a.H, wh_t, dh_out, nrows, a.H, H2, rowmap);
+    if (mid) hipLaunchKernelGGL(dec_bwd_query_mid, dim3(a2s_cdiv(H2, 32), a2s_cdiv(nrows, 64)), dim3(256), 0, st,
+                                DecBwdQueryMidArgs{a.dq_all + (long)s * R * a.H, wh_t, dh_out, nrows, a.H, H2, rowmap});
     else hipLaunchKernelGGL(dec_bwd_query, dim3(a2s_cdiv(H2, 32), a2s_cdiv(nrows, 16)), dim3(64 * NW), 0, st, a.dq_all + (long)s * R * a.H, wh_t, dh_out, nrows, a.H, H2,
                             rowmap);
     A2S_CHECK_LAUNCH("dec_bwd_query");
@@ -871,9 +882,8 @@
     for (int i = 0; i < nptrs; ++i) if (!aligned16(ptrs[i])) return false;
     return true;
 }
-int a2s_note_step_mid_gru(hipStream_t st, const a2s_note_dec_args& a, int si, int so, int sv, int sv_next, int nrows, const int* rowmap) {
+static DecGruArgs mid_gru_args(const a2s_note_dec_args& a, int si, int so, int sv, int nrows, const int* rowmap) {
     const int H2 = 2 * a.H, ldx = a.E + H2, R = a.R;
-    if (nrows <= 0) return A2S_OK;
     DecGruArgs g;
     g.x = a.x + (long)si * R * ldx; g.ldx = ldx; g.kx = ldx;
     g.h = a.h + (long)si * R * H2;
@@ -883,41 +893,110 @@
     g.n_done = nullptr; g.skip = nullptr;
     g.rowmap = rowmap;
     g.R = nrows; g.H2 = H2;
-    hipLaunchKernelGGL(dec_gru_mid, dim3(H2 / 16, a2s_cdiv(nrows, 64)), dim3(256), 0, st, g);
-    __atomic_fetch_add(&g_dec_mid_launches, 1, __ATOMIC_RELAXED);
-    A2S_CHECK_LAUNCH("dec_gru_mid");
+    return g;
+}
+static DecOutqMidArgs mid_outq_args(const a2s_note_dec_args& a, int sv, int sv_next, int nrows, const int* rowmap) {
+    const int H2 = 2 * a.H, R = a.R;
     DecOutqMidArgs f;
-    f.o = g.o; f.ldo = 2 * H2; f.out_w = a.out_w; f.out_b = a.out_b; f.logits = a.logits; f.ldl = a.V; f.V = a.V;
+    f.o = a.o + (long)sv * R * 2 * H2; f.ldo = 2 * H2; f.out_w = a.out_w; f.out_b = a.out_b; f.logits = a.logits; f.ldl = a.V; f.V = a.V;
     f.attn_w = a.attn_w; f.ld_aw = 2 * H2; f.attn_b = a.attn_b; f.q_next = sv_next >= 0 ? a.q + (long)sv_next * R * a.H : nullptr; f.H = a.H;
     f.rowmap = rowmap;
     f.nva = a2s_cdiv(a.V, 32); f.R = nrows; f.H2 = H2;
-    hipLaunchKernelGGL(dec_outq_mid, dim3(f.nva + (f.q_next ? a2s_cdiv(a.H, 32) : 0), a2s_cdiv(nrows, 64)), dim3(256), 0, st, f);
+    return f;
+}
+static int mid_outq_gx(const DecOutqMidArgs& f) { return f.nva + (f.q_next ? a2s_cdiv(f.H, 32) : 0); }
+int a2s_note_step_mid_gru(hipStream_t st, const a2s_note_dec_args& a, int si, int so, int sv, int sv_next, int nrows, const int* rowmap) {
+    if (nrows <= 0) return A2S_OK;
+    const DecGruArgs g = mid_gru_args(a, si, so, sv, nrows, rowmap);
+    hipLaunchKernelGGL(dec_gru_mid, dim3(g.H2 / 16, a2s_cdiv(nrows, 64)), dim3(256), 0, st, g);
+    __atomic_fetch_add(&g_dec_mid_launches, 1, __ATOMIC_RELAXED);
+    A2S_CHECK_LAUNCH("dec_gru_mid");
+    const DecOutqMidArgs f = mid_outq_args(a, sv, sv_next, nrows, rowmap);
+    hipLaunchKernelGGL(dec_outq_mid, dim3(mid_outq_gx(f), a2s_cdiv(nrows, 64)), dim3(256), 0, st, f);
     A2S_CHECK_LAUNCH("dec_outq_mid");
+    return A2S_OK;
+}
+int a2s_note_step_mid_gru_pair(hipStream_t st, const a2s_note_dec_args* const as[2], int si, int so, int sv, const int sv_next[2], const int nrows[2],
+                               const int* const rowmap[2]) {
+    const int served = (nrows[0] > 0) + (nrows[1] > 0);
+    if (!served) return A2S_OK;
+    DecGruArgs g[2];
+    DecOutqMidArgs f[2];
+    PairGrid gg, fg;
+    for (int k = 0; k < 2; ++k) {
+        const int n = nrows[k] > 0 ? nrows[k] : 0;
+        g[k] = mid_gru_args(*as[k], si, so, sv, n, rowmap[k]);
+        f[k] = mid_outq_args(*as[k], sv, sv_next[k], n, rowmap[k]);
+        a2s_pair_grid_set(gg, k, g[k].H2 / 16, a2s_cdiv(n, 64));
+        a2s_pair_grid_set(fg, k, mid_outq_gx(f[k]), a2s_cdiv(n, 64));
+    }
+    hipLaunchKernelGGL(dec_gru_mid_pair, a2s_pair_grid_dim(gg), dim3(256), 0, st, g[0], g[1], gg);
+    __atomic_fetch_add(&g_dec_mid_launches, served, __ATOMIC_RELAXED);
+    A2S_CHECK_LAUNCH("dec_gru_mid_pair");
+    hipLaunchKernelGGL(dec_outq_mid_pair, a2s_pair_grid_dim(fg), dim3(256), 0, st, f[0], f[1], fg);
+    A2S_CHECK_LAUNCH("dec_outq_mid_pair");
     return A2S_OK;
 }
 bool a2s_note_step_mid_bwd_ok(const a2s_note_dec_bwd_args& a) {
     const void* ptrs[] = {a.dgi_all, a.dgh_all, a.dx, a.dh, a.step_ws};
     return a.step_ws && a.step_ws_floats >= a2s_note_step_workspace_floats_impl(a.H, a.E) && a2s_note_step_mid_ok(a.H, a.E, ptrs, 5);
 }
-int a2s_note_step_mid_bwd(hipStream_t st, const a2s_note_dec_bwd_args& a, int s, float* dh_out, int nrows, const int* rowmap) {
+static DecBwdProdArgs mid_bwd_args(const a2s_note_dec_bwd_args& a, int s, float* dh_out, int nrows, const int* rowmap) {
     const int H2 = 2 * a.H, ldx = a.E + H2, R = a.R;
-    if (nrows <= 0) return A2S_OK;
     DecBwdProdArgs p;
     p.dgi = a.dgi_all + (long)s * R * 3 * H2; p.dgh = a.dgh_all + (long)s * R * 3 * H2;
     p.wih_t = a.step_ws + FUSED_HEAD; p.whh_t = p.wih_t + (long)ldx * 3 * H2;
     p.dx = a.dx + (long)s * R * ldx; p.ldx = ldx; p.dh = dh_out;
     p.rowmap = rowmap;
     p.nxa = a2s_cdiv(ldx, 32); p.kx = ldx; p.R = nrows; p.H2 = H2;
-    hipLaunchKernelGGL(dec_bwd_mid, dim3(p.nxa + a2s_cdiv(H2, 32), a2s_cdiv(nrows, 64)), dim3(256), 0, st, p);
+    return p;
+}
+int a2s_note_step_mid_bwd(hipStream_t st, const a2s_note_dec_bwd_args& a, int s, float* dh_out, int nrows, const int* rowmap) {
+    if (nrows <= 0) return A2S_OK;
+    const DecBwdProdArgs p = mid_bwd_args(a, s, dh_out, nrows, rowmap);
+    hipLaunchKernelGGL(dec_bwd_mid, dim3(p.nxa + a2s_cdiv(p.H2, 32), a2s_cdiv(nrows, 64)), dim3(256), 0, st, p);
     __atomic_fetch_add(&g_dec_mid_launches, 1, __ATOMIC_RELAXED);
     A2S_CHECK_LAUNCH("dec_bwd_mid");
     return A2S_OK;
 }
+int a2s_note_step_mid_bwd_pair(hipStream_t st, const a2s_note_dec_bwd_args* const as[2], int s, float* const dh_out[2], const int nrows[2],
+                               const int* const rowmap[2]) {
+    const int served = (nrows[0] > 0) + (nrows[1] > 0);
+    if (!served) return A2S_OK;
+    DecBwdProdArgs p[2];
+    PairGrid pg;
+    for (int k = 0; k < 2; ++k) {
+        const int n = nrows[k] > 0 ? nrows[k] : 0;
+        p[k] = mid_bwd_args(*as[k], s, dh_out[k], n, rowmap[k]);
+        a2s_pair_grid_set(pg, k, p[k].nxa + a2s_cdiv(p[k].H2, 32), a2s_cdiv(n, 64));
+    }
+    hipLaunchKernelGGL(dec_bwd_mid_pair, a2s_pair_grid_dim(pg), dim3(256), 0, st, p[0], p[1], pg);
+    __atomic_fetch_add(&g_dec_mid_launches, served, __ATOMIC_RELAXED);
+    A2S_CHECK_LAUNCH("dec_bwd_mid_pair");
+    return A2S_OK;
+}
+static DecBwdQueryMidArgs mid_bwd_query_args(const a2s_note_dec_bwd_args& a, int s, float* dh_out, int nrows, const int* rowmap) {
+    const int H2 = 2 * a.H, ldx = a.E + H2, R = a.R;
+    const float* wh_t = a.step_ws + FUSED_HEAD + (long)ldx * 3 * H2 + (long)H2 * 3 * H2;
+    return DecBwdQueryMidArgs{a.dq_all + (long)s * R * a.H, wh_t, dh_out, nrows, a.H, H2, rowmap};
+}
 int a2s_note_step_mid_bwd_query(hipStream_t st, const a2s_note_dec_bwd_args& a, int s, float* dh_out, int nrows, const int* rowmap) {
-    const int H2 = 2 * a.H, ldx = a.E + H2, R = a.R;
     if (nrows <= 0) return A2S_OK;
-    const float* wh_t = a.step_ws + FUSED_HEAD + (long)ldx * 3 * H2 + (long)H2 * 3 * H2;
-    hipLaunchKernelGGL(dec_bwd_query_mid, dim3(a2s_cdiv(H2, 32), a2s_cdiv(nrows, 64)), dim3(256), 0, st, a.dq_all + (long)s * R * a.H, wh_t, dh_out, nrows, a.H, H2, rowmap);
+    hipLaunchKernelGGL(dec_bwd_query_mid, dim3(a2s_cdiv(2 * a.H, 32), a2s_cdiv(nrows, 64)), dim3(256), 0, st, mid_bwd_query_args(a, s, dh_out, nrows, rowmap));
     A2S_CHECK_LAUNCH("dec_bwd_query_mid");
     return A2S_OK;
 }
+int a2s_note_step_mid_bwd_query_pair(hipStream_t st, const a2s_note_dec_bwd_args* const as[2], int s, float* const dh_out[2], const int nrows[2],
+                                     const int* const rowmap[2]) {
+    if (nrows[0] <= 0 && nrows[1] <= 0) return A2S_OK;
+    DecBwdQueryMidArgs q[2];
+    PairGrid qg;
+    for (int k = 0; k < 2; ++k) {
+        const int n = nrows[k] > 0 ? nrows[k] : 0;
+        q[k] = mid_bwd_query_args(*as[k], s, dh_out[k], n, rowmap[k]);
+        a2s_pair_grid_set(qg, k, a2s_cdiv(2 * as[k]->H, 32), a2s_cdiv(n, 64));
+    }
+    hipLaunchKernelGGL(dec_bwd_query_mid_pair, a2s_pair_grid_dim(qg), dim3(256), 0, st, q[0], q[1], qg);
+    A2S_CHECK_LAUNCH("dec_bwd_query_mid_pair");
+    return A2S_OK;
+}
```

Result: no change. 629.4 (-0.0%).
